# monatis/clip.cpp

Hardware: AMD Instinct MI355X
Metric: image+text embeddings/sec (higher is better)
Workload: dtype f16

## Files before the change

clip_cpp_amd/__init__.py:

```python
import ctypes as C
import os
import weakref

import numpy as np

_HERE = os.path.dirname(os.path.abspath(__file__))
LIB_PATH = os.environ.get("CLIP_AMD_LIB") or os.path.join(_HERE, "libclip.so")


class ClipTextHparams(C.Structure):
    _fields_ = [("n_vocab", C.c_int32), ("num_positions", C.c_int32), ("hidden_size", C.c_int32),
                ("n_intermediate", C.c_int32), ("projection_dim", C.c_int32), ("n_head", C.c_int32),
                ("n_layer", C.c_int32), ("eps", C.c_float)]


class ClipVisionHparams(C.Structure):
    _fields_ = [("image_size", C.c_int32), ("patch_size", C.c_int32), ("hidden_size", C.c_int32),
                ("n_intermediate", C.c_int32), ("projection_dim", C.c_int32), ("n_head", C.c_int32),
                ("n_layer", C.c_int32), ("eps", C.c_float)]


class ClipTokens(C.Structure):
    _fields_ = [("data", C.POINTER(C.c_int32)), ("size", C.c_size_t)]


class ClipImageU8(C.Structure):
    _fields_ = [("nx", C.c_int), ("ny", C.c_int), ("data", C.POINTER(C.c_uint8)), ("size", C.c_size_t)]


class ClipImageF32(C.Structure):
    _fields_ = [("nx", C.c_int), ("ny", C.c_int), ("data", C.POINTER(C.c_float)), ("size", C.c_size_t)]


class ClipImageU8Batch(C.Structure):
    _fields_ = [("data", C.POINTER(ClipImageU8)), ("size", C.c_size_t)]


class ClipImageF32Batch(C.Structure):
    _fields_ = [("data", C.POINTER(ClipImageF32)), ("size", C.c_size_t)]


API_SYMBOLS = [
    "clip_model_load", "clip_free", "clip_get_text_hparams", "clip_get_vision_hparams", "clip_tokenize",
    "clip_image_u8_make", "clip_image_f32_make", "clip_image_u8_clean", "clip_image_f32_clean", "clip_image_u8_free",
    "clip_image_f32_free", "clip_image_load_from_file", "clip_image_preprocess", "clip_image_batch_preprocess",
    "clip_text_encode", "clip_image_encode", "clip_image_batch_encode", "clip_compare_text_and_image",
    "clip_similarity_score", "softmax_with_sorting", "clip_zero_shot_label_image", "clip_model_quantize",
    "ggml_time_init", "ggml_time_us", "ggml_time_ms",
]
AMD_SYMBOLS = [
    "clip_amd_device_count", "clip_amd_model_load", "clip_amd_model_load_multi", "clip_amd_ctx_device_count", "clip_amd_weights_from_cache", "clip_amd_shard_bounds",
    "clip_amd_gathered_embeddings", "clip_amd_ctx_device", "clip_amd_set_stream", "clip_amd_set_device_shared", "clip_amd_image_batch_encode_device_multi",
    "clip_amd_text_batch_encode_device_multi", "clip_amd_encode_pair_device_multi",
    "clip_amd_image_batch_encode_device", "clip_text_batch_encode", "clip_amd_text_batch_encode_device",
    "clip_amd_image_batch_preprocess_device", "clip_amd_image_batch_encode_u8",
    "clip_amd_zero_shot_score_device", "clip_amd_zero_shot_label_images",
    "clip_amd_synchronize", "clip_amd_profile_enable", "clip_amd_profile_read", "clip_amd_profile_report",
    "clip_amd_test_gemm", "clip_amd_test_gemm_ex", "clip_amd_test_gemm_tile", "clip_amd_test_gemm_tile_ex", "clip_amd_test_skinny", "clip_amd_test_layernorm", "clip_amd_test_attention", "clip_amd_bench_gemm",
    "clip_amd_test_attention_ex", "clip_amd_bench_attention",
    "clip_amd_index_create", "clip_amd_index_add", "clip_amd_index_add_device", "clip_amd_index_size", "clip_amd_index_dim",
    "clip_amd_index_search", "clip_amd_index_search_device", "clip_amd_index_save", "clip_amd_index_load", "clip_amd_index_free",
    "clip_amd_bench_search", "clip_amd_index_range_search", "clip_amd_index_pairs", "clip_amd_bench_range",
]

_lib = None


def build_lib(force=False):
    import importlib
    return importlib.import_module(__name__ + ".build").build(force=force)


def lib():
    global _lib
    if _lib is not None:
        return _lib
    if not os.path.exists(LIB_PATH):
        build_lib()
    L = C.CDLL(LIB_PATH)
    vp, i32, f32p = C.c_void_p, C.c_int, C.POINTER(C.c_float)
    L.clip_model_load.restype = vp
    L.clip_model_load.argtypes = [C.c_char_p, i32]
    L.clip_amd_model_load.restype = vp
    L.clip_amd_model_load.argtypes = [C.c_char_p, i32, i32]
    L.clip_amd_model_load_multi.restype = vp
    L.clip_amd_model_load_multi.argtypes = [C.c_char_p, i32, i32]
    L.clip_amd_ctx_device_count.restype = i32
    L.clip_amd_ctx_device_count.argtypes = [vp]
    L.clip_amd_weights_from_cache.restype = i32
    L.clip_amd_weights_from_cache.argtypes = [vp]
    L.clip_amd_shard_bounds.argtypes = [i32, i32, i32, C.POINTER(i32), C.POINTER(i32), C.POINTER(i32)]
    L.clip_amd_gathered_embeddings.restype = vp
    L.clip_amd_gathered_embeddings.argtypes = [vp, i32]
    L.clip_free.argtypes = [vp]
    L.clip_get_text_hparams.restype = C.POINTER(ClipTextHparams)
    L.clip_get_text_hparams.argtypes = [vp]
    L.clip_get_vision_hparams.restype = C.POINTER(ClipVisionHparams)
    L.clip_get_vision_hparams.argtypes = [vp]
    L.clip_tokenize.restype = C.c_bool
    L.clip_tokenize.argtypes = [vp, C.c_char_p, C.POINTER(ClipTokens)]
    L.clip_image_u8_make.restype = C.POINTER(ClipImageU8)
    L.clip_image_f32_make.restype = C.POINTER(ClipImageF32)
    L.clip_image_u8_clean.argtypes = [C.POINTER(ClipImageU8)]
    L.clip_image_f32_clean.argtypes = [C.POINTER(ClipImageF32)]
    L.clip_image_u8_free.argtypes = [C.POINTER(ClipImageU8)]
    L.clip_image_f32_free.argtypes = [C.POINTER(ClipImageF32)]
    L.clip_image_load_from_file.restype = C.c_bool
    L.clip_image_load_from_file.argtypes = [C.c_char_p, C.POINTER(ClipImageU8)]
    L.clip_image_preprocess.restype = C.c_bool
    L.clip_image_preprocess.argtypes = [vp, C.POINTER(ClipImageU8), C.POINTER(ClipImageF32)]
    L.clip_image_batch_preprocess.argtypes = [vp, i32, C.POINTER(ClipImageU8Batch), C.POINTER(ClipImageF32Batch)]
    L.clip_text_encode.restype = C.c_bool
    L.clip_text_encode.argtypes = [vp, i32, C.POINTER(ClipTokens), f32p, C.c_bool]
    L.clip_text_batch_encode.restype = C.c_bool
    L.clip_text_batch_encode.argtypes = [vp, i32, C.POINTER(ClipTokens), C.c_size_t, f32p, C.c_bool]
    L.clip_image_encode.restype = C.c_bool
    L.clip_image_encode.argtypes = [vp, i32, C.POINTER(ClipImageF32), f32p, C.c_bool]
    L.clip_image_batch_encode.restype = C.c_bool
    L.clip_image_batch_encode.argtypes = [vp, i32, C.POINTER(ClipImageF32Batch), f32p, C.c_bool]
    L.clip_compare_text_and_image.restype = C.c_bool
    L.clip_compare_text_and_image.argtypes = [vp, i32, C.c_char_p, C.POINTER(ClipImageU8), f32p]
    L.clip_similarity_score.restype = C.c_float
    L.clip_similarity_score.argtypes = [f32p, f32p, i32]
    L.softmax_with_sorting.restype = C.c_bool
    L.softmax_with_sorting.argtypes = [f32p, i32, f32p, C.POINTER(C.c_int)]
    L.clip_zero_shot_label_image.restype = C.c_bool
    L.clip_zero_shot_label_image.argtypes = [vp, i32, C.POINTER(ClipImageU8), C.POINTER(C.c_char_p), C.c_size_t, f32p,
                                             C.POINTER(C.c_int)]
    L.clip_model_quantize.restype = C.c_bool
    L.clip_model_quantize.argtypes = [C.c_char_p, C.c_char_p, i32]
    L.clip_amd_device_count.restype = i32
    L.clip_amd_ctx_device.restype = i32
    L.clip_amd_ctx_device.argtypes = [vp]
    L.clip_amd_set_stream.argtypes = [vp, vp]
    L.clip_amd_set_device_shared.restype = None
    L.clip_amd_set_device_shared.argtypes = [vp, i32]
    L.clip_amd_synchronize.argtypes = [vp]
    L.clip_amd_image_batch_encode_device.restype = C.c_bool
    L.clip_amd_image_batch_encode_device.argtypes = [vp, vp, i32, vp, C.c_bool]
    L.clip_amd_image_batch_preprocess_device.restype = C.c_bool
    L.clip_amd_image_batch_preprocess_device.argtypes = [vp, C.POINTER(ClipImageU8), i32, vp]
    L.clip_amd_zero_shot_score_device.restype = C.c_bool
    L.clip_amd_zero_shot_score_device.argtypes = [vp, vp, i32, vp, i32, i32, vp, vp]
    L.clip_amd_zero_shot_label_images.restype = C.c_bool
    L.clip_amd_zero_shot_label_images.argtypes = [vp, C.POINTER(ClipImageU8), i32, C.POINTER(C.c_char_p), C.c_size_t, f32p, C.POINTER(C.c_int)]
    L.clip_amd_image_batch_encode_u8.restype = C.c_bool
    L.clip_amd_image_batch_encode_u8.argtypes = [vp, C.POINTER(ClipImageU8), i32, f32p, C.c_bool]
    L.clip_amd_text_batch_encode_device.restype = C.c_bool
    L.clip_amd_text_batch_encode_device.argtypes = [vp, vp, C.POINTER(C.c_int32), i32, vp, C.c_bool]
    L.clip_amd_image_batch_encode_device_multi.restype = C.c_bool
    L.clip_amd_image_batch_encode_device_multi.argtypes = [vp, C.POINTER(vp), i32, C.c_bool, f32p]
    L.clip_amd_text_batch_encode_device_multi.restype = C.c_bool
    L.clip_amd_text_batch_encode_device_multi.argtypes = [vp, C.POINTER(vp), C.POINTER(C.c_int32), i32, C.c_bool, f32p]
    L.clip_amd_encode_pair_device_multi.restype = C.c_bool
    L.clip_amd_encode_pair_device_multi.argtypes = [vp, C.POINTER(vp), i32, C.POINTER(vp), C.POINTER(C.c_int32), i32, C.c_bool, f32p, f32p]
    L.clip_amd_profile_enable.argtypes = [vp, C.c_bool]
    L.clip_amd_profile_report.restype = i32
    L.clip_amd_profile_report.argtypes = [vp, C.c_char_p, i32, C.c_bool]
    L.clip_amd_test_gemm.restype = i32
    L.clip_amd_test_gemm.argtypes = [i32, vp, C.c_int64, C.c_int64, f32p, C.c_int64, f32p, f32p, f32p, i32, i32]
    L.clip_amd_test_gemm_ex.restype = i32
    L.clip_amd_test_gemm_ex.argtypes = [i32, vp, C.c_int64, C.c_int64, f32p, C.c_int64, f32p, f32p, f32p, i32, i32, i32, C.c_float, i32, i32, f32p]
    L.clip_amd_test_lnfold.restype = i32
    L.clip_amd_test_lnfold.argtypes = [i32, vp, C.c_int64, C.c_int64, vp, C.c_int64, f32p, C.c_int64, f32p, f32p, f32p, f32p, C.c_float, f32p,
                                       i32, i32, i32, i32, i32, C.c_float, f32p, f32p]
    L.clip_amd_test_gemm_tile.restype = i32
    L.clip_amd_test_gemm_tile.argtypes = [C.c_int64, C.c_int64, C.c_int64, i32]
    L.clip_amd_test_gemm_tile_ex.restype = i32
    L.clip_amd_test_gemm_tile_ex.argtypes = [C.c_int64, C.c_int64, C.c_int64, i32, i32]
    L.clip_amd_test_skinny.restype = i32
    L.clip_amd_test_skinny.argtypes = [i32, vp, C.c_int64, C.c_int64, f32p, C.c_int64, f32p, f32p, f32p, f32p, C.c_float, f32p, i32, i32, C.c_float, f32p]
    L.clip_amd_bench_gemm.restype = C.c_float
    L.clip_amd_bench_gemm.argtypes = [i32, C.c_int64, C.c_int64, C.c_int64, i32, i32, i32]
    L.clip_amd_test_layernorm.restype = i32
    L.clip_amd_test_layernorm.argtypes = [f32p, f32p, f32p, C.c_float, C.c_int64, C.c_int64, f32p, i32]
    L.clip_amd_test_attention.restype = i32
    L.clip_amd_test_attention.argtypes = [f32p, i32, i32, i32, i32, i32, f32p]
    L.clip_amd_test_attention_ex.restype = i32
    L.clip_amd_test_attention_ex.argtypes = [f32p, i32, i32, i32, i32, i32, f32p, i32]
    L.clip_amd_bench_attention.restype = C.c_float
    L.clip_amd_bench_attention.argtypes = [i32, i32, i32, i32, i32, i32, i32]
    i64, i64p = C.c_int64, C.POINTER(C.c_int64)
    L.clip_amd_index_create.restype = vp
    L.clip_amd_index_create.argtypes = [vp, i32, i32]
    L.clip_amd_index_add.restype = C.c_bool
    L.clip_amd_index_add.argtypes = [vp, f32p, i64]
    L.clip_amd_index_add_device.restype = C.c_bool
    L.clip_amd_index_add_device.argtypes = [vp, vp, i64]
    L.clip_amd_index_size.restype = i64
    L.clip_amd_index_size.argtypes = [vp]
    L.clip_amd_index_dim.restype = i32
    L.clip_amd_index_dim.argtypes = [vp]
    L.clip_amd_index_search.restype = C.c_bool
    L.clip_amd_index_search.argtypes = [vp, f32p, i32, i32, f32p, i64p]
    L.clip_amd_index_search_device.restype = C.c_bool
    L.clip_amd_index_search_device.argtypes = [vp, vp, i32, i32, vp, vp]
    L.clip_amd_index_save.restype = C.c_bool
    L.clip_amd_index_save.argtypes = [vp, C.c_char_p]
    L.clip_amd_index_load.restype = vp
    L.clip_amd_index_load.argtypes = [vp, C.c_char_p]
    L.clip_amd_index_free.restype = None
    L.clip_amd_index_free.argtypes = [vp]
    L.clip_amd_bench_search.restype = C.c_float
    L.clip_amd_bench_search.argtypes = [i32, i64, i32, i32, i32, i32]
    L.clip_amd_index_range_search.restype = i64
    L.clip_amd_index_range_search.argtypes = [vp, f32p, i32, C.c_float, i64p, f32p, i64p, i64]
    L.clip_amd_index_pairs.restype = i64
    L.clip_amd_index_pairs.argtypes = [vp, C.c_float, i64p, f32p, i64p, i64]
    L.clip_amd_bench_range.restype = C.c_float
    L.clip_amd_bench_range.argtypes = [i32, i64, i32, i32, C.c_float, i32]
    _lib = L
    return L


def device_count():
    return lib().clip_amd_device_count()


def _fp(a):
    return a.ctypes.data_as(C.POINTER(C.c_float))


def _struct_to_dict(s):
    return {f: getattr(s, f) for f, _ in s._fields_}


class Clip:

    def __init__(self, model_path_or_repo_id, verbosity=0, device=None, n_devices=None):
        L = lib()
        path = os.fsencode(model_path_or_repo_id)
        if n_devices is not None:
            self.ctx = L.clip_amd_model_load_multi(path, verbosity, int(n_devices))
        elif device is None:
            self.ctx = L.clip_model_load(path, verbosity)
        else:
            self.ctx = L.clip_amd_model_load(path, verbosity, int(device))
        if not self.ctx:
            raise RuntimeError("clip_model_load failed for %r (no file, malformed GGUF, or no HIP device)" % (model_path_or_repo_id,))
        self.vec_dim = self.vision_config["projection_dim"] or self.text_config["projection_dim"]

    @property
    def vision_config(self):
        return _struct_to_dict(lib().clip_get_vision_hparams(self.ctx).contents)

    @property
    def text_config(self):
        return _struct_to_dict(lib().clip_get_text_hparams(self.ctx).contents)

    @property
    def device(self):
        return lib().clip_amd_ctx_device(self.ctx)

    def tokenize(self, text):
        t = ClipTokens()
        if not lib().clip_tokenize(self.ctx, text.encode("utf-8"), C.byref(t)):
            raise RuntimeError("Could not tokenize text")
        return [t.data[i] for i in range(t.size)]

    def encode_text(self, tokens, n_threads=os.cpu_count(), normalize=True):
        arr = (C.c_int32 * len(tokens))(*tokens)
        t = ClipTokens(C.cast(arr, C.POINTER(C.c_int32)), len(tokens))
        out = np.empty(self.text_config["projection_dim"], dtype=np.float32)
        if not lib().clip_text_encode(self.ctx, n_threads or 1, C.byref(t), _fp(out), normalize):
            raise RuntimeError("Could not encode text")
        return out.tolist()

    def load_preprocess_encode_image(self, image_path, n_threads=os.cpu_count(), normalize=True):
        L = lib()
        img = L.clip_image_u8_make()
        res = L.clip_image_f32_make()
        try:
            if not L.clip_image_load_from_file(os.fsencode(image_path), img):
                raise RuntimeError("Could not load image '%s'" % image_path)
            if not L.clip_image_preprocess(self.ctx, img, res):
                raise RuntimeError("Could not preprocess image")
            out = np.empty(self.vec_dim, dtype=np.float32)
            if not L.clip_image_encode(self.ctx, n_threads or 1, res, _fp(out), normalize):
                raise RuntimeError("Could not encode image")
            return out.tolist()
        finally:
            L.clip_image_u8_free(img)
            L.clip_image_f32_free(res)

    def calculate_similarity(self, text_embedding, image_embedding):
        a = np.asarray(text_embedding, dtype=np.float32)
        b = np.asarray(image_embedding, dtype=np.float32)
        return float(lib().clip_similarity_score(_fp(a), _fp(b), a.size))

    def compare_text_and_image(self, text, image_path, n_threads=os.cpu_count()):
        L = lib()
        img = L.clip_image_u8_make()
        try:
            if not L.clip_image_load_from_file(os.fsencode(image_path), img):
                raise RuntimeError("Could not load image '%s'" % image_path)
            score = C.c_float()
            if not L.clip_compare_text_and_image(self.ctx, n_threads or 1, text.encode("utf-8"), img, C.byref(score)):
                raise RuntimeError("Could not compare text and image")
            return score.value
        finally:
            L.clip_image_u8_free(img)

    def zero_shot_label_image(self, image_path, labels, n_threads=os.cpu_count()):
        L = lib()
        img = L.clip_image_u8_make()
        try:
            if not L.clip_image_load_from_file(os.fsencode(image_path), img):
                raise RuntimeError("Could not load image '%s'" % image_path)
            return self.zero_shot_label_pixels(img, labels, n_threads)
        finally:
            L.clip_image_u8_free(img)

    def zero_shot_label_pixels(self, img_u8_ptr, labels, n_threads=1):
        n = len(labels)
        arr = (C.c_char_p * n)(*[s.encode("utf-8") for s in labels])
        scores = np.empty(n, dtype=np.float32)
        idx = np.empty(n, dtype=np.int32)
        if not lib().clip_zero_shot_label_image(self.ctx, n_threads or 1, img_u8_ptr, arr, n, _fp(scores),
                                                idx.ctypes.data_as(C.POINTER(C.c_int))):
            raise RuntimeError("Could not zero-shot label image")
        return scores.tolist(), idx.tolist()

    def preprocess(self, rgb):
        rgb = np.ascontiguousarray(rgb, dtype=np.uint8)
        ny, nx, _ = rgb.shape
        src = ClipImageU8(nx, ny, rgb.ctypes.data_as(C.POINTER(C.c_uint8)), rgb.size)
        res = ClipImageF32()
        if not lib().clip_image_preprocess(self.ctx, C.byref(src), C.byref(res)):
            raise RuntimeError("Could not preprocess image")
        S = self.vision_config["image_size"]
        out = np.ctypeslib.as_array(res.data, shape=(S, S, 3)).copy()
        lib().clip_image_f32_clean(C.byref(res))
        return out

    @staticmethod
    def _u8_array(images):
        if isinstance(images, np.ndarray) and images.ndim == 4 and images.shape[0] > 0:
            blk = np.ascontiguousarray(images, dtype=np.uint8)
            B = blk.shape[0]
            rec = np.empty(B, dtype=np.dtype([("nx", np.int32), ("ny", np.int32), ("data", np.uint64), ("size", np.uint64)], align=True))
            assert rec.dtype.itemsize == C.sizeof(ClipImageU8)
            rec["nx"], rec["ny"], rec["size"] = blk.shape[2], blk.shape[1], blk[0].size
            rec["data"] = blk.ctypes.data + np.arange(B, dtype=np.uint64) * np.uint64(blk.strides[0])
            return (blk, rec), C.cast(rec.ctypes.data, C.POINTER(ClipImageU8)), B
        keep = [np.ascontiguousarray(im, dtype=np.uint8) for im in images]
        arr = (ClipImageU8 * len(keep))()
        for i, im in enumerate(keep):
            arr[i] = ClipImageU8(im.shape[1], im.shape[0], im.ctypes.data_as(C.POINTER(C.c_uint8)), im.size)
        return keep, arr, len(keep)

    def encode_images_u8(self, images, normalize=True):
        keep, arr, n = self._u8_array(images)
        out = np.empty((n, self.vision_config["projection_dim"]), dtype=np.float32)
        if not lib().clip_amd_image_batch_encode_u8(self.ctx, arr, n, _fp(out), normalize):
            raise RuntimeError("clip_amd_image_batch_encode_u8 failed (see stderr)")
        return out

    def zero_shot_label_images(self, images, labels):
        keep, arr, B = self._u8_array(images)
        n = len(labels)
        lab = (C.c_char_p * n)(*[l.encode("utf-8") for l in labels])
        scores = np.empty((B, n), dtype=np.float32)
        idx = np.empty((B, n), dtype=np.int32)
        if not lib().clip_amd_zero_shot_label_images(self.ctx, arr, B, lab, n, _fp(scores), idx.ctypes.data_as(C.POINTER(C.c_int))):
            raise RuntimeError("clip_amd_zero_shot_label_images failed (see stderr)")
        return scores, idx

    def preprocess_device(self, images, d_out_ptr):
        keep, arr, B = self._u8_array(images)
        if not lib().clip_amd_image_batch_preprocess_device(self.ctx, arr, B, C.c_void_p(d_out_ptr)):
            raise RuntimeError("clip_amd_image_batch_preprocess_device failed (see stderr)")
        self.synchronize()

    @property
    def weights_from_cache(self):
        return bool(lib().clip_amd_weights_from_cache(self.ctx))

    @property
    def n_devices(self):
        return lib().clip_amd_ctx_device_count(self.ctx)

    def encode_images(self, imgs, normalize=True, n_threads=None):
        imgs = np.ascontiguousarray(imgs, dtype=np.float32)
        B, S = imgs.shape[0], imgs.shape[1]
        rec = np.empty(B, dtype=np.dtype([("nx", np.int32), ("ny", np.int32), ("data", np.uint64), ("size", np.uint64)], align=True))
        assert rec.dtype.itemsize == C.sizeof(ClipImageF32)
        rec["nx"], rec["ny"], rec["size"] = S, imgs.shape[2], imgs[0].size if B else 0
        rec["data"] = imgs.ctypes.data + np.arange(B, dtype=np.uint64) * np.uint64(imgs.strides[0] if B else 0)
        batch = ClipImageF32Batch(C.cast(rec.ctypes.data, C.POINTER(ClipImageF32)), B)
        out = np.empty((B, self.vision_config["projection_dim"]), dtype=np.float32)
        if not lib().clip_image_batch_encode(self.ctx, n_threads or min(16, os.cpu_count() or 1), C.byref(batch), _fp(out), normalize):
            raise RuntimeError("clip_image_batch_encode failed (see stderr)")
        return out

    def encode_texts(self, token_lists, normalize=True):
        n = len(token_lists)
        keep = [np.ascontiguousarray(t, dtype=np.int32) for t in token_lists]
        arr = (ClipTokens * n)()
        for i, t in enumerate(keep):
            arr[i] = ClipTokens(t.ctypes.data_as(C.POINTER(C.c_int32)), t.size)
        out = np.empty((n, self.text_config["projection_dim"]), dtype=np.float32)
        if not lib().clip_text_batch_encode(self.ctx, 1, C.cast(arr, C.POINTER(ClipTokens)), n, _fp(out), normalize):
            raise RuntimeError("clip_text_batch_encode failed (see stderr)")
        return out

    def set_stream(self, stream_handle):
        lib().clip_amd_set_stream(self.ctx, C.c_void_p(stream_handle))

    def set_device_shared(self, shared=True):
        lib().clip_amd_set_device_shared(self.ctx, 1 if shared else 0)

    def synchronize(self):
        lib().clip_amd_synchronize(self.ctx)

    def encode_images_device(self, d_imgs_ptr, batch, d_out_ptr, normalize=True):
        if not lib().clip_amd_image_batch_encode_device(self.ctx, C.c_void_p(d_imgs_ptr), batch, C.c_void_p(d_out_ptr), normalize):
            raise RuntimeError("clip_amd_image_batch_encode_device failed (see stderr)")

    def encode_texts_device(self, d_ids_ptr, offsets, d_out_ptr, normalize=True):
        off = np.ascontiguousarray(offsets, dtype=np.int32)
        if not lib().clip_amd_text_batch_encode_device(self.ctx, C.c_void_p(d_ids_ptr), off.ctypes.data_as(C.POINTER(C.c_int32)),
                                                       off.size - 1, C.c_void_p(d_out_ptr), normalize):
            raise RuntimeError("clip_amd_text_batch_encode_device failed (see stderr)")

    def encode_images_device_multi(self, d_img_ptrs, total, normalize=True, out=None):
        arr = (C.c_void_p * len(d_img_ptrs))(*[C.c_void_p(p) for p in d_img_ptrs])
        if not lib().clip_amd_image_batch_encode_device_multi(self.ctx, arr, total, normalize, _fp(out) if out is not None else None):
            raise RuntimeError("clip_amd_image_batch_encode_device_multi failed (see stderr)")
        return out

    def encode_texts_device_multi(self, d_ids_ptrs, offsets, normalize=True, out=None):
        off = np.ascontiguousarray(offsets, dtype=np.int32)
        arr = (C.c_void_p * len(d_ids_ptrs))(*[C.c_void_p(p) for p in d_ids_ptrs])
        if not lib().clip_amd_text_batch_encode_device_multi(self.ctx, arr, off.ctypes.data_as(C.POINTER(C.c_int32)), off.size - 1, normalize,
                                                             _fp(out) if out is not None else None):
            raise RuntimeError("clip_amd_text_batch_encode_device_multi failed (see stderr)")
        return out

    def encode_pair_device_multi(self, d_img_ptrs, n_images, d_ids_ptrs, offsets, normalize=True, out_img=None, out_txt=None):
        off = np.ascontiguousarray(offsets, dtype=np.int32)
        ia = (C.c_void_p * len(d_img_ptrs))(*[C.c_void_p(p) for p in d_img_ptrs])
        ta = (C.c_void_p * len(d_ids_ptrs))(*[C.c_void_p(p) for p in d_ids_ptrs])
        if not lib().clip_amd_encode_pair_device_multi(self.ctx, ia, n_images, ta, off.ctypes.data_as(C.POINTER(C.c_int32)), off.size - 1, normalize,
                                                       _fp(out_img) if out_img is not None else None, _fp(out_txt) if out_txt is not None else None):
            raise RuntimeError("clip_amd_encode_pair_device_multi failed (see stderr)")
        return out_img, out_txt

    def gathered_embeddings_ptr(self, device_index=0):
        return lib().clip_amd_gathered_embeddings(self.ctx, device_index)

    def profile(self, on=True):
        lib().clip_amd_profile_enable(self.ctx, on)

    def profile_report(self, reset=True):
        n = lib().clip_amd_profile_report(self.ctx, None, 0, False)
        buf = C.create_string_buffer(n + 16)
        lib().clip_amd_profile_report(self.ctx, buf, n + 16, reset)
        out = {}
        for line in buf.value.decode().splitlines():
            tag, launches, ms, fl, by = line.split()
            out[tag] = dict(launches=int(launches), ms=float(ms), flops=float(fl), bytes=float(by))
        return out

    def close(self):
        if getattr(self, "ctx", None):
            for ix in list(getattr(self, "_indexes", ())):
                ix.close()
            lib().clip_free(self.ctx)
            self.ctx = None

    def __del__(self):
        try:
            self.close()
        except Exception:
            pass


class Index:

    DTYPES = {"f32": 0, "f16": 1, "i8": 3}
# ... 120 lines not shown
```

clip_cpp_amd/build.py:

```python
import os
import shutil
import subprocess
import sys
from concurrent.futures import ThreadPoolExecutor

HERE = os.path.dirname(os.path.abspath(__file__))
CSRC = os.path.join(HERE, "csrc")
BUILD = os.path.join(HERE, "build")
LIB = os.path.join(HERE, "libclip.so")
GGML_STUB = os.path.join(HERE, "libggml.so")
ARCH = "gfx950"

HOST_SOURCES = ["gguf.cpp", "quant.cpp", "load.cpp", "forward.cpp", "tokenizer.cpp", "preprocess.cpp", "image_io.cpp", "image_formats.cpp",
                "jpeg_decode.cpp", "host_pipeline.cpp", "api.cpp", "search.cpp"]
HIP_SOURCES = ["k_attn.hip", "k_attn_long.hip", "k_attn_f32.hip", "k_misc.hip", "k_preproc.hip", "k_gemm.hip", "k_gemm8.hip", "k_gemm4.hip", "k_gemm32.hip", "k_gemm_f32.hip", "k_skinny.hip", "k_gemm_ring.hip", "k_fold.hip", "k_search.hip", "k_join.hip"]
GEMM_WTYPES = [0, 1, 2, 3, 4, 5]
EXTRA_FLAGS = {"k_attn_f32.hip": ["-fno-slp-vectorize"], "k_attn_long.hip": ["-fno-slp-vectorize"], "k_gemm_f32.hip": ["-fno-slp-vectorize"]}

COMMON = ["-O3", "-std=c++17", "-fPIC", "-ffp-contract=off", "-Wall", "-Wno-unused-function", "-Wno-unused-result", "-Wno-inline-asm", "-Wno-bitwise-instead-of-logical",
          "-I" + os.path.join(os.path.dirname(HERE), "include")]


def hipcc():
    for c in (os.environ.get("HIPCC"), shutil.which("hipcc"), "/opt/rocm/bin/hipcc"):
        if c and os.path.exists(c):
            return c
    raise RuntimeError("hipcc not found")


def _newer(target, deps):
    if not os.path.exists(target):
        return True
    t = os.path.getmtime(target)
    return any(os.path.getmtime(d) > t for d in deps)


def _run(cmd):
    r = subprocess.run(cmd, stdout=subprocess.PIPE, stderr=subprocess.STDOUT, text=True)
    if r.returncode != 0:
        raise RuntimeError("command failed: %s\n%s" % (" ".join(cmd), r.stdout))
    return r.stdout


def build(force=False, verbose=False):
    os.makedirs(BUILD, exist_ok=True)
    cc = hipcc()
    headers = [os.path.join(CSRC, f) for f in os.listdir(CSRC) if f.endswith(".h")]
    headers += [os.path.join(os.path.dirname(HERE), "include", f) for f in ("clip.h", "clip_amd.h")]
    jobs = []
    objs = []
    for src in HOST_SOURCES:
        o = os.path.join(BUILD, src + ".o")
        objs.append(o)
        s = os.path.join(CSRC, src)
        if force or _newer(o, [s] + headers):
            jobs.append([cc, "-x", "hip", "--offload-arch=" + ARCH, "-fwrapv"] + COMMON + ["-c", s, "-o", o])
    for src in HIP_SOURCES:
        s = os.path.join(CSRC, src)
        o = os.path.join(BUILD, src + ".o")
        objs.append(o)
        if force or _newer(o, [s] + headers):
            jobs.append([cc, "--offload-arch=" + ARCH] + COMMON + EXTRA_FLAGS.get(src, []) + ["-c", s, "-o", o])
    s = os.path.join(CSRC, "k_gemm.hip")
    for wt in GEMM_WTYPES:
        o = os.path.join(BUILD, "k_gemm_wt%d.o" % wt)
        objs.append(o)
        if force or _newer(o, [s] + headers):
            jobs.append([cc, "--offload-arch=" + ARCH] + COMMON + ["-DCLIPAMD_GEMM_WT=%d" % wt, "-c", s, "-o", o])
    s = os.path.join(CSRC, "k_skinny.hip")
    for wt in GEMM_WTYPES:
        o = os.path.join(BUILD, "k_skinny_wt%d.o" % wt)
        objs.append(o)
        if force or _newer(o, [s] + headers):
            jobs.append([cc, "--offload-arch=" + ARCH] + COMMON + ["-DCLIPAMD_SKINNY_WT=%d" % wt, "-c", s, "-o", o])
    s = os.path.join(CSRC, "k_gemm_ring.hip")
    for wt in GEMM_WTYPES:
        o = os.path.join(BUILD, "k_gemm_ring_wt%d.o" % wt)
        objs.append(o)
        if force or _newer(o, [s] + headers):
            jobs.append([cc, "--offload-arch=" + ARCH] + COMMON + ["-DCLIPAMD_RING_WT=%d" % wt, "-c", s, "-o", o])
    if jobs:
        with ThreadPoolExecutor(max_workers=min(8, os.cpu_count() or 4)) as ex:
            for out in ex.map(_run, jobs):
                if verbose and out.strip():
                    print(out)
    if force or jobs or _newer(LIB, objs):
        _run([cc, "--offload-arch=" + ARCH, "-shared", "-fPIC", "-o", LIB] + objs + ["-lz", "-lpthread", "-ldl"])
    stub_src = os.path.join(CSRC, "ggml_stub.c")
    if force or _newer(GGML_STUB, [stub_src]):
        _run(["gcc", "-O2", "-fPIC", "-shared", "-o", GGML_STUB, stub_src])
    return LIB


if __name__ == "__main__":
    p = build(force="--force" in sys.argv, verbose=True)
    print("built", p)
```

clip_cpp_amd/csrc/api.cpp:

```cpp
#include <algorithm>
#include <chrono>
#include <cmath>
#include <cstdio>
#include <cstdlib>
#include <cstring>
#include <exception>
#include <thread>
#include <vector>

#include "../../include/clip_amd.h"
#include "model.h"

using namespace clipamd;

namespace {

int default_device() {
    const char * e = getenv("CLIP_AMD_DEVICE");
    if (!e || !*e) e = getenv("LOCAL_RANK");
    if (e && *e) {
        int n = 0;
        if (hipGetDeviceCount(&n) == hipSuccess && n > 0) return atoi(e) % n;
        (void)hipGetLastError();
    }
// ... 683 lines not shown
    DBuf dmu((size_t)M * 4), dmu2((size_t)M * 4);
    if (fold == 2) {
        std::vector<float> mu((size_t)M);
        for (int64_t m = 0; m < M; m++) {
            double sacc = 0;
            for (int64_t k = 0; k < h; k++) sacc += resid[m * h + k];
            mu[(size_t)m] = (float)(sacc / (double)h);
        }
        (void)hipMemcpy(dmu.p, mu.data(), (size_t)M * 4, hipMemcpyHostToDevice);
    }
    launch_f32_to_f16((const float *)da32.p, (int)K1, (half_t *)da16.p, W1.Kpad, (int)M, (int)K1, W1.Kpad, s);
    DBuf skw((size_t)64 << 20), skc(4096 * 4);
    (void)hipMemset(skc.p, 0, 4096 * 4);
    DBuf panel1((size_t)W1.Npad * W1.Kpad * 2), panel2((size_t)W2.Npad * W2.Kpad * 2);
    auto common = [&](GemmParams & p, const DBuf & panel, const DevWeight & W) {
        p.sk_ws = (float *)skw.p; p.sk_ws_floats = (size_t)16 << 20; p.sk_cnt = (unsigned *)skc.p; p.sk_cnt_n = 4096;
        p.w16_scratch = (half_t *)panel.p; p.w16_scratch_halfs = panel.p ? (size_t)W.Npad * W.Kpad : 0;
    };
    GemmParams p1;
    p1.A = (const half_t *)da16.p; p1.lda = W1.Kpad; p1.M = (int)M; p1.W = W1; p1.bias = (const float *)db1.p; p1.out = dx.p; p1.ldc = (int)h;
    p1.resid = (const float *)dx.p;
    common(p1, panel1, W1);
    GemmParams p2;
    p2.A = (const half_t *)dxn.p; p2.lda = W2.Kpad; p2.M = (int)M; p2.W = W2; p2.out = dy16.p; p2.ldc = (int)N2; p2.qcols = qcols; p2.qscale = qscale;
    common(p2, panel2, W2);
    const int epi = epi2 == 1 ? EPI_F16 : epi2 == 2 ? EPI_GELU_F16 : EPI_QGELU_F16;
    if (tile1 < 0) {
        if (M > 128 || h > 2048) { (void)hipFree(w1base); (void)hipFree(w2base); return -5; }
        DBuf dskst((size_t)2 * SKINNY_MAX_ROWS * 128 * sizeof(float2));
        SkinnyParams a1;
        a1.A16 = (const half_t *)da16.p; a1.lda = W1.Kpad; a1.M = (int)M; a1.W = W1; a1.bias = (const float *)db1.p; a1.out = dx.p; a1.ldc = (int)h; a1.resid = (const float *)dx.p;
        SkinnyParams a2;
        a2.M = (int)M; a2.W = W2; a2.out = dy16.p; a2.ldc = (int)N2; a2.qcols = qcols; a2.qscale = qscale; a2.eps = eps;
        if (fold) {
            launch_fold_vectors(W2, (const float *)dg.p, (const float *)dbeta.p, (const float *)db2.p, (float *)dc.p, (float *)dbf.p, s);
            a1.xg_out = (half_t *)dxn.p; a1.ldxg = W2.Kpad; a1.xg_gamma = (const float *)dg.p; a1.fstats_out = (float2 *)dstats.p; a1.fstride_out = st_stride;
            a2.A16 = (const half_t *)dxn.p; a2.lda = W2.Kpad; a2.bias = (const float *)dbf.p; a2.ln_c = (const float *)dc.p;
            a2.fstats = (const float2 *)dstats.p; a2.fslots = (int)h / 16; a2.fslotw = 16; a2.fstride = st_stride;
            if (fold == 2) { a1.xg_mu = (const float *)dmu.p; a2.ln_mu = (const float *)dmu.p; a2.mu_out = (float *)dmu2.p; }
        } else {
            a1.stats_out = (float2 *)dskst.p;
            a2.x32 = (const float *)dx.p; a2.ldx = (int)h; a2.ln_w = (const float *)dg.p; a2.ln_b = (const float *)dbeta.p; a2.stats_in = (const float2 *)dskst.p;
            a2.stats_slots = (int)h / 16; a2.bias = (const float *)db2.p;
        }
        int rc2 = 0;
        if (!skinny_supported(a1, EPI_RESID_F32) || !skinny_supported(a2, epi)) rc2 = -5;
        else {
            launch_skinny(a1, EPI_RESID_F32, s);
            launch_skinny(a2, epi, s);
            launch_f16_to_f32((const half_t *)dy16.p, (int)N2, (float *)dy32.p, (int)N2, (int)M, (int)N2, s);
            if (hipDeviceSynchronize() != hipSuccess || hipGetLastError() != hipSuccess) rc2 = -4;
            else {
                (void)hipMemcpy(x1_out, dx.p, (size_t)M * h * 4, hipMemcpyDeviceToHost);
                (void)hipMemcpy(y_out, dy32.p, (size_t)M * N2 * 4, hipMemcpyDeviceToHost);
            }
        }
        (void)hipFree(w1base);
        (void)hipFree(w2base);
        return rc2;
    }
    if (fold) {
        launch_fold_vectors(W2, (const float *)dg.p, (const float *)dbeta.p, (const float *)db2.p, (float *)dc.p, (float *)dbf.p, s);
        p1.xg_out = (half_t *)dxn.p; p1.ldxg = W2.Kpad; p1.xg_gamma = (const float *)dg.p; p1.stats_out = (float2 *)dstats.p; p1.stats_stride = st_stride;
        int t1 = tile1 ? tile1 : gemm_tile_for((int)M, (int)h, W1.Kpad, W1.wtype != W_F16);
        const int slotw = gemm_fold_slotw(t1);
        if (fold == 2) p1.xg_mu = (const float *)dmu.p;
        launch_gemm(p1, EPI_RESID_F32, tile1, s);
        p2.bias = (const float *)dbf.p; p2.ln_c = (const float *)dc.p; p2.ln_stats = (const float2 *)dstats.p; p2.ln_slotw = slotw; p2.ln_slots = (int)h / slotw;
        p2.ln_stride = st_stride; p2.ln_eps = eps;
        if (fold == 2) { p1.xg_mu = (const float *)dmu.p; p2.ln_mu = (const float *)dmu.p; p2.mu_out = (float *)dmu2.p; }
        launch_gemm(p2, epi, tile2, s);
    } else {
        launch_gemm(p1, EPI_RESID_F32, tile1, s);
        launch_layernorm((const float *)dx.p, (int)h, nullptr, 1, (const float *)dg.p, (const float *)dbeta.p, eps, (int)M, (int)h, (half_t *)dxn.p, W2.Kpad, nullptr, 0, s);
        p2.bias = (const float *)db2.p;
        launch_gemm(p2, epi, tile2, s);
    }
    launch_f16_to_f32((const half_t *)dy16.p, (int)N2, (float *)dy32.p, (int)N2, (int)M, (int)N2, s);
    int rc = 0;
    if (hipDeviceSynchronize() != hipSuccess || hipGetLastError() != hipSuccess) rc = -4;
    else {
        (void)hipMemcpy(x1_out, dx.p, (size_t)M * h * 4, hipMemcpyDeviceToHost);
        (void)hipMemcpy(y_out, dy32.p, (size_t)M * N2 * 4, hipMemcpyDeviceToHost);
    }
    (void)hipFree(w1base);
    (void)hipFree(w2base);
    return rc;
}

int clip_amd_test_gemm(int type, const void * w_raw, int64_t N, int64_t K, const float * x, int64_t M, const float * bias, const float * resid,
                       float * y, int epilogue, int tile) {
    return clip_amd_test_gemm_ex(type, w_raw, N, K, x, M, bias, resid, y, epilogue, tile, 0, 1.0f, 0, 0, nullptr);
}


float clip_amd_bench_gemm(int type, int64_t N, int64_t K, int64_t M, int epilogue, int tile, int iters) {
    int ndev = 0;
    if (hipGetDeviceCount(&ndev) != hipSuccess || ndev <= 0) { (void)hipGetLastError(); return -1.f; }
    std::vector<float> w((size_t)N * K);
    uint32_t st = 12345u;
    for (auto & v : w) { st = st * 1664525u + 1013904223u; v = ((int)(st >> 9) % 2001 - 1000) * 4e-5f; }
    std::vector<uint8_t> raw(ggml_row_bytes(type, K) * (size_t)N);
    if (raw.empty() || quantize_rows(type, w.data(), raw.data(), N, K) == 0) return -2.f;
    DevWeight W;
    void * wbase = nullptr;
    if (!repack_for_test(type, raw.data(), N, K, W, &wbase)) return -2.f;
    const int Kpad = W.Kpad;
    DBuf dx((size_t)(M + 1) * Kpad * 2), dbias((size_t)N * 4), dout((size_t)M * N * 4);
    std::vector<uint16_t> hx((size_t)M * Kpad);
    for (auto & v : hx) { st = st * 1664525u + 1013904223u; v = f32_to_f16_bits(((int)(st >> 9) % 2001 - 1000) * 1e-3f); }
    (void)hipMemcpy(dx.p, hx.data(), hx.size() * 2, hipMemcpyHostToDevice);
    (void)hipMemset(dbias.p, 0, (size_t)N * 4);
    (void)hipMemset(dout.p, 0, (size_t)M * N * 4);
    GemmParams p;
    p.A = (const half_t *)dx.p; p.lda = Kpad; p.M = (int)M; p.W = W; p.bias = (const float *)dbias.p; p.ldc = (int)N; p.out = dout.p;
    p.resid = (const float *)dout.p; p.qcols = 0;
    DBuf skw((size_t)64 << 20), skc(4096 * 4);
    (void)hipMemset(skc.p, 0, 4096 * 4);
    p.sk_ws = (float *)skw.p; p.sk_ws_floats = (size_t)16 << 20; p.sk_cnt = (unsigned *)skc.p; p.sk_cnt_n = 4096;
    DBuf panel((size_t)W.Npad * W.Kpad * 2);
    const bool pre = (epilogue >> 16) & 1;
    if (pre && W.wtype != W_F16 && W.wtype != W_F32 && panel.p) {
        const DevWeight * w = &W;
        half_t * o = (half_t *)panel.p;
        launch_dequant(&w, &o, 1, nullptr);
        p.w16_pre = (const half_t *)panel.p;
    } else {
        p.w16_scratch = (half_t *)panel.p; p.w16_scratch_halfs = panel.p ? (size_t)W.Npad * W.Kpad : 0;
    }
    p.debug = (epilogue >> 8) & 0xFF;
    const bool fold = (epilogue >> 17) & 1;
    epilogue &= 0xFF;
    const int st_stride = (int)((M + 63) & ~(int64_t)63);
    DBuf dstats(fold ? (size_t)(N > K ? N : K) / 32 * st_stride * 8 + 64 : 16), dvec(fold ? (size_t)(N > K ? N : K) * 4 + 64 : 16), dxg(fold ? (size_t)M * N * 2 + 64 : 16);
    if (fold) {
        std::vector<float> hs((size_t)(N > K ? N : K) / 32 * st_stride * 2), hv((size_t)(N > K ? N : K), 1.0f);
        for (size_t i = 0; i < hs.size(); i += 2) { hs[i] = 0.5f * 64; hs[i + 1] = 60.f; }
        (void)hipMemcpy(dstats.p, hs.data(), hs.size() * 4, hipMemcpyHostToDevice);
        (void)hipMemcpy(dvec.p, hv.data(), hv.size() * 4, hipMemcpyHostToDevice);
        if (epilogue == EPI_RESID_F32) {
            p.xg_out = (half_t *)dxg.p; p.ldxg = (int)N; p.xg_gamma = (const float *)dvec.p; p.stats_out = (float2 *)dstats.p; p.stats_stride = st_stride;
        } else if (epilogue == EPI_F16 || epilogue == EPI_GELU_F16 || epilogue == EPI_QGELU_F16) {
            p.ln_c = (const float *)dvec.p; p.ln_stats = (const float2 *)dstats.p; p.ln_slotw = 64; p.ln_slots = (int)K / 64; p.ln_stride = st_stride; p.ln_eps = 1e-5f;
        }
    }
    hipEvent_t a, b;
    (void)hipEventCreate(&a);
    (void)hipEventCreate(&b);
    int rot = 1;
    { const char * e = getenv("GEMM_ROTATE"); if (e) rot = atoi(e); if (rot < 1) rot = 1; if (rot > 64) rot = 64; }
    std::vector<DevWeight> Ws(1, p.W);
    std::vector<const half_t *> pans(1, p.w16_pre);
    std::vector<void *> owned;
    for (int r = 1; r < rot; r++) {
        DevWeight Wr;
        void * base = nullptr;
        if (!repack_for_test(type, raw.data(), N, K, Wr, &base)) break;
        owned.push_back(base);
        const half_t * pr = nullptr;
        if (pre && Wr.wtype != W_F16 && Wr.wtype != W_F32) {
            void * pp = nullptr;
            if (hipMalloc(&pp, (size_t)Wr.Npad * Wr.Kpad * 2) != hipSuccess) break;
            owned.push_back(pp);
            const DevWeight * w = &Wr;
            half_t * o = (half_t *)pp;
            launch_dequant(&w, &o, 1, nullptr);
            pr = (const half_t *)pp;
        }
        Ws.push_back(Wr);
        pans.push_back(pr);
    }
    rot = (int)Ws.size();
    auto go = [&](int i) { p.W = Ws[i % rot]; if (pre) p.w16_pre = pans[i % rot]; launch_gemm(p, epilogue, tile, nullptr); };
    for (int i = 0; i < 3; i++) go(i);
    (void)hipEventRecord(a, nullptr);
    for (int i = 0; i < iters; i++) go(i);
    (void)hipEventRecord(b, nullptr);
    float ms = -1.f;
    if (hipEventSynchronize(b) == hipSuccess && hipGetLastError() == hipSuccess) (void)hipEventElapsedTime(&ms, a, b);
    (void)hipEventDestroy(a);
    (void)hipEventDestroy(b);
    for (void * o : owned) (void)hipFree(o);
    if (getenv("CLIPAMD_G8_STAMPS")) {
        const int nwg = 4096;
        std::vector<unsigned long long> st((size_t)nwg * 8);
        (void)hipMemcpy(st.data(), skw.p, st.size() * 8, hipMemcpyDeviceToHost);
        FILE * f = fopen(getenv("CLIPAMD_G8_STAMPS"), "a");
        if (f) {
            fprintf(f, "# N=%lld K=%lld M=%lld epi=%d tile=%d\n", (long long)N, (long long)K, (long long)M, epilogue, tile);
            for (int i = 0; i < nwg; i++) {
                const unsigned long long * s8 = &st[(size_t)i * 8];
                if (!s8[0] || !s8[3]) continue;
                fprintf(f, "%d %llu %llu %llu %llu %llu %llu %llu\n", i, s8[0], s8[1], s8[2], s8[3], s8[5], s8[4], s8[6]);
            }
            fclose(f);
        }
    }
    (void)hipFree(wbase);
    return ms < 0 ? -4.f : ms * 1000.f / iters;
}

int clip_amd_test_skinny(int type, const void * w_raw, int64_t N, int64_t K, const float * x, int64_t M, const float * bias, const float * resid,
                         const float * ln_w, const float * ln_b, float eps, float * y, int epilogue, int qcols, float qscale, float * stats_out) {
    int ndev = 0;
    if (hipGetDeviceCount(&ndev) != hipSuccess || ndev <= 0) { (void)hipGetLastError(); return -1; }
    DevWeight W;
    void * wbase = nullptr;
    if (!repack_for_test(type, w_raw, N, K, W, &wbase)) return -2;
    const int Kpad = W.Kpad;
    DBuf dx32((size_t)M * K * 4), dx16((size_t)(M + 1) * Kpad * 2), dbias((size_t)N * 4), dout((size_t)M * N * 4), dout32((size_t)M * N * 4), dlw((size_t)K * 4), dlb((size_t)K * 4),
        dst((size_t)2 * SKINNY_MAX_ROWS * 128 * 8);
    hipStream_t s = nullptr;
    (void)hipMemcpy(dx32.p, x, (size_t)M * K * 4, hipMemcpyHostToDevice);
    if (bias) (void)hipMemcpy(dbias.p, bias, (size_t)N * 4, hipMemcpyHostToDevice);
    (void)hipMemset(dst.p, 0, (size_t)2 * SKINNY_MAX_ROWS * 128 * 8);
    SkinnyParams p;
    p.M = (int)M; p.W = W; p.bias = bias ? (const float *)dbias.p : nullptr; p.ldc = (int)N; p.qcols = qcols; p.qscale = qscale;
    if (ln_w) {
        (void)hipMemcpy(dlw.p, ln_w, (size_t)K * 4, hipMemcpyHostToDevice);
        (void)hipMemcpy(dlb.p, ln_b, (size_t)K * 4, hipMemcpyHostToDevice);
        launch_row_stats((const float *)dx32.p, (int)K, (int)M, (int)K, (float2 *)dst.p, s);
        p.x32 = (const float *)dx32.p; p.ldx = (int)K; p.ln_w = (const float *)dlw.p; p.ln_b = (const float *)dlb.p; p.eps = eps;
        p.stats_in = (const float2 *)dst.p; p.stats_slots = 1;
    } else {
        launch_f32_to_f16((const float *)dx32.p, (int)K, (half_t *)dx16.p, Kpad, (int)M, (int)K, Kpad, s);
        p.A16 = (const half_t *)dx16.p; p.lda = Kpad;
    }
    int epi = EPI_F32;
    switch (epilogue) {
    case 0: epi = EPI_F32; p.out = dout32.p; break;
    case 1: epi = EPI_F16; p.out = dout.p; break;
    case 2: epi = EPI_GELU_F16; p.out = dout.p; break;
    case 3: epi = EPI_QGELU_F16; p.out = dout.p; break;
    case 4:
        epi = EPI_RESID_F32;
        (void)hipMemcpy(dout32.p, resid, (size_t)M * N * 4, hipMemcpyHostToDevice);
        p.out = dout32.p; p.resid = (const float *)dout32.p;
        p.stats_out = (float2 *)dst.p + (size_t)SKINNY_MAX_ROWS * 128;
        break;
    default: (void)hipFree(wbase); return -3;
    }
    int rc = 0;
    if (!skinny_supported(p, epi)) rc = -5;
    else {
        launch_skinny(p, epi, s);
        if (epi == EPI_F16 || epi == EPI_GELU_F16 || epi == EPI_QGELU_F16)
            launch_f16_to_f32((const half_t *)dout.p, (int)N, (float *)dout32.p, (int)N, (int)M, (int)N, s);
        if (hipDeviceSynchronize() != hipSuccess || hipGetLastError() != hipSuccess) rc = -4;
        else {
            (void)hipMemcpy(y, dout32.p, (size_t)M * N * 4, hipMemcpyDeviceToHost);
            if (stats_out && epi == EPI_RESID_F32) (void)hipMemcpy(stats_out, (float2 *)dst.p + (size_t)SKINNY_MAX_ROWS * 128, (size_t)128 * 128 * 8, hipMemcpyDeviceToHost);
        }
    }
    (void)hipFree(wbase);
    return rc;
}

int clip_amd_test_layernorm(const float * x, const float * w, const float * b, float eps, int64_t rows, int64_t h, float * y, int out_f16) {
    int ndev = 0;
    if (hipGetDeviceCount(&ndev) != hipSuccess || ndev <= 0) { (void)hipGetLastError(); return -1; }
    DBuf dx((size_t)rows * h * 4), dw((size_t)h * 4), db((size_t)h * 4), dy((size_t)rows * h * 4), dh_((size_t)rows * h * 2);
    (void)hipMemcpy(dx.p, x, (size_t)rows * h * 4, hipMemcpyHostToDevice);
    (void)hipMemcpy(dw.p, w, (size_t)h * 4, hipMemcpyHostToDevice);
    (void)hipMemcpy(db.p, b, (size_t)h * 4, hipMemcpyHostToDevice);
    if (out_f16) {
        launch_layernorm((const float *)dx.p, (int)h, nullptr, 1, (const float *)dw.p, (const float *)db.p, eps, (int)rows, (int)h, (half_t *)dh_.p, (int)h, nullptr, 0, nullptr);
        launch_f16_to_f32((const half_t *)dh_.p, (int)h, (float *)dy.p, (int)h, (int)rows, (int)h, nullptr);
    } else {
        launch_layernorm((const float *)dx.p, (int)h, nullptr, 1, (const float *)dw.p, (const float *)db.p, eps, (int)rows, (int)h, nullptr, 0, (float *)dy.p, (int)h, nullptr);
    }
    if (hipDeviceSynchronize() != hipSuccess || hipGetLastError() != hipSuccess) return -4;
    (void)hipMemcpy(y, dy.p, (size_t)rows * h * 4, hipMemcpyDeviceToHost);
    return 0;
}

static bool launch_attention_kernel(int kernel, const half_t * qkv, half_t * out, int nseq, int T, int h, int n_head, bool causal) {
    switch (kernel) {
    case 0: return launch_attention(qkv, out, nseq, T, nullptr, T, h, n_head, causal, nullptr);
    case 1: return launch_attention_whole_row(qkv, out, nseq, T, nullptr, T, h, n_head, causal, nullptr);
    case 2: return launch_attention_long(qkv, out, nseq, T, nullptr, T, h, n_head, causal, nullptr);
    }
    return false;
}

int clip_amd_test_attention_ex(const float * qkv, int nseq, int T, int h, int n_head, int causal, float * out, int kernel) {
    int ndev = 0;
    if (hipGetDeviceCount(&ndev) != hipSuccess || ndev <= 0) { (void)hipGetLastError(); return -1; }
    if (nseq <= 0 || T <= 0 || h <= 0 || n_head <= 0 || h % n_head) return -3;
    const size_t rows = (size_t)nseq * T;
    DBuf d32(rows * 3 * h * 4), d16(rows * 3 * h * 2), o16(rows * h * 2), o32(rows * h * 4);
    (void)hipMemcpy(d32.p, qkv, rows * 3 * h * 4, hipMemcpyHostToDevice);
    launch_f32_to_f16((const float *)d32.p, 3 * h, (half_t *)d16.p, 3 * h, (int)rows, 3 * h, 3 * h, nullptr);
    if (!launch_attention_kernel(kernel, (const half_t *)d16.p, (half_t *)o16.p, nseq, T, h, n_head, causal != 0)) return -2;
    launch_f16_to_f32((const half_t *)o16.p, h, (float *)o32.p, h, (int)rows, h, nullptr);
    if (hipDeviceSynchronize() != hipSuccess || hipGetLastError() != hipSuccess) return -4;
    (void)hipMemcpy(out, o32.p, rows * h * 4, hipMemcpyDeviceToHost);
    return 0;
}

int clip_amd_test_attention(const float * qkv, int nseq, int T, int h, int n_head, int causal, float * out) {
    return clip_amd_test_attention_ex(qkv, nseq, T, h, n_head, causal, out, 0);
}

float clip_amd_bench_attention(int nseq, int T, int h, int n_head, int causal, int kernel, int iters) {
    int ndev = 0;
    if (hipGetDeviceCount(&ndev) != hipSuccess || ndev <= 0) { (void)hipGetLastError(); return -1.f; }
    if (nseq <= 0 || T <= 0 || h <= 0 || n_head <= 0 || h % n_head || iters <= 0) return -3.f;
    const size_t rows = (size_t)nseq * T;
    std::vector<uint16_t> hx(rows * 3 * h);
    uint32_t st = 12345u;
    const float qs = 1.0f / sqrtf((float)(h / n_head));
    for (size_t i = 0; i < hx.size(); i++) {
        st = st * 1664525u + 1013904223u;
        const float v = ((int)(st >> 9) % 2001 - 1000) * 1e-3f;
        hx[i] = f32_to_f16_bits((int)(i % (3 * h)) < h ? v * qs : v);
    }
    DBuf d16(hx.size() * 2), o16(rows * h * 2);
    (void)hipMemcpy(d16.p, hx.data(), hx.size() * 2, hipMemcpyHostToDevice);
    if (!launch_attention_kernel(kernel, (const half_t *)d16.p, (half_t *)o16.p, nseq, T, h, n_head, causal != 0)) return -2.f;
    if (hipDeviceSynchronize() != hipSuccess) { (void)hipGetLastError(); return -4.f; }
    hipEvent_t e0, e1;
    (void)hipEventCreate(&e0);
    (void)hipEventCreate(&e1);
    (void)hipEventRecord(e0, nullptr);
    for (int i = 0; i < iters; i++) launch_attention_kernel(kernel, (const half_t *)d16.p, (half_t *)o16.p, nseq, T, h, n_head, causal != 0);
    (void)hipEventRecord(e1, nullptr);
    float ms = -1.f;
    if (hipEventSynchronize(e1) != hipSuccess || hipEventElapsedTime(&ms, e0, e1) != hipSuccess) { (void)hipGetLastError(); ms = -1.f; }
    (void)hipEventDestroy(e0);
    (void)hipEventDestroy(e1);
    return ms < 0 ? -4.f : ms * 1000.f / iters;
}

#endif

}
```

clip_cpp_amd/csrc/forward.cpp:

```cpp
#include <cmath>
#include <cstdio>
#include <cstdlib>
#include <cstring>
#include <thread>
#include <utility>

#include "model.h"

namespace clipamd {

namespace {

constexpr size_t kGuardBytes = 4096;
constexpr int kGuardByte = 0xA5;
bool guard_mode() {
    static const bool on = [] { const char * e = getenv("CLIP_AMD_GUARD"); return e && e[0] == '1'; }();
    return on;
}

struct Carver {
    uint8_t * base;
    size_t off = 0;
    std::vector<size_t> * gaps = nullptr;
    explicit Carver(void * b, std::vector<size_t> * g = nullptr) : base((uint8_t *)b), gaps(g) { if (gaps) gaps->clear(); }
    template <typename T> T * take(size_t n) {
        off = (off + 255) & ~(size_t)255;
        T * p = base ? (T *)(base + off) : nullptr;
        off += n * sizeof(T);
        if (guard_mode()) {
            if (gaps) gaps->push_back(off);
            off += kGuardBytes;
        }
        return p;
    }
};

bool guard_arm(clip_ctx * ctx) {
    if (!guard_mode()) return true;
    if (hipMemsetAsync(ctx->ws.base, 0xFF, ctx->ws.bytes, ctx->stream) != hipSuccess) return false;
    for (size_t o : ctx->guard_gaps)
        if (hipMemsetAsync((uint8_t *)ctx->ws.base + o, kGuardByte, kGuardBytes, ctx->stream) != hipSuccess) return false;
    static const bool selftest = [] { const char * e = getenv("CLIP_AMD_GUARD_SELFTEST"); return e && e[0] == '1'; }();
    if (selftest && !ctx->guard_gaps.empty())
        return hipMemsetAsync((uint8_t *)ctx->ws.base + ctx->guard_gaps.back() + 100, 0, 1, ctx->stream) == hipSuccess;
    return true;
}

bool guard_check(clip_ctx * ctx, const char * who) {
    if (!guard_mode()) return true;
    if (hipStreamSynchronize(ctx->stream) != hipSuccess) return false;
    std::vector<uint8_t> h(kGuardBytes);
    bool ok = true;
    for (size_t i = 0; i < ctx->guard_gaps.size(); i++) {
        if (hipMemcpy(h.data(), (uint8_t *)ctx->ws.base + ctx->guard_gaps[i], kGuardBytes, hipMemcpyDeviceToHost) != hipSuccess) return false;
        for (size_t k = 0; k < kGuardBytes; k++)
            if (h[k] != (uint8_t)kGuardByte) {
                fprintf(stderr, "%s: CLIP_AMD_GUARD: workspace buffer %zu was written %zu bytes past its end\n", who, i, k);
                ok = false;
                break;
            }
    }
    return ok;
}

struct ProfScope {
    clip_ctx * ctx;
    hipEvent_t a = nullptr, b = nullptr;
    bool on;
    std::string tag;
    double flops, bytes;
    ProfScope(clip_ctx * c, const char * family, long m, long n, long k, double fl, double by) : ctx(c), on(c->profiling), flops(fl), bytes(by) {
        if (!on) return;
        char buf[96];
        snprintf(buf, sizeof buf, "%s:%ldx%ldx%ld", family, m, n, k);
        tag = buf;
        (void)hipEventCreate(&a);
        (void)hipEventCreate(&b);
        (void)hipEventRecord(a, ctx->stream);
    }
    ~ProfScope() {
        if (!on) return;
        (void)hipEventRecord(b, ctx->stream);
        ctx->pending.push_back({a, b, tag, flops, bytes});
    }
};

double weight_bytes(const DevWeight & W) {
    const double nblk = (double)(W.K / 32) * W.N;
    switch (W.wtype) {
    case W_F16: return (double)W.N * W.K * 2;
    case W_Q4_0: return nblk * 18;
    case W_Q4_1: return nblk * 20;
    case W_Q5_0: return nblk * 22;
    case W_Q5_1: return nblk * 24;
    case W_Q8_0: return nblk * 34;
    case W_F32: return (double)W.N * W.K * 4;
    }
    return 0;
}

bool acts_f32(const clip_ctx * ctx, const DevTower & tw) {
    return ctx->f32_acts && !tw.layers.empty() && tw.layers[0].qkv.wtype == W_F32 && tw.layers[0].o.wtype == W_F32 && tw.layers[0].ff1.wtype == W_F32 && tw.layers[0].ff2.wtype == W_F32 &&
           tw.proj.wtype == W_F32;
}
void layernorm_act(bool f32, const float * x, int ldx, const int * in_rows, int in_row_mul, const float * w, const float * b, float eps, int rows, int h, half_t * dst,
                   hipStream_t s) {
    if (f32) launch_layernorm(x, ldx, in_rows, in_row_mul, w, b, eps, rows, h, nullptr, 0, (float *)dst, h, s);
    else launch_layernorm(x, ldx, in_rows, in_row_mul, w, b, eps, rows, h, dst, h, nullptr, 0, s);
}

bool device_shared(const clip_ctx * ctx) { return ctx->device_shared || ctx->sibling_busy || ctx->owner != nullptr; }

void gemm(clip_ctx * ctx, const char * what, const GemmParams & p0, int epi) {
    GemmParams p = p0;
    p.shared_device = device_shared(ctx);
    p.sk_ws = ctx->sk_ws; p.sk_ws_floats = ctx->sk_ws_floats; p.sk_cnt = ctx->sk_cnt; p.sk_cnt_n = ctx->sk_cnt_n;
    if (!ctx->profiling) {
        launch_gemm(p, epi, 0, ctx->stream);
        return;
    }
    const int wt = p.w16_pre ? (int)W_F16 : p.W.wtype;
    const int tile = gemm_tile_for(p.M, p.W.N, p.W.Kpad, wt != W_F16, p.shared_device);
    const bool panel = gemm_tile_uses_panel(tile) && wt == W_F16;
    const double fl = 2.0 * p.M * (double)p.W.N * p.W.K;
    const double wb = wt == W_F16 ? (double)p.W.N * p.W.K * 2 : weight_bytes(p.W);
    const double by = wb + (double)p.M * p.W.K * 2 + (double)p.M * p.W.N * (epi == EPI_F16 || epi == EPI_GELU_F16 || epi == EPI_QGELU_F16 ? 2 : epi == EPI_RESID_F32 ? 8 : 4)
                      + (p.xg_out ? (double)p.M * p.W.N * 2 : 0.0);
    char fam[96];
    if (wt == W_F32) snprintf(fam, sizeof fam, "gemm_f32_kernel<%d>/%s", epi, what);
    else if (panel && tile % 1000 == 261 && (epi == EPI_F16 || epi == EPI_GELU_F16 || epi == EPI_QGELU_F16)) snprintf(fam, sizeof fam, "gemm32_kernel<%d,4,%d>/%s", tile / 1000 == 320 ? 5 : 4, epi, what);
    else if (panel && tile % 1000 >= 259) snprintf(fam, sizeof fam, "gemm4_kernel<%d>/%s", epi, what);
    else if (panel) snprintf(fam, sizeof fam, "gemm8_kernel<%d,%d>/%s", tile / 32000, epi, what);
    else if (gemm_tile_is_ring(tile)) snprintf(fam, sizeof fam, "gemm_ring_kernel<%d,%d,4,%d,%d>/%s", wt, tile % 1000, tile % 1000 >= 128 ? 4 : 2, epi, what);
    else snprintf(fam, sizeof fam, "gemm_dma_kernel<%d,%d,%d,%d>/%s", wt, gemm_tile_uses_panel(tile) ? 160 : tile / 1000, gemm_tile_uses_panel(tile) ? 128 : tile % 1000, epi, what);
    ProfScope ps(ctx, fam, p.M, p.W.N, p.W.K, fl, by);
    launch_gemm(p, epi, 0, ctx->stream);
}

struct LayerPanels { const half_t * qkv = nullptr, * o = nullptr, * ff1 = nullptr, * ff2 = nullptr; };

bool ensure_panel(clip_ctx * ctx, size_t halfs) {
    if (ctx->w16_panel_halfs >= halfs) return true;
    (void)hipStreamSynchronize(ctx->stream);
    if (ctx->w16_panel) (void)hipFree(ctx->w16_panel);
    ctx->w16_panel = nullptr;
    ctx->w16_panel_halfs = 0;
    if (hipMalloc((void **)&ctx->w16_panel, halfs * sizeof(half_t)) != hipSuccess) { (void)hipGetLastError(); return false; }
    ctx->w16_panel_halfs = halfs;
    return true;
}

LayerPanels dequant_layer(clip_ctx * ctx, const DevLayer & l, int rows, const half_t * const * res = nullptr) {
    LayerPanels lp;
    const DevWeight * ws[4] = {&l.qkv, &l.o, &l.ff1, &l.ff2};
    const half_t ** slot[4] = {&lp.qkv, &lp.o, &lp.ff1, &lp.ff2};
    const DevWeight * jw[4];
    half_t * jo[4];
    int nj = 0;
    size_t need = 0;
    bool todo[4];
    for (int i = 0; i < 4; i++) {
        const bool for32 = i == 0 || i == 2;
        if (res && res[i] && (!for32 || gemm_tile_for(rows, ws[i]->N, ws[i]->Kpad, false, device_shared(ctx)) % 1000 == 261)) { *slot[i] = res[i]; todo[i] = false; continue; }
        todo[i] = ws[i]->wtype != W_F16 && ws[i]->wtype != W_F32 && gemm_tile_uses_panel(gemm_tile_for(rows, ws[i]->N, ws[i]->Kpad, true));
        if (todo[i]) need += (size_t)ws[i]->Npad * ws[i]->Kpad;
    }
    if (!need || !ensure_panel(ctx, need)) return lp;
    size_t off = 0;
    for (int i = 0; i < 4; i++)
        if (todo[i]) {
            jw[nj] = ws[i];
            jo[nj] = ctx->w16_panel + off;
            *slot[i] = jo[nj];
            off += (size_t)ws[i]->Npad * ws[i]->Kpad;
            nj++;
        }
    ProfScope ps(ctx, "dequant_layer", rows, nj, 0, 0, (double)need * 2.5625);
    launch_dequant(jw, jo, nj, ctx->stream);
    return lp;
}

bool skinny_enabled() {
    static int on = -1;
    if (on < 0) { const char * e = getenv("CLIP_AMD_SKINNY"); on = !(e && e[0] == '0'); }
    return on != 0;
}

#ifdef CLIPAMD_SK_TIMING
unsigned long long * g_sk_stamps = nullptr;
int g_sk_stamp_launch = 0;
constexpr int SK_STAMP_LAUNCHES = 512;
#endif

void skinny(clip_ctx * ctx, const char * what, const SkinnyParams & p0, int epi) {
#ifdef CLIPAMD_SK_TIMING
    SkinnyParams p = p0;
    if (!g_sk_stamps && hipMalloc((void **)&g_sk_stamps, SK_STAMP_LAUNCHES * 16 * 8) == hipSuccess) (void)hipMemset(g_sk_stamps, 0, SK_STAMP_LAUNCHES * 16 * 8);
    if (g_sk_stamps) p.stamps = g_sk_stamps + (size_t)(g_sk_stamp_launch++ % SK_STAMP_LAUNCHES) * 16;
#else
    const SkinnyParams & p = p0;
#endif
    if (!ctx->profiling) { launch_skinny(p, epi, ctx->stream); return; }
    char fam[96];
    const int nw = (!p.x32 && p.W.Kpad >= 2048 && (epi == EPI_RESID_F32 || epi == EPI_PATCH_F32)) ? 8 : 4;
    snprintf(fam, sizeof fam, "skinny_kernel<%d,1,%d,%d,%s>/%s", p.W.wtype, nw, epi, p.x32 ? "true" : "false", what);
    const double fl = 2.0 * p.M * (double)p.W.N * p.W.K;
    const double by = weight_bytes(p.W) + (double)p.M * p.W.K * (p.x32 ? 4 : 2) + (double)p.M * p.W.N * (epi == EPI_RESID_F32 ? 8 : epi == EPI_F32 || epi == EPI_PATCH_F32 ? 4 : 2);
    ProfScope ps(ctx, fam, p.M, p.W.N, p.W.K, fl, by);
    launch_skinny(p, epi, ctx->stream);
}

int skinny_row_limit() {
    static int lim = -1;
    if (lim < 0) {
        const char * e = getenv("CLIP_AMD_SKINNY_ROWS");
        lim = e ? atoi(e) : 64;
        if (lim > SKINNY_MAX_ROWS) lim = SKINNY_MAX_ROWS;
    }
    return lim;
}

bool layers_fit_skinny(const DevTower & tw, int rows, int h, int ff) {
    if (!skinny_enabled() || rows <= 0 || rows > skinny_row_limit() || h > 2048 || h % 16 || h / 16 > 128 || tw.layers.empty()) return false;
    const DevLayer & l = tw.layers[0];
    if (l.qkv.wtype == W_F32 || l.o.wtype == W_F32 || l.ff1.wtype == W_F32 || l.ff2.wtype == W_F32) return false;
    return l.qkv.K == l.qkv.Kpad && l.ff1.K == l.ff1.Kpad && l.o.N == h && l.ff2.N == h && l.ff1.N == ff;
}

bool run_layers_skinny(clip_ctx * ctx, const DevTower & tw, int rows, int h, int nh, int ff, float eps, int nseq, int T_uniform,
                       const int * d_seq_start, int max_len, bool causal, float * x, half_t * qkv, half_t * att, half_t * mid) {
    hipStream_t s = ctx->stream;
    const int dh = h / nh;
    const float qscale = 1.0f / sqrtf((float)dh);
    const int act = ctx->use_gelu ? EPI_GELU_F16 : EPI_QGELU_F16;
    float2 * stA = ctx->sk_stats, * stB = ctx->sk_stats + (size_t)SKINNY_MAX_ROWS * 128;
    int slotsA = 1;
    for (const DevLayer & l : tw.layers) {
        SkinnyParams q;
        q.x32 = x; q.ldx = h; q.ln_w = l.ln1_w; q.ln_b = l.ln1_b; q.eps = eps; q.stats_in = stA; q.stats_slots = slotsA;
        q.M = rows; q.W = l.qkv; q.bias = l.qkv_b; q.out = qkv; q.ldc = 3 * h; q.qscale = qscale; q.qcols = h;
        skinny(ctx, "ln1_qkv", q, EPI_F16);
        {
            const double afl = 4.0 * (double)nseq * nh * (double)max_len * max_len * dh;
            ProfScope ps(ctx, "attention", nseq * nh, max_len, dh, afl, (double)rows * h * 8);
            if (!launch_attention(qkv, att, nseq, T_uniform, d_seq_start, max_len, h, nh, causal, s)) {
                fprintf(stderr, "clip (hip): attention kernel does not support T=%d d_head=%d\n", max_len, dh);
                return false;
            }
        }
        SkinnyParams o;
        o.A16 = att; o.lda = h; o.M = rows; o.W = l.o; o.bias = l.o_b; o.out = x; o.ldc = h; o.resid = x; o.stats_out = stB;
        skinny(ctx, "out_resid", o, EPI_RESID_F32);
        SkinnyParams u;
        u.x32 = x; u.ldx = h; u.ln_w = l.ln2_w; u.ln_b = l.ln2_b; u.eps = eps; u.stats_in = stB; u.stats_slots = h / 16;
        u.M = rows; u.W = l.ff1; u.bias = l.ff1_b; u.out = mid; u.ldc = ff;
        skinny(ctx, "ln2_ffn_up", u, act);
        SkinnyParams d;
        d.A16 = mid; d.lda = ff; d.M = rows; d.W = l.ff2; d.bias = l.ff2_b; d.out = x; d.ldc = h; d.resid = x; d.stats_out = stA;
        skinny(ctx, "ffn_down_resid", d, EPI_RESID_F32);
        slotsA = h / 16;
    }
    return true;
}

bool run_layers_skinny_fold(clip_ctx * ctx, const DevTower & tw, int rows, int h, int nh, int ff, float eps, int nseq, int T_uniform,
                            const int * d_seq_start, int max_len, bool causal, float * x, half_t * xn, half_t * qkv, half_t * att, half_t * mid,
                            float2 * stats, int stats_stride, float * mu) {
    hipStream_t s = ctx->stream;
    const int dh = h / nh;
    const float qscale = 1.0f / sqrtf((float)dh);
    const int act = ctx->use_gelu ? EPI_GELU_F16 : EPI_QGELU_F16;
    int slots = 1, slotw = h;
    float * mu_cur = mu, * mu_alt = mu ? mu + stats_stride : nullptr;
    auto consume = [&](SkinnyParams & p, const float * c, const float * bf) {
        p.A16 = xn; p.lda = h; p.bias = bf; p.ln_c = c; p.fstats = stats; p.fslots = slots; p.fslotw = slotw; p.fstride = stats_stride; p.eps = eps;
        if (mu) { p.ln_mu = mu_cur; p.mu_out = mu_alt; std::swap(mu_cur, mu_alt); }
    };
    auto produce = [&](SkinnyParams & p, const float * gamma_next) {
        if (!gamma_next) return;
        p.xg_mu = mu_cur;
        p.xg_out = xn; p.ldxg = h; p.xg_gamma = gamma_next; p.fstats_out = stats; p.fstride_out = stats_stride;
        slots = h / 16; slotw = 16;
    };
    for (size_t li = 0; li < tw.layers.size(); li++) {
        const DevLayer & l = tw.layers[li];
        SkinnyParams q;
        q.M = rows; q.W = l.qkv; q.out = qkv; q.ldc = 3 * h; q.qscale = qscale; q.qcols = h;
        consume(q, l.qkv_c, l.qkv_bf);
        skinny(ctx, "ln1_qkv", q, EPI_F16);
        {
            const double afl = 4.0 * (double)nseq * nh * (double)max_len * max_len * dh;
            ProfScope ps(ctx, "attention", nseq * nh, max_len, dh, afl, (double)rows * h * 8);
            if (!launch_attention(qkv, att, nseq, T_uniform, d_seq_start, max_len, h, nh, causal, s)) {
                fprintf(stderr, "clip (hip): attention kernel does not support T=%d d_head=%d\n", max_len, dh);
                return false;
            }
        }
        SkinnyParams o;
        o.A16 = att; o.lda = h; o.M = rows; o.W = l.o; o.bias = l.o_b; o.out = x; o.ldc = h; o.resid = x;
        produce(o, l.ln2_w);
        skinny(ctx, "out_resid", o, EPI_RESID_F32);
        SkinnyParams u;
        u.M = rows; u.W = l.ff1; u.out = mid; u.ldc = ff;
        consume(u, l.ff1_c, l.ff1_bf);
        skinny(ctx, "ln2_ffn_up", u, act);
        SkinnyParams d;
        d.A16 = mid; d.lda = ff; d.M = rows; d.W = l.ff2; d.bias = l.ff2_b; d.out = x; d.ldc = h; d.resid = x;
        produce(d, li + 1 < tw.layers.size() ? tw.layers[li + 1].ln1_w : nullptr);
        skinny(ctx, "ffn_down_resid", d, EPI_RESID_F32);
    }
    return true;
}

bool run_layers(clip_ctx * ctx, const DevTower & tw, int rows, int h, int nh, int ff, float eps, int nseq, int T_uniform,
                const int * d_seq_start, int max_len, bool causal, float * x, half_t * xn, half_t * qkv, half_t * att, half_t * mid, bool prune_last,
                const half_t * const * resp = nullptr) {
    hipStream_t s = ctx->stream;
    const int dh = h / nh;
    const float qscale = 1.0f / sqrtf((float)dh);
    const int act = ctx->use_gelu ? EPI_GELU_F16 : EPI_QGELU_F16;
    const bool f32 = acts_f32(ctx, tw);
    for (size_t li = 0; li < tw.layers.size(); li++) {
        const DevLayer & l = tw.layers[li];
        const LayerPanels lp = dequant_layer(ctx, l, rows, resp ? resp + 4 * li : nullptr);
        {
            ProfScope ps(ctx, "layernorm", rows, h, 0, 0, (double)rows * h * 6);
            layernorm_act(f32, x, h, nullptr, 1, l.ln1_w, l.ln1_b, eps, rows, h, xn, s);
        }
        GemmParams p;
        p.A = xn; p.lda = h; p.M = rows; p.W = l.qkv; p.bias = l.qkv_b; p.out = qkv; p.ldc = 3 * h; p.w16_pre = lp.qkv;
        p.qscale = qscale; p.qcols = h;
        p.act_f32 = f32;
        gemm(ctx, "gemm_qkv", p, EPI_F16);
        {
            const double afl = 4.0 * (double)nseq * nh * (double)max_len * max_len * dh;
            ProfScope ps(ctx, "attention", nseq * nh, max_len, dh, afl, (double)rows * h * 8);
            if (!(f32 ? launch_attention_f32((const float *)qkv, (float *)att, nseq, T_uniform, d_seq_start, max_len, h, nh, causal, s)
                      : launch_attention(qkv, att, nseq, T_uniform, d_seq_start, max_len, h, nh, causal, s))) {
                fprintf(stderr, "clip (hip): attention kernel does not support T=%d d_head=%d\n", max_len, dh);
                return false;
            }
        }
        if (prune_last && li + 1 == tw.layers.size()) break;
        GemmParams po;
        po.A = att; po.lda = h; po.M = rows; po.W = l.o; po.bias = l.o_b; po.out = x; po.ldc = h; po.resid = x; po.w16_pre = lp.o; po.act_f32 = f32;
        gemm(ctx, "gemm_out", po, EPI_RESID_F32);
        {
            ProfScope ps(ctx, "layernorm", rows, h, 0, 0, (double)rows * h * 6);
            layernorm_act(f32, x, h, nullptr, 1, l.ln2_w, l.ln2_b, eps, rows, h, xn, s);
        }
        GemmParams p1;
        p1.A = xn; p1.lda = h; p1.M = rows; p1.W = l.ff1; p1.bias = l.ff1_b; p1.out = mid; p1.ldc = ff; p1.w16_pre = lp.ff1; p1.act_f32 = f32;
        gemm(ctx, "gemm_ffn_up", p1, act);
        GemmParams p2;
        p2.A = mid; p2.lda = ff; p2.M = rows; p2.W = l.ff2; p2.bias = l.ff2_b; p2.out = x; p2.ldc = h; p2.resid = x; p2.w16_pre = lp.ff2; p2.act_f32 = f32;
        gemm(ctx, "gemm_ffn_down", p2, EPI_RESID_F32);
    }
    return true;
}

bool run_layers_fold(clip_ctx * ctx, const DevTower & tw, int rows, int h, int nh, int ff, float eps, int nseq, int T_uniform,
                     const int * d_seq_start, int max_len, bool causal, float * x, half_t * xn, half_t * qkv, half_t * att, half_t * mid,
                     float2 * stats, int stats_stride, float * mu, bool prune_last, const half_t * const * ff2p = nullptr) {
    hipStream_t s = ctx->stream;
    const int dh = h / nh;
    const float qscale = 1.0f / sqrtf((float)dh);
    const int act = ctx->use_gelu ? EPI_GELU_F16 : EPI_QGELU_F16;
    int slots = 1, slotw = h;
    float * mu_cur = mu, * mu_alt = mu ? mu + stats_stride : nullptr;
    auto consume = [&](GemmParams & p, const float * c, const float * bf) {
        p.A = xn; p.lda = h; p.bias = bf; p.ln_c = c; p.ln_stats = stats; p.ln_slots = slots; p.ln_slotw = slotw; p.ln_stride = stats_stride; p.ln_eps = eps;
        if (mu) { p.ln_mu = mu_cur; p.mu_out = mu_alt; std::swap(mu_cur, mu_alt); }
    };
    auto produce = [&](GemmParams & p, const float * gamma_next) {
        if (!gamma_next) return;
        p.xg_mu = mu_cur;
        p.xg_out = xn; p.ldxg = h; p.xg_gamma = gamma_next; p.stats_out = stats; p.stats_stride = stats_stride;
        const bool quant = !p.w16_pre && p.W.wtype != W_F16;
        slotw = gemm_fold_slotw_for(p.M, p.W.N, p.W.Kpad, quant, device_shared(ctx));
        slots = h / slotw;
    };
    for (size_t li = 0; li < tw.layers.size(); li++) {
        const DevLayer & l = tw.layers[li];
        const LayerPanels lp = dequant_layer(ctx, l, rows, ff2p ? ff2p + 4 * li : nullptr);
        GemmParams p;
        p.M = rows; p.W = l.qkv; p.out = qkv; p.ldc = 3 * h; p.w16_pre = lp.qkv;
        p.qscale = qscale; p.qcols = h;
        consume(p, l.qkv_c, l.qkv_bf);
        gemm(ctx, "gemm_qkv", p, EPI_F16);
        {
            const double afl = 4.0 * (double)nseq * nh * (double)max_len * max_len * dh;
            ProfScope ps(ctx, "attention", nseq * nh, max_len, dh, afl, (double)rows * h * 8);
            if (!launch_attention(qkv, att, nseq, T_uniform, d_seq_start, max_len, h, nh, causal, s)) {
                fprintf(stderr, "clip (hip): attention kernel does not support T=%d d_head=%d\n", max_len, dh);
                return false;
            }
        }
        if (prune_last && li + 1 == tw.layers.size()) break;
        GemmParams po;
        po.A = att; po.lda = h; po.M = rows; po.W = l.o; po.bias = l.o_b; po.out = x; po.ldc = h; po.resid = x; po.w16_pre = lp.o;
        produce(po, l.ln2_w);
        gemm(ctx, "gemm_out", po, EPI_RESID_F32);
        GemmParams p1;
        p1.M = rows; p1.W = l.ff1; p1.out = mid; p1.ldc = ff; p1.w16_pre = lp.ff1;
        consume(p1, l.ff1_c, l.ff1_bf);
        gemm(ctx, "gemm_ffn_up", p1, act);
        GemmParams p2;
        p2.A = mid; p2.lda = ff; p2.M = rows; p2.W = l.ff2; p2.bias = l.ff2_b; p2.out = x; p2.ldc = h; p2.resid = x; p2.w16_pre = lp.ff2;
        produce(p2, li + 1 < tw.layers.size() ? tw.layers[li + 1].ln1_w : nullptr);
        gemm(ctx, "gemm_ffn_down", p2, EPI_RESID_F32);
    }
    return true;
}

bool pooled_tail(clip_ctx * ctx, const DevLayer & l, int n, int h, int ff, float eps, const float * x, const half_t * att, const int * in_rows,
                 int in_row_mul, float * xp, half_t * ap, half_t * xnp, half_t * midp) {
    hipStream_t s = ctx->stream;
    const int act = ctx->use_gelu ? EPI_GELU_F16 : EPI_QGELU_F16;
    const bool f32 = ctx->f32_acts && l.o.wtype == W_F32 && l.ff1.wtype == W_F32 && l.ff2.wtype == W_F32;
    {
        ProfScope ps(ctx, "gather_pooled", n, h, 0, 0, (double)n * h * 12);
        if (f32) {
            launch_gather_rows(x, nullptr, in_rows, in_row_mul, n, h, xp, nullptr, s);
            launch_gather_rows((const float *)att, nullptr, in_rows, in_row_mul, n, h, (float *)ap, nullptr, s);
        } else launch_gather_rows(x, att, in_rows, in_row_mul, n, h, xp, ap, s);
    }
    GemmParams po;
    po.A = ap; po.lda = h; po.M = n; po.W = l.o; po.bias = l.o_b; po.out = xp; po.ldc = h; po.resid = xp; po.act_f32 = f32;
    gemm(ctx, "gemm_out_pooled", po, EPI_RESID_F32);
    {
        ProfScope ps(ctx, "layernorm", n, h, 0, 0, (double)n * h * 6);
        layernorm_act(f32, xp, h, nullptr, 1, l.ln2_w, l.ln2_b, eps, n, h, xnp, s);
    }
    GemmParams p1;
    p1.A = xnp; p1.lda = h; p1.M = n; p1.W = l.ff1; p1.bias = l.ff1_b; p1.out = midp; p1.ldc = ff; p1.act_f32 = f32;
    gemm(ctx, "gemm_ffn_up_pooled", p1, act);
    GemmParams p2;
    p2.A = midp; p2.lda = ff; p2.M = n; p2.W = l.ff2; p2.bias = l.ff2_b; p2.out = xp; p2.ldc = h; p2.resid = xp; p2.act_f32 = f32;
    gemm(ctx, "gemm_ffn_down_pooled", p2, EPI_RESID_F32);
    return true;
}

const half_t * const * resident_panels(clip_ctx * ctx, const DevTower & tw, int which, int rows) {
    if (!ctx->resident_panels_on || tw.layers.empty()) return nullptr;
    if (ctx->owner) {
        clip_ctx * o = ctx->owner;
        return (o->res_panel_mask[which] && o->res_panels[which].size() == 4 * tw.layers.size()) ? o->res_panels[which].data() : nullptr;
    }
    const DevLayer & l0 = tw.layers[0];
    unsigned want = 0;
    if (l0.ff2.wtype != W_F16 && l0.ff2.wtype != W_F32 && rows >= 4096 && gemm_tile_uses_panel(gemm_tile_for(rows, l0.ff2.N, l0.ff2.Kpad, false))) want |= 8u;
    if (l0.o.wtype != W_F16 && l0.o.wtype != W_F32 && rows >= 4096 && rows < 32768 && gemm_tile_uses_panel(gemm_tile_for(rows, l0.o.N, l0.o.Kpad, false))) want |= 2u;
    if (rows >= 32768 && l0.qkv.wtype != W_F16 && l0.qkv.wtype != W_F32 && gemm_tile_for(rows, l0.qkv.N, l0.qkv.Kpad, false, device_shared(ctx)) % 1000 == 261) want |= 1u;
    if (rows >= 32768 && l0.ff1.wtype != W_F16 && l0.ff1.wtype != W_F32 && gemm_tile_for(rows, l0.ff1.N, l0.ff1.Kpad, false, device_shared(ctx)) % 1000 == 261) want |= 4u;
    if (!want) return nullptr;
    auto & tab = ctx->res_panels[which];
    if ((ctx->res_panel_mask[which] & want) == want && tab.size() == 4 * tw.layers.size()) return tab.data();
    hipStreamCaptureStatus cs = hipStreamCaptureStatusNone;
    (void)hipStreamIsCapturing(ctx->stream, &cs);
    if (cs != hipStreamCaptureStatusNone) return (ctx->res_panel_mask[which] && tab.size() == 4 * tw.layers.size()) ? tab.data() : nullptr;
    want |= ctx->res_panel_mask[which];
    (void)hipStreamSynchronize(ctx->stream);
    if (ctx->res_panel_buf[which]) (void)hipFree(ctx->res_panel_buf[which]);
    ctx->res_panel_buf[which] = nullptr;
    ctx->res_panel_mask[which] = 0;
    tab.clear();
    size_t halfs = 0;
    for (const DevLayer & l : tw.layers) {
        const DevWeight * ws[4] = {&l.qkv, &l.o, &l.ff1, &l.ff2};
        for (int i = 0; i < 4; i++) if (want >> i & 1) halfs += (size_t)ws[i]->Npad * ws[i]->Kpad;
    }
    if (hipMalloc((void **)&ctx->res_panel_buf[which], halfs * sizeof(half_t)) != hipSuccess) { (void)hipGetLastError(); return nullptr; }
    size_t off = 0;
    for (const DevLayer & l : tw.layers) {
        const DevWeight * ws[4] = {&l.qkv, &l.o, &l.ff1, &l.ff2};
        for (int i = 0; i < 4; i++) {
            if (!(want >> i & 1)) { tab.push_back(nullptr); continue; }
            half_t * o = ctx->res_panel_buf[which] + off;
            launch_dequant(&ws[i], &o, 1, ctx->stream);
            tab.push_back(o);
            off += (size_t)ws[i]->Npad * ws[i]->Kpad;
        }
    }
    (void)hipStreamSynchronize(ctx->stream);
    ctx->res_panel_mask[which] = want;
    return tab.data();
}

bool fold_pays(const DevTower & tw, int rows, bool shared) {
    if (tw.layers.empty()) return false;
    const DevLayer & l = tw.layers[0];
    for (const DevWeight * w : {&l.qkv, &l.o, &l.ff1, &l.ff2})
        if (gemm_tile_uses_panel(gemm_tile_for(rows, w->N, w->Kpad, w->wtype != W_F16, shared)) &&
            gemm_tile_for(rows, w->N, w->Kpad, w->wtype != W_F16, shared) % 1000 != 261) return false;
    return true;
}

bool check_device(clip_ctx * ctx, const char * who) {
    if (!ctx || ctx->device < 0) {
        fprintf(stderr, "%s: no HIP device bound to this context — the encoders have no CPU fallback\n", who);
        return false;
    }
    if (hipSetDevice(ctx->device) != hipSuccess) {
        fprintf(stderr, "%s: hipSetDevice(%d) failed\n", who, ctx->device);
        return false;
    }
    return true;
}

bool launch_ok(const char * who) {
    const hipError_t e = hipGetLastError();
    if (e != hipSuccess) {
        fprintf(stderr, "%s: HIP launch error: %s\n", who, hipGetErrorString(e));
        return false;
    }
    return true;
}

}

void drop_graphs(clip_ctx * ctx) {
    for (auto & g : ctx->vgraphs) {
        if (g.exec) (void)hipGraphExecDestroy(g.exec);
        if (g.graph) (void)hipGraphDestroy(g.graph);
    }
    ctx->vgraphs.clear();
    for (auto & g : ctx->tgraphs) {
        if (g.exec) (void)hipGraphExecDestroy(g.exec);
        if (g.graph) (void)hipGraphDestroy(g.graph);
    }
    ctx->tgraphs.clear();
}

bool ensure_workspace(clip_ctx * ctx, size_t bytes) {
    if (ctx->ws.bytes >= bytes) return true;
    (void)hipStreamSynchronize(ctx->stream);
    drop_graphs(ctx);
    if (ctx->owner) {
        (void)hipStreamSynchronize(ctx->owner->stream);
        drop_graphs(ctx->owner);
    }
    if (ctx->ws.base) (void)hipFree(ctx->ws.base);
    ctx->ws.base = nullptr;
    ctx->ws.bytes = 0;
    const size_t want = bytes + bytes / 8 + (1 << 20);
    if (hipMalloc(&ctx->ws.base, want) != hipSuccess) {
        (void)hipGetLastError();
        fprintf(stderr, "clip (hip): cannot allocate %zu MB of workspace\n", want >> 20);
        return false;
    }
    ctx->ws.bytes = want;
    return true;
}

bool ensure_pinned(clip_ctx * ctx, size_t bytes) {
    if (ctx->pinned_bytes >= bytes) return true;
    if (ctx->pinned) (void)hipHostFree(ctx->pinned);
    ctx->pinned = nullptr;
    ctx->pinned_bytes = 0;
    if (hipHostMalloc(&ctx->pinned, bytes, hipHostMallocDefault) != hipSuccess) {
        (void)hipGetLastError();
        return false;
    }
    ctx->pinned_bytes = bytes;
    return true;
}

bool ensure_io(clip_ctx * ctx, size_t in_bytes, size_t out_bytes) {
    auto grow = [&](void *& p, size_t & have, size_t want) {
        if (have >= want) return true;
        (void)hipStreamSynchronize(ctx->stream);
        if (p) (void)hipFree(p);
        p = nullptr;
        have = 0;
        if (hipMalloc(&p, want) != hipSuccess) { (void)hipGetLastError(); return false; }
        have = want;
        return true;
    };
    return grow(ctx->io_in, ctx->io_in_bytes, in_bytes) && grow(ctx->io_out, ctx->io_out_bytes, out_bytes);
}

void prof_collect(clip_ctx * ctx) {
    if (ctx->pending.empty()) return;
    (void)hipStreamSynchronize(ctx->stream);
    for (auto & p : ctx->pending) {
        float ms = 0;
        if (hipEventElapsedTime(&ms, p.a, p.b) == hipSuccess) {
            ProfEntry & e = ctx->prof[p.tag];
            e.ms += ms;
            e.launches += 1;
            e.flops += p.flops;
            e.bytes += p.bytes;
        }
        (void)hipEventDestroy(p.a);
        (void)hipEventDestroy(p.b);
    }
    ctx->pending.clear();
}

static bool vision_forward_one(clip_ctx * ctx, const float * d_imgs, int B, float * d_out, bool normalize);

static bool vision_forward_launch(clip_ctx * ctx, const float * d_imgs, int B, float * d_out, bool normalize) {
    bool split = !ctx->weights_borrowed && !ctx->sibling_busy && !ctx->profiling && ctx->has_vision_encoder && B >= 2;
    if (split) {
        if (ctx->split_max >= 0) split = B >= ctx->split_min && B <= ctx->split_max;
        else {
            const auto & hp = ctx->vision_hparams;
            const int G = hp.image_size / hp.patch_size;
            const long rows = (long)B * (G * G + 1);
            split = hp.hidden_size >= 1024 ? (rows >= 2000 && rows <= 8400) : (rows >= 2000 && rows <= 3300);
        }
    }
    int ways = split ? std::min(ctx->split_ways, B) : 1;
    clip_ctx * part_ctx[4] = {ctx, nullptr, nullptr, nullptr};
    if (split) {
        hipStreamCaptureStatus cs = hipStreamCaptureStatusNone;
        (void)hipStreamIsCapturing(ctx->stream, &cs);
        for (int w = 1; w < ways; w++) {
            clip_ctx * have = w == 1 ? ctx->sibling : ctx->more_siblings[w - 2];
            part_ctx[w] = have ? have : (cs == hipStreamCaptureStatusNone ? sibling_context(ctx, w - 1) : nullptr);
            if (!part_ctx[w]) { ways = 1; break; }
        }
    }
    ctx->last_launch_split = ways >= 2;
    if (ways < 2) return vision_forward_one(ctx, d_imgs, B, d_out, normalize);
    const size_t per = (size_t)ctx->vision_hparams.image_size * ctx->vision_hparams.image_size * 3;
    const int proj = ctx->vision_hparams.projection_dim;
    if (hipEventRecord(ctx->ev_fork, ctx->stream) != hipSuccess) return false;
    bool ok = true;
    int b0 = 0;
    for (int w = 0; w < ways; w++) {
        const int n = B / ways + (w < B % ways ? 1 : 0);
        clip_ctx * c = part_ctx[w];
        c->input_f16 = ctx->input_f16;
        const float * src = ctx->input_f16 ? (const float *)((const half_t *)d_imgs + (size_t)b0 * per) : d_imgs + (size_t)b0 * per;
        if (w > 0 && hipStreamWaitEvent(c->stream, ctx->ev_fork, 0) != hipSuccess) return false;
        ok = vision_forward_one(c, src, n, d_out + (size_t)b0 * proj, normalize) && ok;
        b0 += n;
    }
    for (int w = 1; w < ways; w++) {
        hipEvent_t ej = w == 1 ? ctx->ev_join : ctx->ev_join_more[w - 2];
        if (hipEventRecord(ej, part_ctx[w]->stream) != hipSuccess || hipStreamWaitEvent(ctx->stream, ej, 0) != hipSuccess) return false;
    }
    return ok;
}

bool renew_streams_after_failed_capture(clip_ctx * ctx) {
    bool ok = true, synced = false;
    auto one = [&](clip_ctx * c) {
        if (!c) return;
        hipStreamCaptureStatus st = hipStreamCaptureStatusNone;
        const hipError_t qe = hipStreamIsCapturing(c->stream, &st);
        (void)hipGetLastError();
        if (qe == hipSuccess && st == hipStreamCaptureStatusNone) return;
        if (c->stream != c->own_stream) { ok = false; return; }
        if (!synced) { (void)hipDeviceSynchronize(); (void)hipGetLastError(); synced = true; }
        hipStream_t fresh = nullptr;
        if (hipStreamCreateWithFlags(&fresh, hipStreamNonBlocking) != hipSuccess) { (void)hipGetLastError(); ok = false; return; }
        (void)hipStreamDestroy(c->own_stream);
        (void)hipGetLastError();
        c->own_stream = c->stream = fresh;
        if (c->verbosity >= 1 || (c->owner && c->owner->verbosity >= 1)) fprintf(stderr, "clip (hip): stream replaced after an invalidated capture\n");
    };
    one(ctx);
    one(ctx->sibling);
    for (clip_ctx * ms : ctx->more_siblings) one(ms);
    return ok;
}

namespace {
void break_capture_for_test() {
    static const bool on = [] { const char * e = getenv("CLIP_AMD_TEST_BREAK_CAPTURE"); return e && e[0] == '1'; }();
    if (!on) return;
    hipStreamCaptureMode m = hipStreamCaptureModeThreadLocal;
    (void)hipThreadExchangeStreamCaptureMode(&m);
    void * q = nullptr;
    if (hipMalloc(&q, 256) == hipSuccess && q) (void)hipFree(q);
    (void)hipThreadExchangeStreamCaptureMode(&m);
    (void)hipGetLastError();
}
}

bool vision_forward_device(clip_ctx * ctx, const float * d_imgs, int B, float * d_out, bool normalize) {
    if (!check_device(ctx, "clip_image_batch_encode")) return false;
    if (!ctx->graphs_enabled || ctx->profiling || B <= 0 || B > 32 || !ctx->has_vision_encoder || guard_mode())
        return vision_forward_launch(ctx, d_imgs, B, d_out, normalize);
    auto find = [&]() -> clip_ctx::GraphEntry * {
        for (auto & g : ctx->vgraphs)
            if (g.B == B && g.in == d_imgs && g.out == d_out && g.norm == normalize && g.in_f16 == ctx->input_f16 && g.busy_seen == ctx->sibling_busy) return &g;
        return nullptr;
    };
    clip_ctx::GraphEntry * e = find();
    if (e && e->exec) {
        if (e->split && ctx->sibling_busy) return vision_forward_launch(ctx, d_imgs, B, d_out, normalize);
        return hipGraphLaunch(e->exec, ctx->stream) == hipSuccess;
    }
    if (!e) {
        if (ctx->vgraphs.size() >= 16) drop_graphs(ctx);
        ctx->vgraphs.push_back({B, d_imgs, d_out, normalize, ctx->input_f16, 1, nullptr, nullptr, false, ctx->sibling_busy});
        return vision_forward_launch(ctx, d_imgs, B, d_out, normalize);
    }
    if (hipStreamBeginCapture(ctx->stream, hipStreamCaptureModeThreadLocal) != hipSuccess) {
        (void)hipGetLastError();
        return vision_forward_launch(ctx, d_imgs, B, d_out, normalize);
    }
    break_capture_for_test();
    const bool ok = vision_forward_launch(ctx, d_imgs, B, d_out, normalize);
    const bool captured_split = ctx->last_launch_split;
    hipGraph_t graph = nullptr;
    const hipError_t ce = hipStreamEndCapture(ctx->stream, &graph);
    e = find();
    if (!ok || ce != hipSuccess || !graph || !e) {
        (void)hipGetLastError();
        if (graph) (void)hipGraphDestroy(graph);
        ctx->graphs_enabled = false;
        if (!renew_streams_after_failed_capture(ctx)) { fprintf(stderr, "clip_image_batch_encode: the caller's stream is left in an invalidated capture\n"); return false; }
        return vision_forward_launch(ctx, d_imgs, B, d_out, normalize);
    }
    hipGraphExec_t exec = nullptr;
    if (hipGraphInstantiate(&exec, graph, nullptr, nullptr, 0) != hipSuccess) {
        (void)hipGetLastError();
        (void)hipGraphDestroy(graph);
        ctx->graphs_enabled = false;
        return vision_forward_launch(ctx, d_imgs, B, d_out, normalize);
    }
    e->graph = graph;
    e->exec = exec;
    e->split = captured_split;
    return hipGraphLaunch(exec, ctx->stream) == hipSuccess;
}

bool vision_stage_begin(clip_ctx * ctx, int Bc, VisionStage & st) {
    const auto & hp = ctx->vision_hparams;
    const DevTower & V = ctx->vision;
    const int S = hp.image_size, P = hp.patch_size, G = S / P, Np = G * G, T = Np + 1;
    const int h = hp.hidden_size, ff = hp.n_intermediate, proj = hp.projection_dim;
    const int rows = Bc * T;
    st.Bc = Bc;
    st.st_stride = (rows + 63) & ~63;
    auto carve = [&](Carver & c) {
        st.stats = c.take<float2>((size_t)(h / 16) * st.st_stride);
        st.mu = c.take<float>((size_t)2 * st.st_stride);
        st.x = c.take<float>((size_t)rows * h);
        const size_t aw = acts_f32(ctx, V) ? 2 : 1;
        st.xn = c.take<half_t>(aw * rows * h);
        st.qkv = c.take<half_t>(aw * rows * 3 * h);
        st.att = c.take<half_t>(aw * rows * h);
        st.mid = c.take<half_t>(aw * rows * ff);
        st.col = c.take<half_t>((size_t)Bc * Np * V.patch.Kpad);
        st.pooled = c.take<half_t>(aw * Bc * h);
        st.emb = c.take<float>((size_t)Bc * proj);
        st.xp = c.take<float>((size_t)Bc * h);
        st.ap = c.take<half_t>(aw * Bc * h);
        st.xnp = c.take<half_t>(aw * Bc * h);
        st.midp = c.take<half_t>(aw * Bc * ff);
    };
    Carver sizer(nullptr);
    carve(sizer);
    if (!ensure_workspace(ctx, sizer.off + 4096)) return false;
    Carver c(ctx->ws.base, &ctx->guard_gaps);
    carve(c);
    return guard_arm(ctx);
}

bool vision_stage_patch(clip_ctx * ctx, const VisionStage & st, const void * imgs, int i0, int n) {
    const bool piece = n < st.Bc;
    const auto & hp = ctx->vision_hparams;
    const DevTower & V = ctx->vision;
    const int S = hp.image_size, P = hp.patch_size, G = S / P, Np = G * G, T = Np + 1, h = hp.hidden_size;
    hipStream_t s = ctx->stream;
    half_t * col = st.col + (size_t)i0 * Np * V.patch.Kpad;
    float * x = st.x + (size_t)i0 * T * h;
    {
        ProfScope ps(ctx, "im2col", n * Np, V.patch.Kpad, 0, 0, (double)n * S * S * 3 * (ctx->input_f16 ? 2 : 4) + (double)n * Np * V.patch.Kpad * 2);
        launch_im2col(imgs, ctx->input_f16, col, n, S, P, V.patch.Kpad, s);
    }
    GemmParams pp;
    pp.A = col; pp.lda = V.patch.Kpad; pp.M = n * Np; pp.W = V.patch; pp.out = x; pp.ldc = h;
    pp.Np = Np; pp.T = T; pp.pos = V.pos; pp.no_splitk = piece;
    gemm(ctx, "gemm_patch", pp, EPI_PATCH_F32);
    return true;
}

bool vision_stage_finish(clip_ctx * ctx, const VisionStage & st, float * d_out, bool normalize) {
    const auto & hp = ctx->vision_hparams;
    const DevTower & V = ctx->vision;
    const int S = hp.image_size, P = hp.patch_size, G = S / P, Np = G * G, T = Np + 1;
    const int h = hp.hidden_size, ff = hp.n_intermediate, nh = hp.n_head, proj = hp.projection_dim;
    hipStream_t s = ctx->stream;
    const int Bc = st.Bc, rows = Bc * T;
    float * x = st.x;
    const bool skinny = layers_fit_skinny(V, rows, h, ff);
    const bool fold = ctx->ln_fold && !V.layers.empty() && (ctx->ln_fold_force || fold_pays(V, rows, device_shared(ctx)));
    {
        ProfScope ps(ctx, "layernorm", rows, h, 0, 0, (double)rows * h * (fold ? 10 : 8));
        if (fold)
            launch_layernorm_prep(x, h, V.pre_ln_w, V.pre_ln_b, hp.eps, rows, h, x, h, V.layers[0].ln1_w, st.xn, h, st.stats, s, ctx->ln_fold_centre ? st.mu : nullptr,
                                  V.class_embd, V.pos, T);
        else {
            launch_cls_rows(x, V.class_embd, V.pos, Bc, T, h, s);
            launch_layernorm(x, h, nullptr, 1, V.pre_ln_w, V.pre_ln_b, hp.eps, rows, h, nullptr, 0, x, h, s);
        }
    }
    const bool prune = ctx->prune_last && !skinny && !V.layers.empty() && T > 1;
    if (skinny && fold) {
        if (!run_layers_skinny_fold(ctx, V, rows, h, nh, ff, hp.eps, Bc, T, nullptr, T, false, x, st.xn, st.qkv, st.att, st.mid, st.stats, st.st_stride, ctx->ln_fold_centre ? st.mu : nullptr)) return false;
    } else if (skinny) {
        launch_row_stats(x, h, rows, h, ctx->sk_stats, s);
        if (!run_layers_skinny(ctx, V, rows, h, nh, ff, hp.eps, Bc, T, nullptr, T, false, x, st.qkv, st.att, st.mid)) return false;
    } else if (fold) {
        if (!run_layers_fold(ctx, V, rows, h, nh, ff, hp.eps, Bc, T, nullptr, T, false, x, st.xn, st.qkv, st.att, st.mid, st.stats, st.st_stride, ctx->ln_fold_centre ? st.mu : nullptr, prune, resident_panels(ctx, V, 0, rows))) return false;
    } else if (!run_layers(ctx, V, rows, h, nh, ff, hp.eps, Bc, T, nullptr, T, false, x, st.xn, st.qkv, st.att, st.mid, prune, resident_panels(ctx, V, 0, rows))) return false;
    const bool f32 = acts_f32(ctx, V);
    if (prune) {
        if (!pooled_tail(ctx, V.layers.back(), Bc, h, ff, hp.eps, x, st.att, nullptr, T, st.xp, st.ap, st.xnp, st.midp)) return false;
        layernorm_act(f32, st.xp, h, nullptr, 1, V.post_ln_w, V.post_ln_b, hp.eps, Bc, h, st.pooled, s);
    } else {
        layernorm_act(f32, x, h, nullptr, T, V.post_ln_w, V.post_ln_b, hp.eps, Bc, h, st.pooled, s);
    }
    GemmParams pj;
    pj.A = st.pooled; pj.lda = h; pj.M = Bc; pj.W = V.proj; pj.out = st.emb; pj.ldc = proj; pj.act_f32 = f32;
    gemm(ctx, "gemm_proj", pj, EPI_F32);
    launch_l2norm(st.emb, d_out, Bc, proj, normalize, s);
    return launch_ok("clip_image_batch_encode") && guard_check(ctx, "clip_image_batch_encode");
}

int vision_max_chunk(const clip_ctx * ctx) {
    const auto & hp = ctx->vision_hparams;
    const int S = hp.image_size, P = hp.patch_size, G = S / P, Np = G * G, T = Np + 1;
    const int h = hp.hidden_size, ff = hp.n_intermediate;
    const size_t aw = acts_f32(ctx, ctx->vision) ? 2 : 1;
    const size_t per_img = (size_t)T * ((size_t)h * 4 + aw * ((size_t)h * 2 * 2 + (size_t)3 * h * 2 + (size_t)ff * 2)) + (size_t)Np * ctx->vision.patch.Kpad * 2;
    return (int)std::min<size_t>(1024, std::max<size_t>(1, ((size_t)6 << 30) / per_img));
}

static bool vision_forward_one(clip_ctx * ctx, const float * d_imgs, int B, float * d_out, bool normalize) {
    if (!ctx->has_vision_encoder) {
        printf("This gguf file seems to have no vision encoder\n");
        return false;
    }
    if (B <= 0) return true;
    const int S = ctx->vision_hparams.image_size, proj = ctx->vision_hparams.projection_dim;
    const int chunk = std::min(B, vision_max_chunk(ctx));
    for (int b0 = 0; b0 < B; b0 += chunk) {
        const int Bc = std::min(chunk, B - b0);
        VisionStage st;
        if (!vision_stage_begin(ctx, Bc, st)) return false;
        const void * imgs = ctx->input_f16 ? (const void *)((const half_t *)d_imgs + (size_t)b0 * S * S * 3) : (const void *)(d_imgs + (size_t)b0 * S * S * 3);
        if (!vision_stage_patch(ctx, st, imgs, 0, Bc)) return false;
        if (!vision_stage_finish(ctx, st, d_out + (size_t)b0 * proj, normalize)) return false;
    }
    return true;
}

bool text_forward_device(clip_ctx * ctx, const int32_t * d_ids, const int32_t * h_offsets, int n_texts, float * d_out,
                         bool normalize) {
    if (!check_device(ctx, "clip_text_encode")) return false;
    if (!ctx->has_text_encoder) {
        printf("This GGUF file seems to have no text encoder\n");
        return false;
    }
    if (n_texts <= 0) return true;
    const auto & hp = ctx->text_hparams;
    const DevTower & Tw = ctx->text;
    const int h = hp.hidden_size, ff = hp.n_intermediate, nh = hp.n_head, proj = hp.projection_dim;
    hipStream_t s = ctx->stream;
    const int rows = h_offsets[n_texts] - h_offsets[0];
    int max_len = 0;
    for (int i = 0; i < n_texts; i++) {
        const int len = h_offsets[i + 1] - h_offsets[i];
        if (len <= 0 || len > hp.num_positions) {
            fprintf(stderr, "clip_text_encode: %d tokens is outside [1, %d]\n", len, hp.num_positions);
            return false;
        }
        max_len = std::max(max_len, len);
    }
    const int st_stride = (rows + 63) & ~63;
    float2 * stats = nullptr;
    float * mu = nullptr;
    float * xp = nullptr;
    half_t * ap = nullptr, * xnp = nullptr, * midp = nullptr;
    auto carve = [&](Carver & c, float *& x, half_t *& xn, half_t *& qkv, half_t *& att, half_t *& mid, half_t *& pooled,
                     float *& emb, int *& seq, int *& last) {
        stats = c.take<float2>((size_t)(h / 16) * st_stride);
        mu = c.take<float>((size_t)2 * st_stride);
        x = c.take<float>((size_t)rows * h);
        const size_t aw = acts_f32(ctx, Tw) ? 2 : 1;
        xn = c.take<half_t>(aw * rows * h);
        qkv = c.take<half_t>(aw * rows * 3 * h);
        att = c.take<half_t>(aw * rows * h);
        mid = c.take<half_t>(aw * rows * ff);
        pooled = c.take<half_t>(aw * n_texts * h);
        emb = c.take<float>((size_t)n_texts * proj);
        seq = c.take<int>((size_t)n_texts + 1);
        last = c.take<int>((size_t)n_texts);
        xp = c.take<float>((size_t)n_texts * h);
        ap = c.take<half_t>(aw * n_texts * h);
        xnp = c.take<half_t>(aw * n_texts * h);
        midp = c.take<half_t>(aw * n_texts * ff);
    };
    float *x, *emb;
    half_t *xn, *qkv, *att, *mid, *pooled;
    int *seq, *last;
    Carver sizer(nullptr);
    carve(sizer, x, xn, qkv, att, mid, pooled, emb, seq, last);
    if (!ensure_workspace(ctx, sizer.off + 4096)) return false;
    Carver c(ctx->ws.base, &ctx->guard_gaps);
    carve(c, x, xn, qkv, att, mid, pooled, emb, seq, last);
    if (!guard_arm(ctx)) return false;
    {
        MetaRing & mr = ctx->meta;
        const int sl = mr.next;
        mr.next = (mr.next + 1) % MetaRing::SLOTS;
        const size_t n_ints = 2 * (size_t)n_texts + 1;
        if (!mr.done) {
            unsigned * d = nullptr;
            if (hipHostMalloc((void **)&d, MetaRing::SLOTS * sizeof(unsigned), hipHostMallocMapped) == hipSuccess) {
                memset(d, 0, MetaRing::SLOTS * sizeof(unsigned));
                if (hipHostGetDevicePointer((void **)&mr.done_dev, d, 0) == hipSuccess) mr.done = d;
                else { (void)hipGetLastError(); (void)hipHostFree(d); }
            } else (void)hipGetLastError();
        }
        if (mr.done && mr.expect[sl]) {
            for (unsigned spins = 0; mr.done[sl] != mr.expect[sl]; spins++) {
                if (spins > 64) std::this_thread::yield();
                if (spins > 20000) {
                    const hipError_t qe = hipStreamSynchronize(s);
                    if (qe != hipSuccess || mr.done[sl] != mr.expect[sl]) {
                        fprintf(stderr, "clip_text_encode: the metadata upload of an earlier call never completed (%s)\n", hipGetErrorString(qe));
                        (void)hipGetLastError();
                        mr.expect[sl] = 0;
                        if (qe != hipSuccess) return false;
                    }
                    break;
                }
            }
        } else if (mr.busy[sl]) {
            (void)hipEventSynchronize(mr.ev[sl]);
        }
        if (mr.cap[sl] < n_ints) {
            if (mr.pin[sl]) (void)hipHostFree(mr.pin[sl]);
            mr.pin[sl] = nullptr;
            mr.dev[sl] = nullptr;
            mr.cap[sl] = 0;
            const size_t want = std::max<size_t>(n_ints, 1024);
            if (hipHostMalloc((void **)&mr.pin[sl], want * sizeof(int), hipHostMallocMapped) != hipSuccess) { (void)hipGetLastError(); return false; }
            if (hipHostGetDevicePointer((void **)&mr.dev[sl], mr.pin[sl], 0) != hipSuccess) { (void)hipGetLastError(); mr.dev[sl] = nullptr; }
            mr.cap[sl] = want;
        }
        int * hs = mr.pin[sl];
        for (int i = 0; i <= n_texts; i++) hs[i] = h_offsets[i] - h_offsets[0];
        for (int i = 0; i < n_texts; i++) hs[n_texts + 1 + i] = hs[i + 1] - 1;
        if (mr.done && mr.dev[sl]) {
            if (++mr.stamp == 0) mr.stamp = 1;
            mr.expect[sl] = mr.stamp;
            mr.busy[sl] = false;
            launch_meta_upload(mr.dev[sl], seq, last, n_texts, mr.done_dev + sl, mr.stamp, s);
            if (hipGetLastError() != hipSuccess) {
                mr.expect[sl] = 0;
                fprintf(stderr, "clip_text_encode: metadata upload launch failed\n");
                return false;
            }
        } else {
            if (!mr.ev[sl] && hipEventCreateWithFlags(&mr.ev[sl], hipEventDisableTiming) != hipSuccess) return false;
            (void)hipMemcpyAsync(seq, hs, ((size_t)n_texts + 1) * 4, hipMemcpyHostToDevice, s);
            (void)hipMemcpyAsync(last, hs + n_texts + 1, (size_t)n_texts * 4, hipMemcpyHostToDevice, s);
            (void)hipEventRecord(mr.ev[sl], s);
            mr.expect[sl] = 0;
            mr.busy[sl] = true;
        }
    }
    auto launch_all = [&]() -> bool {
        const bool skinny = layers_fit_skinny(Tw, rows, h, ff);
        const bool fold = ctx->ln_fold && !Tw.layers.empty() && (ctx->ln_fold_force || fold_pays(Tw, rows, device_shared(ctx)));
        const bool prune = ctx->prune_last && !skinny && !Tw.layers.empty() && rows > n_texts;
        if (fold)
            launch_text_embed(d_ids + h_offsets[0], seq, n_texts, rows, Tw.tok_raw, Tw.tok_type, Tw.pos, h, x, s, Tw.layers[0].ln1_w, xn, h, stats, ctx->ln_fold_centre ? mu : nullptr);
        else launch_text_embed(d_ids + h_offsets[0], seq, n_texts, rows, Tw.tok_raw, Tw.tok_type, Tw.pos, h, x, s);
        if (skinny && fold) {
            if (!run_layers_skinny_fold(ctx, Tw, rows, h, nh, ff, hp.eps, n_texts, 0, seq, max_len, true, x, xn, qkv, att, mid, stats, st_stride, ctx->ln_fold_centre ? mu : nullptr)) return false;
        } else if (skinny) {
            launch_row_stats(x, h, rows, h, ctx->sk_stats, s);
            if (!run_layers_skinny(ctx, Tw, rows, h, nh, ff, hp.eps, n_texts, 0, seq, max_len, true, x, qkv, att, mid)) return false;
        } else if (fold) {
            if (!run_layers_fold(ctx, Tw, rows, h, nh, ff, hp.eps, n_texts, 0, seq, max_len, true, x, xn, qkv, att, mid, stats, st_stride, ctx->ln_fold_centre ? mu : nullptr, prune, resident_panels(ctx, Tw, 1, rows))) return false;
        } else if (!run_layers(ctx, Tw, rows, h, nh, ff, hp.eps, n_texts, 0, seq, max_len, true, x, xn, qkv, att, mid, prune, resident_panels(ctx, Tw, 1, rows))) return false;
        if (prune) {
            if (!pooled_tail(ctx, Tw.layers.back(), n_texts, h, ff, hp.eps, x, att, last, 1, xp, ap, xnp, midp)) return false;
            layernorm_act(acts_f32(ctx, Tw), xp, h, nullptr, 1, Tw.post_ln_w, Tw.post_ln_b, hp.eps, n_texts, h, pooled, s);
        } else {
            layernorm_act(acts_f32(ctx, Tw), x, h, last, 1, Tw.post_ln_w, Tw.post_ln_b, hp.eps, n_texts, h, pooled, s);
        }
        GemmParams pj;
        pj.A = pooled; pj.lda = h; pj.M = n_texts; pj.W = Tw.proj; pj.out = emb; pj.ldc = proj; pj.act_f32 = acts_f32(ctx, Tw);
        gemm(ctx, "gemm_proj", pj, EPI_F32);
        launch_l2norm(emb, d_out, n_texts, proj, normalize, s);
        return true;
    };
    const int nt_bucket = (max_len + 15) / 16;
    if (ctx->graphs_enabled && !ctx->profiling && rows <= 1024 && !guard_mode()) {
        clip_ctx::TextGraphEntry * e = nullptr;
        const void * ids_key = d_ids + h_offsets[0];
        for (auto & g : ctx->tgraphs)
            if (g.n_texts == n_texts && g.rows == rows && g.nt == nt_bucket && g.ids == ids_key && g.out == d_out && g.norm == normalize) { e = &g; break; }
        if (e && e->exec) return hipGraphLaunch(e->exec, s) == hipSuccess;
        if (!e) {
            if (ctx->tgraphs.size() >= 96) drop_graphs(ctx);
            ctx->tgraphs.push_back({n_texts, rows, nt_bucket, ids_key, d_out, normalize, 1, nullptr, nullptr});
        } else if (hipStreamBeginCapture(s, hipStreamCaptureModeThreadLocal) == hipSuccess) {
            break_capture_for_test();
            const bool ok = launch_all();
            hipGraph_t graph = nullptr;
            const hipError_t ce = hipStreamEndCapture(s, &graph);
            hipGraphExec_t exec = nullptr;
            if (ok && ce == hipSuccess && graph && hipGraphInstantiate(&exec, graph, nullptr, nullptr, 0) == hipSuccess) {
                e->graph = graph;
                e->exec = exec;
                return hipGraphLaunch(exec, s) == hipSuccess;
            }
            (void)hipGetLastError();
            if (graph) (void)hipGraphDestroy(graph);
            ctx->graphs_enabled = false;
            if (!renew_streams_after_failed_capture(ctx)) { fprintf(stderr, "clip_text_encode: the caller's stream is left in an invalidated capture\n"); return false; }
            s = ctx->stream;
        } else {
            (void)hipGetLastError();
        }
    }
    if (!launch_all()) return false;
    return launch_ok("clip_text_encode") && guard_check(ctx, "clip_text_encode");
}

}

#ifdef CLIPAMD_SK_TIMING
extern "C" int clip_amd_debug_read_sk_stamps(unsigned long long * out, int cap_launches) {
    using namespace clipamd;
    (void)hipDeviceSynchronize();
    const int n = g_sk_stamp_launch < cap_launches ? g_sk_stamp_launch : cap_launches;
    if (g_sk_stamps && n > 0) (void)hipMemcpy(out, g_sk_stamps, (size_t)n * 16 * 8, hipMemcpyDeviceToHost);
    g_sk_stamp_launch = 0;
    return n;
}
#endif
```

clip_cpp_amd/csrc/k_misc.hip:

```cpp

#include "kernels.h"

namespace clipamd {

typedef _Float16 h2 __attribute__((ext_vector_type(2)));
typedef float f4 __attribute__((ext_vector_type(4)));

namespace {

__device__ __forceinline__ float wave_sum(float v) {
#pragma unroll
    for (int o = 32; o > 0; o >>= 1) v += __shfl_xor(v, o);
    return v;
}

template <int LN_MAXV, int RW>
__global__ void __launch_bounds__(256) layernorm_kernel(const float * __restrict__ x, int ldx, const int * __restrict__ in_rows, int in_row_mul,
                                                        const float * __restrict__ w, const float * __restrict__ b, float eps,
                                                        int rows, int h, half_t * __restrict__ out16, int ld16,
                                                        float * __restrict__ out32, int ld32) {
    const int lane = threadIdx.x & 63;
    const int r0 = (blockIdx.x * 4 + (threadIdx.x >> 6)) * RW;
    if (r0 >= rows) return;
    f4 v[RW][LN_MAXV];
// ... 223 lines not shown
        const uint32_t qh = blk[4] | (blk[5] << 8) | (blk[6] << 16) | ((uint32_t)blk[7] << 24);
        const uint8_t q = blk[8 + (j & 15)];
        const int lo = j < 16 ? (q & 0x0F) : (q >> 4);
        const int hi = (qh >> j) & 1;
        return (float)(lo | (hi << 4)) * ld_h(blk) + ld_h(blk + 2);
    }
    case 8: {
        const uint8_t * blk = row + ib * 34;
        return (float)(int8_t)blk[2 + j] * ld_h(blk);
    }
    }
    return 0.f;
}

__device__ __forceinline__ f4 dequant4(const uint8_t * row, int type, int k) {
    const int ib = k >> 5, j = k & 31;
    f4 o;
    switch (type) {
    case 0: return *(const f4 *)((const float *)row + k);
    case 1: {
#pragma unroll
        for (int e = 0; e < 4; e++) o[e] = ld_h(row + 2 * (k + e));
        return o;
    }
    case 2: {
        const uint8_t * blk = row + ib * 18;
        const float d = ld_h(blk);
#pragma unroll
        for (int e = 0; e < 4; e++) {
            const uint8_t q = blk[2 + ((j + e) & 15)];
            o[e] = (float)((j < 16 ? (q & 0x0F) : (q >> 4)) - 8) * d;
        }
        return o;
    }
    case 3: {
        const uint8_t * blk = row + ib * 20;
        const float d = ld_h(blk), m = ld_h(blk + 2);
#pragma unroll
        for (int e = 0; e < 4; e++) {
            const uint8_t q = blk[4 + ((j + e) & 15)];
            o[e] = (float)(j < 16 ? (q & 0x0F) : (q >> 4)) * d + m;
        }
        return o;
    }
    case 6: {
        const uint8_t * blk = row + ib * 22;
        const float d = ld_h(blk);
        const uint32_t qh = blk[2] | (blk[3] << 8) | (blk[4] << 16) | ((uint32_t)blk[5] << 24);
#pragma unroll
        for (int e = 0; e < 4; e++) {
            const uint8_t q = blk[6 + ((j + e) & 15)];
            const int lo = j < 16 ? (q & 0x0F) : (q >> 4);
            o[e] = (float)((lo | (int)(((qh >> (j + e)) & 1u) << 4)) - 16) * d;
        }
        return o;
    }
    case 7: {
        const uint8_t * blk = row + ib * 24;
        const float d = ld_h(blk), m = ld_h(blk + 2);
        const uint32_t qh = blk[4] | (blk[5] << 8) | (blk[6] << 16) | ((uint32_t)blk[7] << 24);
#pragma unroll
        for (int e = 0; e < 4; e++) {
            const uint8_t q = blk[8 + ((j + e) & 15)];
            const int lo = j < 16 ? (q & 0x0F) : (q >> 4);
            o[e] = (float)(lo | (int)(((qh >> (j + e)) & 1u) << 4)) * d + m;
        }
        return o;
    }
    case 8: {
        const uint8_t * blk = row + ib * 34;
        const float d = ld_h(blk);
#pragma unroll
        for (int e = 0; e < 4; e++) o[e] = (float)(int8_t)blk[2 + j + e] * d;
        return o;
    }
    }
    return (f4){0.f, 0.f, 0.f, 0.f};
}

template <int NV>
__global__ void __launch_bounds__(256) text_embed_kernel(const int32_t * __restrict__ ids, const int * __restrict__ seq_start, int nseq, int rows,
                                                         const uint8_t * __restrict__ tok, int tok_type, size_t tok_row_bytes,
                                                         const float * __restrict__ pos, int h, float * __restrict__ x,
                                                         const float * __restrict__ gnext, half_t * __restrict__ xg, int ldxg,
                                                         float2 * __restrict__ stats, float * __restrict__ mu_out) {
    const int lane = threadIdx.x & 63;
    const int row = blockIdx.x * 4 + (threadIdx.x >> 6);
    if (row >= rows) return;
    const int id = ids[row];
    int lo = 0, hi = nseq, start = seq_start[0];
    while (hi - lo > 1) {
        const int step = (hi - lo + 63) >> 6;
        const int idx = lo + (lane + 1) * step;
        const int val = idx < hi ? seq_start[idx] : 0x7fffffff;
        const int cnt = __popcll(__ballot(val <= row));
        if (cnt > 0) start = __shfl(val, cnt - 1, 64);
        const int nlo = lo + cnt * step;
        hi = min(hi, nlo + step);
        lo = nlo;
    }
    const int t = row - start;
    const uint8_t * trow = tok + (size_t)id * tok_row_bytes;
    f4 v[NV];
#pragma unroll
    for (int i = 0; i < NV; i++) {
        const int c = (i * 64 + lane) * 4;
        if (c < h) {
            const f4 pe = *(const f4 *)(pos + (size_t)t * h + c);
            v[i] = pe + dequant4(trow, tok_type, c);
            *(f4 *)(x + (size_t)row * h + c) = v[i];
        } else {
            v[i] = (f4){0.f, 0.f, 0.f, 0.f};
        }
    }
    if (gnext) row_fold_prep<NV>(v, h, lane, gnext, xg + (size_t)row * ldxg, stats + row, mu_out ? mu_out + row : nullptr);
}

__global__ void __launch_bounds__(256, 4) l2norm_kernel(const float * __restrict__ v, float * __restrict__ out, int rows, int n,
                                                     int normalize) {
    const int lane = threadIdx.x & 63;
    const int r = blockIdx.x * 4 + (threadIdx.x >> 6);
    if (r >= rows) return;
    const float * vr = v + (size_t)r * n;
    float sq = 0.f;
    for (int c = lane; c < n; c += 64) sq += vr[c] * vr[c];
    sq = wave_sum(sq);
    const float inv = normalize ? 1.0f / sqrtf(sq) : 1.0f;
    for (int c = lane; c < n; c += 64) out[(size_t)r * n + c] = vr[c] * inv;
}

__global__ void __launch_bounds__(256) f32_to_f16_kernel(const float * __restrict__ src, int lds, half_t * __restrict__ dst, int ldd,
                                                         int rows, int cols, int cols_pad) {
    const long i = (long)blockIdx.x * 256 + threadIdx.x;
    if (i >= (long)rows * cols_pad) return;
    const int r = (int)(i / cols_pad), c = (int)(i % cols_pad);
    dst[(size_t)r * ldd + c] = c < cols ? (_Float16)src[(size_t)r * lds + c] : (_Float16)0.f;
}
__global__ void __launch_bounds__(256) f16_to_f32_kernel(const half_t * __restrict__ src, int lds, float * __restrict__ dst, int ldd,
                                                         int rows, int cols) {
    const long i = (long)blockIdx.x * 256 + threadIdx.x;
    if (i >= (long)rows * cols) return;
    const int r = (int)(i / cols), c = (int)(i % cols);
    dst[(size_t)r * ldd + c] = (float)src[(size_t)r * lds + c];
}

}

void launch_layernorm(const float * x, int ldx, const int * in_rows, int in_row_mul, const float * w, const float * b, float eps,
                      int rows, int h, half_t * out16, int ld16, float * out32, int ld32, hipStream_t stream) {
    if (rows <= 0) return;
    const dim3 block(256);
    const bool two = rows >= 4096;
    const dim3 grid(two ? (rows + 7) / 8 : (rows + 3) / 4);
#define CLIPAMD_LN(NV)                                                                                                               \
    if (two) hipLaunchKernelGGL((layernorm_kernel<NV, 2>), grid, block, 0, stream, x, ldx, in_rows, in_row_mul, w, b, eps, rows, h, out16, ld16, out32, ld32); \
    else hipLaunchKernelGGL((layernorm_kernel<NV, 1>), grid, block, 0, stream, x, ldx, in_rows, in_row_mul, w, b, eps, rows, h, out16, ld16, out32, ld32)
    if (h <= 256) { CLIPAMD_LN(1); }
    else if (h <= 512) { CLIPAMD_LN(2); }
    else if (h <= 768) { CLIPAMD_LN(3); }
    else if (h <= 1024) { CLIPAMD_LN(4); }
    else if (h <= 1280) { CLIPAMD_LN(5); }
    else { CLIPAMD_LN(8); }
#undef CLIPAMD_LN
}

template <typename IT>
static void launch_im2col_t(const IT * imgs, half_t * col, int B, int S, int P, int Kpad, hipStream_t stream) {
    const int G = S / P;
    const long total2 = (long)B * G * G * (Kpad / 2);
    if (total2 <= 0) return;
    if (P % 2 == 0 && Kpad == 3 * P * P && S % 2 == 0) {
        const long total = (long)B * G * G * P * (P / 2);
        hipLaunchKernelGGL(im2col_rows_kernel<IT>, dim3((unsigned)((total + 255) / 256)), dim3(256), 0, stream, imgs, col, S, P, Kpad, total);
        return;
    }
    hipLaunchKernelGGL(im2col_kernel<IT>, dim3((unsigned)((total2 + 255) / 256)), dim3(256), 0, stream, imgs, col, B, S, P, Kpad, total2);
}

void launch_im2col(const void * imgs, bool imgs_f16, half_t * col, int B, int S, int P, int Kpad, hipStream_t stream) {
    if (imgs_f16) launch_im2col_t<half_t>((const half_t *)imgs, col, B, S, P, Kpad, stream);
    else launch_im2col_t<float>((const float *)imgs, col, B, S, P, Kpad, stream);
}

void launch_cls_rows(float * x, const float * class_embd, const float * pos, int B, int T, int h, hipStream_t stream) {
    if (B <= 0) return;
    hipLaunchKernelGGL(cls_rows_kernel, dim3((B * h + 255) / 256), dim3(256), 0, stream, x, class_embd, pos, B, T, h);
}


__global__ void __launch_bounds__(256) zero_shot_kernel(const float * img, const float * txt, int n, int dim, int npad, float * scores, int * indices) {
    extern __shared__ __attribute__((aligned(16))) unsigned char zs_smem[];
    float * key = (float *)zs_smem;
    int * idx = (int *)(key + npad);
    float * iv = (float *)(idx + npad);
    __shared__ double red[256];
    const int b = blockIdx.x, tid = threadIdx.x;
    for (int i = tid; i < dim; i += 256) iv[i] = img[(size_t)b * dim + i];
    __syncthreads();
    double part = 0.0;
    for (int j = tid; j < npad; j += 256) {
        float e = -1.0f;
        if (j < n) {
            const float * t = txt + (size_t)j * dim;
            float dot = 0.0f;
            for (int i = 0; i < dim; i++) dot += iv[i] * t[i];
            e = (float)(exp((double)dot) + 1e-9);
            part += (double)e;
        }
        key[j] = e;
        idx[j] = j;
    }
    red[tid] = part;
    __syncthreads();
    for (int s = 128; s > 0; s >>= 1) {
        if (tid < s) red[tid] += red[tid + s];
        __syncthreads();
    }
    const double sum = red[0];
    for (int j = tid; j < n; j += 256) key[j] = (float)((double)key[j] / sum);
    __syncthreads();
    for (int k = 2; k <= npad; k <<= 1) {
        for (int j = k >> 1; j > 0; j >>= 1) {
            for (int i = tid; i < npad; i += 256) {
                const int l = i ^ j;
                if (l > i) {
                    const float ka = key[i], kb = key[l];
                    const int ia = idx[i], ib = idx[l];
                    const bool a_first = ka > kb || (ka == kb && ia < ib);
                    const bool up = (i & k) == 0;
                    if (up ? !a_first : a_first) { key[i] = kb; key[l] = ka; idx[i] = ib; idx[l] = ia; }
                }
            }
            __syncthreads();
        }
    }
    for (int j = tid; j < n; j += 256) {
        scores[(size_t)b * n + j] = key[j];
        indices[(size_t)b * n + j] = idx[j];
    }
}

static size_t raw_row_bytes(int type, int k) {
    switch (type) {
    case 0: return (size_t)k * 4;
    case 1: return (size_t)k * 2;
    case 2: return (size_t)(k / 32) * 18;
    case 3: return (size_t)(k / 32) * 20;
    case 6: return (size_t)(k / 32) * 22;
    case 7: return (size_t)(k / 32) * 24;
    case 8: return (size_t)(k / 32) * 34;
    }
    return 0;
}

void launch_text_embed(const int32_t * ids, const int * seq_start, int nseq, int rows, const void * tok_raw, int tok_type,
                       const float * pos, int h, float * x, hipStream_t stream, const float * gamma_next, half_t * xg, int ldxg, float2 * stats, float * mu_out) {
    if (rows <= 0) return;
    const dim3 grid((rows + 3) / 4), block(256);
#define CLIPAMD_TE(NV)                                                                                                              \
    hipLaunchKernelGGL((text_embed_kernel<NV>), grid, block, 0, stream, ids, seq_start, nseq, rows, (const uint8_t *)tok_raw, tok_type, \
                       raw_row_bytes(tok_type, h), pos, h, x, gamma_next, xg, ldxg, stats, mu_out)
    if (h <= 256) { CLIPAMD_TE(1); }
    else if (h <= 512) { CLIPAMD_TE(2); }
    else if (h <= 768) { CLIPAMD_TE(3); }
    else if (h <= 1024) { CLIPAMD_TE(4); }
    else if (h <= 1280) { CLIPAMD_TE(5); }
    else { CLIPAMD_TE(8); }
#undef CLIPAMD_TE
}

void launch_layernorm_prep(const float * x, int ldx, const float * w, const float * b, float eps, int rows, int h, float * out32, int ld32,
                           const float * gamma_next, half_t * xg, int ldxg, float2 * stats, hipStream_t stream, float * mu_out,
                           const float * class_embd, const float * pos0, int T) {
    if (rows <= 0) return;
    const dim3 grid((rows + 3) / 4), block(256);
#define CLIPAMD_LNP(NV)                                                                                                             \
    hipLaunchKernelGGL((layernorm_prep_kernel<NV>), grid, block, 0, stream, x, ldx, w, b, eps, rows, h, out32, ld32, gamma_next, xg, ldxg, stats, mu_out, class_embd, pos0, T > 0 ? T : 1)
    if (h <= 256) { CLIPAMD_LNP(1); }
    else if (h <= 512) { CLIPAMD_LNP(2); }
    else if (h <= 768) { CLIPAMD_LNP(3); }
    else if (h <= 1024) { CLIPAMD_LNP(4); }
    else if (h <= 1280) { CLIPAMD_LNP(5); }
    else { CLIPAMD_LNP(8); }
#undef CLIPAMD_LNP
}

namespace {
__global__ void __launch_bounds__(256) gather_rows_kernel(const float * __restrict__ x, const half_t * __restrict__ a, const int * __restrict__ in_rows,
                                                          int in_row_mul, int rows, int h, float * __restrict__ xp, half_t * __restrict__ ap) {
    const int r = blockIdx.x;
    const long src = in_rows ? (long)in_rows[r] : (long)r * in_row_mul;
    for (int c = threadIdx.x * 4; c < h; c += 256 * 4) {
        *(f4 *)(xp + (size_t)r * h + c) = *(const f4 *)(x + (size_t)src * h + c);
        if (a) *(uint2 *)(ap + (size_t)r * h + c) = *(const uint2 *)(a + (size_t)src * h + c);
    }
}
}
void launch_gather_rows(const float * x, const half_t * a, const int * in_rows, int in_row_mul, int rows, int h, float * xp, half_t * ap, hipStream_t stream) {
    if (rows <= 0) return;
    hipLaunchKernelGGL(gather_rows_kernel, dim3(rows), dim3(256), 0, stream, x, a, in_rows, in_row_mul, rows, h, xp, ap);
}

namespace {
__global__ void __launch_bounds__(256) meta_upload_kernel(const int * __restrict__ src, int * __restrict__ seq, int * __restrict__ last, int n_texts,
                                                          unsigned * done, unsigned stamp) {
    for (int i = threadIdx.x; i < 2 * n_texts + 1; i += 256) {
        const int v = src[i];
        if (i <= n_texts) seq[i] = v; else last[i - n_texts - 1] = v;
    }
    __syncthreads();
    if (threadIdx.x == 0) __hip_atomic_store(done, stamp, __ATOMIC_RELEASE, __HIP_MEMORY_SCOPE_SYSTEM);
}
}
void launch_meta_upload(const int * src_mapped, int * seq, int * last, int n_texts, unsigned * done_mapped, unsigned stamp, hipStream_t stream) {
    hipLaunchKernelGGL(meta_upload_kernel, dim3(1), dim3(256), 0, stream, src_mapped, seq, last, n_texts, done_mapped, stamp);
}

void launch_l2norm(const float * v, float * out, int rows, int n, bool normalize, hipStream_t stream) {
    if (rows <= 0) return;
    hipLaunchKernelGGL(l2norm_kernel, dim3((rows + 3) / 4), dim3(256), 0, stream, v, out, rows, n, normalize ? 1 : 0);
}

bool launch_zero_shot(const float * img, int B, const float * txt, int n, int dim, float * scores, int * indices, hipStream_t stream) {
    if (B <= 0 || n <= 0) return true;
    int npad = 1;
    while (npad < n) npad <<= 1;
    if (npad > 8192) return false;
    const size_t smem = (size_t)npad * 8 + (size_t)dim * 4;
    static unsigned long long lds_ok = 0;
    opt_in_dynamic_lds(zero_shot_kernel, 8192 * 8 + 4096 * 4, lds_ok);
    if (dim > 4096) return false;
    hipLaunchKernelGGL(zero_shot_kernel, dim3(B), dim3(256), smem, stream, img, txt, n, dim, npad, scores, indices);
    return true;
}

void launch_f32_to_f16(const float * src, int lds, half_t * dst, int ldd, int rows, int cols, int cols_pad,
                       hipStream_t stream) {
    const long total = (long)rows * cols_pad;
    if (total <= 0) return;
    hipLaunchKernelGGL(f32_to_f16_kernel, dim3((unsigned)((total + 255) / 256)), dim3(256), 0, stream, src, lds, dst, ldd, rows,
                       cols, cols_pad);
}
void launch_f16_to_f32(const half_t * src, int lds, float * dst, int ldd, int rows, int cols, hipStream_t stream) {
    const long total = (long)rows * cols;
    if (total <= 0) return;
    hipLaunchKernelGGL(f16_to_f32_kernel, dim3((unsigned)((total + 255) / 256)), dim3(256), 0, stream, src, lds, dst, ldd, rows,
                       cols);
}

}
```

clip_cpp_amd/csrc/kernels.h:

```cpp
#pragma once

#include <hip/hip_runtime.h>
#include <cstdint>
#include <cstdio>

namespace clipamd {

typedef _Float16 half_t;

template <typename K>
inline void opt_in_dynamic_lds(K kernel, size_t bytes, unsigned long long & done) {
    int dev = 0;
    (void)hipGetDevice(&dev);
    const unsigned long long bit = 1ull << (dev & 63);
    if (done & bit) return;
    const hipError_t e = hipFuncSetAttribute((const void *)kernel, hipFuncAttributeMaxDynamicSharedMemorySize, (int)bytes);
    if (e != hipSuccess) {
        fprintf(stderr, "clip (hip): hipFuncSetAttribute(MaxDynamicSharedMemorySize = %zu) failed: %s\n", bytes, hipGetErrorString(e));
        (void)hipGetLastError();
        return;
    }
    done |= bit;
}

enum WType : int { W_F16 = 0, W_Q4_0 = 1, W_Q4_1 = 2, W_Q5_0 = 3, W_Q5_1 = 4, W_Q8_0 = 5, W_F32 = 6 };

struct DevWeight {
    int wtype = W_F16;
    int N = 0, K = 0;
    int Npad = 0;
    int Kpad = 0;
    const void * qs = nullptr;
    const void * qh = nullptr;
    const void * dm = nullptr;
    const void * w16 = nullptr;
};

enum Epilogue : int {
    EPI_F32 = 0,
    EPI_F16 = 1,
    EPI_GELU_F16 = 2,
    EPI_QGELU_F16 = 3,
    EPI_RESID_F32 = 4,
    EPI_PATCH_F32 = 5,
    EPI_COUNT = 6
};

struct GemmParams {
    const half_t * A = nullptr;
    int lda = 0;
    int M = 0;
    DevWeight W;
    const float * bias = nullptr;
    void * out = nullptr;
    int ldc = 0;
    const float * resid = nullptr;
    float qscale = 1.0f;
    int qcols = 0;
    int Np = 0, T = 0;
    const float * pos = nullptr;
    float * sk_ws = nullptr;
    size_t sk_ws_floats = 0;
    unsigned * sk_cnt = nullptr;
    int sk_cnt_n = 0;
    int ksplit = 1;
    bool no_splitk = false;
    const half_t * w16_pre = nullptr;
    half_t * w16_scratch = nullptr;
    size_t w16_scratch_halfs = 0;
    int debug = 0;
    const float * ln_c = nullptr;
    const float2 * ln_stats = nullptr;
    int ln_slots = 0, ln_slotw = 0;
    int ln_stride = 0;
    float ln_eps = 0.f;
    half_t * xg_out = nullptr;
    int ldxg = 0;
    const float * xg_gamma = nullptr;
    float2 * stats_out = nullptr;
    int stats_stride = 0;
    const float * xg_mu = nullptr;
    const float * ln_mu = nullptr;
    float * mu_out = nullptr;
    bool shared_device = false;
    bool act_f32 = false;
};

void launch_gemm(const GemmParams & p, int epilogue, int tile, hipStream_t stream);
int gemm_tile_for(int M, int N, int Kpad, bool quantised, bool shared_device = false);
inline bool gemm_tile_is_ring(int tile) { return (tile % 1000000) / 1000 == 65; }
inline bool gemm_tile_uses_panel(int tile) { const int bn = tile % 1000; return !gemm_tile_is_ring(tile) && (bn == 256 || (bn >= 258 && bn <= 261)); }

void launch_gemm_ring(const GemmParams & p, int epilogue, int bn, hipStream_t stream);

void launch_gemm8(const GemmParams & p, int epilogue, int tm, hipStream_t stream);
void launch_gemm_f32(const GemmParams & p, int epilogue, hipStream_t stream);
void launch_gemm4(const GemmParams & p, int epilogue, hipStream_t stream);
bool gemm32_supported(const GemmParams & p, int epilogue);
void launch_gemm32(const GemmParams & p, int epilogue, int form, hipStream_t stream);
struct DequantJobs { DevWeight W[4]; half_t * out[4]; int blk_end[4]; int n = 0; };
void launch_dequant(const DevWeight * const * ws, half_t * const * outs, int n, hipStream_t stream);

int gemm_fold_slotw(int tile);
int gemm_fold_slotw_for(int M, int N, int Kpad, bool quantised, bool shared_device = false);
void launch_fold_vectors(const DevWeight & W, const float * gamma, const float * beta, const float * bias, float * c_out, float * b_out,
                         hipStream_t stream);

struct SkinnyParams {
    const half_t * A16 = nullptr;
    int lda = 0;
    const float * x32 = nullptr;
    int ldx = 0;
    const float * ln_w = nullptr, * ln_b = nullptr;
    float eps = 0.f;
    const float2 * stats_in = nullptr;
    int stats_slots = 0;
    int M = 0;
    DevWeight W;
    const float * bias = nullptr;
    void * out = nullptr;
    int ldc = 0;
    const float * resid = nullptr;
    float qscale = 1.0f;
    int qcols = 0;
    int Np = 0, T = 0;
    const float * pos = nullptr;
    float2 * stats_out = nullptr;
    int stats_cap = 128;
    const float * ln_c = nullptr;
    const float2 * fstats = nullptr;
    int fslots = 0, fslotw = 0, fstride = 0;
    half_t * xg_out = nullptr;
    int ldxg = 0;
    const float * xg_gamma = nullptr;
    float2 * fstats_out = nullptr;
    int fstride_out = 0;
    const float * xg_mu = nullptr, * ln_mu = nullptr;
    float * mu_out = nullptr;
    unsigned long long * stamps = nullptr;
};
constexpr int SKINNY_MAX_ROWS = 512;
bool skinny_supported(const SkinnyParams & p, int epilogue);
void launch_skinny(const SkinnyParams & p, int epilogue, hipStream_t stream);
void launch_row_stats(const float * x, int ldx, int rows, int h, float2 * stats, hipStream_t stream);

void launch_layernorm(const float * x, int ldx, const int * in_rows, int in_row_mul, const float * w, const float * b, float eps,
                      int rows, int h, half_t * out16, int ld16, float * out32, int ld32, hipStream_t stream);
void launch_layernorm_prep(const float * x, int ldx, const float * w, const float * b, float eps, int rows, int h, float * out32, int ld32,
                           const float * gamma_next, half_t * xg, int ldxg, float2 * stats, hipStream_t stream, float * mu_out = nullptr,
                           const float * class_embd = nullptr, const float * pos0 = nullptr, int T = 0);

bool launch_attention(const half_t * qkv, half_t * out, int nseq, int T_uniform, const int * seq_start, int max_len,
                      int h, int n_head, bool causal, hipStream_t stream);
int attention_whole_row_max_len(int d_head);
bool launch_attention_whole_row(const half_t * qkv, half_t * out, int nseq, int T_uniform, const int * seq_start, int max_len,
                                int h, int n_head, bool causal, hipStream_t stream);
bool launch_attention_long(const half_t * qkv, half_t * out, int nseq, int T_uniform, const int * seq_start, int max_len,
                           int h, int n_head, bool causal, hipStream_t stream);

bool launch_attention_f32(const float * qkv, float * out, int nseq, int T_uniform, const int * seq_start, int max_len,
                          int h, int n_head, bool causal, hipStream_t stream);

void launch_im2col(const void * imgs, bool imgs_f16, half_t * col, int B, int S, int P, int Kpad, hipStream_t stream);

void launch_gather_rows(const float * x, const half_t * a, const int * in_rows, int in_row_mul, int rows, int h, float * xp, half_t * ap, hipStream_t stream);

void launch_cls_rows(float * x, const float * class_embd, const float * pos, int B, int T, int h, hipStream_t stream);

void launch_meta_upload(const int * src_mapped, int * seq, int * last, int n_texts, unsigned * done_mapped, unsigned stamp, hipStream_t stream);
void launch_text_embed(const int32_t * ids, const int * seq_start, int nseq, int rows, const void * tok_raw,
                       int tok_type, const float * pos, int h, float * x, hipStream_t stream,
                       const float * gamma_next = nullptr, half_t * xg = nullptr, int ldxg = 0, float2 * stats = nullptr, float * mu_out = nullptr);

void launch_l2norm(const float * v, float * out, int rows, int n, bool normalize, hipStream_t stream);

struct PreImg {
    long long src_off;
    int nx, ny;
    int x0, y0;
    int ylo, nrows;
    long long hbuf_off;
    int th, tv;
};
struct PreTaps { long long w_off; int first_off, count_off, ksize; };
void launch_preprocess(const uint8_t * raw, const PreImg * imgs, const PreTaps * taps, const double * wpool, const int * ipool, float * hbuf,
                       float * out, int n_imgs, int S, int max_rows, const float * mean, const float * stdv, hipStream_t stream);

bool launch_zero_shot(const float * img, int B, const float * txt, int n, int dim, float * scores, int * indices, hipStream_t stream);

void launch_f32_to_f16(const float * src, int lds, half_t * dst, int ldd, int rows, int cols, int cols_pad,
                       hipStream_t stream);
void launch_f16_to_f32(const half_t * src, int lds, float * dst, int ldd, int rows, int cols, hipStream_t stream);

enum { SEARCH_F32 = 0, SEARCH_F16 = 1, SEARCH_I8 = 3 };
int search_candidate_capacity(int k);
int search_sort_size(int k);
void launch_search_normalize(const float * src, int64_t n_src, int64_t n_rows, int dim, int Dpad, void * dst, int dtype, hipStream_t stream);
void launch_search_quantize(const float * src, int64_t n_src, int64_t n_rows, int dim, int Dpad, void * dst, float * inv, hipStream_t stream);
void launch_search_row_inv(const void * rows, int64_t n, int Dpad, float * inv, hipStream_t stream);
bool launch_search_scan(const void * rows, const float * rinv, int64_t n, int Dpad, int dtype, const void * q, const float * qinv, int nq, int qt,
                        int k, void * cand, int n_chunks, int64_t rows_per_chunk, hipStream_t stream);
void launch_search_merge(const void * in, int64_t in_stride, int n_in, void * out, int nq, int k, hipStream_t stream);
void launch_search_finish(const void * in, int64_t in_stride, int nq, int k, float * dist, int64_t * ids, hipStream_t stream);
void launch_search_fill_random(float * x, int64_t n, uint64_t seed, hipStream_t stream);

constexpr int JOIN_HIT_BYTES = 12;
bool launch_join(const void * rows, const float * rinv, int64_t n, const void * q, const float * qinv, int64_t nq, int Dpad, int dtype, bool pairs,
                 float radius, int * count, unsigned long long * total, void * hits, int64_t hit_cap, hipStream_t stream);
void launch_join_scatter(const void * hits, int64_t total, const int64_t * offs, int * cursor, void * out, hipStream_t stream);
void * launch_join_sort(void * buf, void * tmp, const int64_t * offs, int64_t nseg, int64_t total, int64_t longest, hipStream_t stream);
void launch_join_finish(const void * in, int64_t total, float * dist, int64_t * ids, hipStream_t stream);
void launch_join_plant(float * x, int64_t rows, int dim, uint64_t seed, hipStream_t stream);

}
```

clip_cpp_amd/csrc/model.h:

```cpp
#pragma once

#include <functional>
#include <map>
#include <string>
#include <unordered_map>
#include <vector>

#include "../../include/clip.h"
#include "gguf.h"
#include "kernels.h"

namespace clipamd {

struct DevLayer {
    DevWeight qkv, o, ff1, ff2;
    const float *qkv_b = nullptr, *o_b = nullptr, *ff1_b = nullptr, *ff2_b = nullptr;
    const float *ln1_w = nullptr, *ln1_b = nullptr, *ln2_w = nullptr, *ln2_b = nullptr;
    const float *qkv_c = nullptr, *qkv_bf = nullptr, *ff1_c = nullptr, *ff1_bf = nullptr;
};

struct DevTower {
    std::vector<DevLayer> layers;
    const float * pos = nullptr;
    const float *post_ln_w = nullptr, *post_ln_b = nullptr;
    DevWeight proj;
    DevWeight patch;
    const float * class_embd = nullptr;
    const float *pre_ln_w = nullptr, *pre_ln_b = nullptr;
    const void * tok_raw = nullptr;
    int tok_type = 0;
};

struct ProfEntry {
    double ms = 0;
    int64_t launches = 0;
    double flops = 0;
    double bytes = 0;
};

struct Workspace {
    void * base = nullptr;
    size_t bytes = 0;
};

struct HostPipe {
    hipStream_t copy_stream = nullptr;
    void * pin_in[2] = {nullptr, nullptr};
    size_t pin_in_bytes[2] = {0, 0};
    void * dev_in[2] = {nullptr, nullptr};
    size_t dev_in_bytes[2] = {0, 0};
    hipEvent_t ev_copied[2] = {nullptr, nullptr};
    hipEvent_t ev_consumed[2] = {nullptr, nullptr};
    hipEvent_t ev_sub = nullptr;
    bool used[2] = {false, false};
    struct PackPool * pool = nullptr;
};

struct MetaRing {
    static constexpr int SLOTS = 8;
    int * pin[SLOTS] = {nullptr};
    int * dev[SLOTS] = {nullptr};
    size_t cap[SLOTS] = {0};
    hipEvent_t ev[SLOTS] = {nullptr};
    bool busy[SLOTS] = {false};
    int next = 0;
    volatile unsigned * done = nullptr;
    unsigned * done_dev = nullptr;
    unsigned expect[SLOTS] = {0};
    unsigned stamp = 0;
};

}

struct clip_ctx {
    bool has_text_encoder = false;
    bool has_vision_encoder = false;
    bool use_gelu = false;
    int32_t ftype = 1;
    clip_text_hparams text_hparams{};
    clip_vision_hparams vision_hparams{};
    float image_mean[3] = {0, 0, 0};
    float image_std[3] = {1, 1, 1};

    std::vector<std::string> id_to_token;
    std::unordered_map<std::string, int32_t> token_to_id;
    size_t max_token_len = 0;

    int device = -1;
    hipStream_t own_stream = nullptr;
    hipStream_t stream = nullptr;
    void * weights_base = nullptr;
    size_t weights_bytes = 0;
    bool weights_from_cache = false;
    clipamd::DevTower vision, text;
    clipamd::Workspace ws;
    std::vector<size_t> guard_gaps;
    void * pinned = nullptr;
    size_t pinned_bytes = 0;
    void * io_in = nullptr;
    size_t io_in_bytes = 0;
    void * io_out = nullptr;
    size_t io_out_bytes = 0;
    bool input_f16 = false;
    clipamd::HostPipe pipe;
    clipamd::MetaRing meta;
    void * multi = nullptr;
    clip_ctx * sibling = nullptr;
    clip_ctx * more_siblings[2] = {nullptr, nullptr};
    hipEvent_t ev_join_more[2] = {nullptr, nullptr};
    int split_ways = 2;
    bool weights_borrowed = false;
    clip_ctx * owner = nullptr;
    bool last_launch_split = false;
    bool f32_acts = true;
    bool device_shared = false;
    bool sibling_busy = false;
    hipEvent_t ev_fork = nullptr, ev_join = nullptr;
    int split_min = -1, split_max = -1;
    hipEvent_t ev_stream_switch = nullptr;
    void * pre_buf = nullptr;
    size_t pre_bytes = 0;
    struct PreSlot { void * pin = nullptr; size_t pin_bytes = 0; void * dev = nullptr; size_t dev_bytes = 0; hipEvent_t ev_h2d = nullptr, ev_done = nullptr; bool used = false; };
    static constexpr int PRE_SLOTS = 4;
    PreSlot pre_slot[PRE_SLOTS];
    hipStream_t pre_copy_stream = nullptr;
    float * sk_ws = nullptr;
    size_t sk_ws_floats = 0;
    unsigned * sk_cnt = nullptr;
    int sk_cnt_n = 0;
    float2 * sk_stats = nullptr;
    bool ln_fold_force = false;
    bool prune_last = true;
    bool ln_fold_centre = true;
    bool ln_fold = true;
    clipamd::half_t * w16_panel = nullptr;
    size_t w16_panel_halfs = 0;
    clipamd::half_t * res_panel_buf[2] = {nullptr, nullptr};
    std::vector<const clipamd::half_t *> res_panels[2];
    unsigned res_panel_mask[2] = {0, 0};
    bool resident_panels_on = true;

    bool profiling = false;
    struct PendingEvent { hipEvent_t a, b; std::string tag; double flops, bytes; };
    std::vector<PendingEvent> pending;
    std::map<std::string, clipamd::ProfEntry> prof;

    struct GraphEntry { int B; const void * in; void * out; bool norm; bool in_f16; int seen; hipGraph_t graph; hipGraphExec_t exec; bool split; bool busy_seen; };
    std::vector<GraphEntry> vgraphs;
    struct TextGraphEntry { int n_texts, rows, nt; const void * ids; void * out; bool norm; int seen; hipGraph_t graph; hipGraphExec_t exec; };
    std::vector<TextGraphEntry> tgraphs;
    bool graphs_enabled = true;

    int verbosity = 0;
    std::string path;
};

namespace clipamd {

struct RelaxCapture {
    hipStreamCaptureMode prev = hipStreamCaptureModeRelaxed;
    bool armed = false;
    RelaxCapture() {
        static const bool off = [] { const char * e = getenv("CLIP_AMD_NO_RELAX_CAPTURE"); return e && e[0] == '1'; }();
        if (off) return;
        armed = hipThreadExchangeStreamCaptureMode(&prev) == hipSuccess;
        if (!armed) (void)hipGetLastError();
    }
    ~RelaxCapture() { if (armed) (void)hipThreadExchangeStreamCaptureMode(&prev); }
    RelaxCapture(const RelaxCapture &) = delete;
    RelaxCapture & operator=(const RelaxCapture &) = delete;
};

clip_ctx * load_model(const char * fname, int verbosity, int device);
clip_ctx * sibling_context(clip_ctx * owner, int index = 0);
void free_model(clip_ctx * ctx);
bool repack_for_test(int type, const void * w_raw, int64_t N, int64_t K, DevWeight & W, void ** dev_base);

bool vision_forward_device(clip_ctx * ctx, const float * d_imgs, int B, float * d_out, bool normalize);
bool text_forward_device(clip_ctx * ctx, const int32_t * d_ids, const int32_t * h_offsets, int n_texts, float * d_out,
                         bool normalize);
struct VisionStage {
    int Bc = 0, st_stride = 0;
    float * x = nullptr, * emb = nullptr;
    half_t * xn = nullptr, * qkv = nullptr, * att = nullptr, * mid = nullptr, * col = nullptr, * pooled = nullptr;
    float2 * stats = nullptr;
    float * mu = nullptr;
    float * xp = nullptr;
    half_t * ap = nullptr, * xnp = nullptr, * midp = nullptr;
};
bool vision_stage_begin(clip_ctx * ctx, int Bc, VisionStage & st);
bool vision_stage_patch(clip_ctx * ctx, const VisionStage & st, const void * imgs, int i0, int n);
bool vision_stage_finish(clip_ctx * ctx, const VisionStage & st, float * d_out, bool normalize);
int vision_max_chunk(const clip_ctx * ctx);
bool ensure_workspace(clip_ctx * ctx, size_t bytes);
bool ensure_pinned(clip_ctx * ctx, size_t bytes);
bool ensure_io(clip_ctx * ctx, size_t in_bytes, size_t out_bytes);
void prof_collect(clip_ctx * ctx);
void drop_graphs(clip_ctx * ctx);
bool renew_streams_after_failed_capture(clip_ctx * ctx);

bool encode_images_from_host(clip_ctx * ctx, const clip_image_f32 * imgs, int n, float * d_out, bool normalize, int n_threads);
void free_host_pipe(clip_ctx * ctx);
void multi_shard(int total, int n_dev, int g, int * lo, int * hi, int * per_dev);
clip_ctx * multi_load(const char * fname, int verbosity, int n_devices);
void multi_free(clip_ctx * primary);
int multi_device_count(const clip_ctx * primary);
bool multi_image_batch_encode(clip_ctx * primary, const clip_image_f32 * imgs, int B, float * vec, bool normalize, int n_threads);
bool multi_run(clip_ctx * primary, int total, int proj, float * vec, const char * who,
               const std::function<bool(int, clip_ctx *, int, int, float *)> & run);
bool multi_run_pair(clip_ctx * primary, int n_img, int n_txt, int proj, float * vec_img, float * vec_txt, const char * who,
                    const std::function<bool(int, clip_ctx *, int, int, float *)> & run_img,
                    const std::function<bool(int, clip_ctx *, int, int, float *)> & run_txt);
clip_ctx * multi_replica(const clip_ctx * primary, int g);
const float * multi_gathered(const clip_ctx * primary, int g);

bool tokenize_text(const clip_ctx * ctx, const char * text, std::vector<int32_t> & out);
bool preprocess_image(const clip_ctx * ctx, const clip_image_u8 * img, clip_image_f32 * res);
bool preprocess_batch_device(clip_ctx * ctx, const clip_image_u8 * imgs, int n, float * d_out, int slot = -1);
void free_preprocess_slots(clip_ctx * ctx);
bool load_image_file(const char * fname, clip_image_u8 * img);

void dequantize_row(int type, const void * src, float * dst, int64_t k);
size_t quantize_rows(int type, const float * src, void * dst, int64_t nrows, int64_t k);
uint16_t f32_to_f16_bits(float x);
float f16_bits_to_f32(uint16_t h);

}
```

include/clip_amd.h:

```cpp
#ifndef CLIP_AMD_H
#define CLIP_AMD_H

#include "clip.h"

#ifdef __cplusplus
extern "C" {
#endif

int clip_amd_device_count(void);

struct clip_ctx * clip_amd_model_load(const char * fname, int verbosity, int device);

struct clip_ctx * clip_amd_model_load_multi(const char * fname, int verbosity, int n_devices);
int clip_amd_ctx_device_count(const struct clip_ctx * ctx);

int clip_amd_weights_from_cache(const struct clip_ctx * ctx);
void clip_amd_shard_bounds(int total, int n_devices, int device_index, int * lo, int * hi, int * rows_per_device);
const float * clip_amd_gathered_embeddings(const struct clip_ctx * ctx, int device_index);

bool clip_amd_image_batch_encode_device_multi(struct clip_ctx * ctx, const float * const * d_imgs, int total, bool normalize, float * vec);
bool clip_amd_text_batch_encode_device_multi(struct clip_ctx * ctx, const int32_t * const * d_ids, const int32_t * h_offsets, int total, bool normalize,
                                             float * vec);
bool clip_amd_encode_pair_device_multi(struct clip_ctx * ctx, const float * const * d_imgs, int n_images, const int32_t * const * d_ids,
                                       const int32_t * h_offsets, int n_texts, bool normalize, float * vec_img, float * vec_txt);

int clip_amd_ctx_device(const struct clip_ctx * ctx);

void clip_amd_set_stream(struct clip_ctx * ctx, void * hip_stream);

void clip_amd_set_device_shared(struct clip_ctx * ctx, int shared);

bool clip_amd_image_batch_encode_device(struct clip_ctx * ctx, const float * d_imgs, int batch, float * d_out,
                                        bool normalize);

bool clip_amd_image_batch_preprocess_device(struct clip_ctx * ctx, const struct clip_image_u8 * imgs, int n, float * d_out);

bool clip_amd_image_batch_encode_u8(struct clip_ctx * ctx, const struct clip_image_u8 * imgs, int n, float * vec, bool normalize);

bool clip_text_batch_encode(const struct clip_ctx * ctx, const int n_threads, const struct clip_tokens * tokens,
                            size_t n_texts, float * vec, const bool normalize);

bool clip_amd_text_batch_encode_device(struct clip_ctx * ctx, const int32_t * d_ids, const int32_t * h_offsets,
                                       int n_texts, float * d_out, bool normalize);

bool clip_amd_zero_shot_score_device(struct clip_ctx * ctx, const float * d_img, int n_images, const float * d_txt, int n_labels, int dim,
                                     float * d_scores, int * d_indices);

bool clip_amd_zero_shot_label_images(struct clip_ctx * ctx, const struct clip_image_u8 * imgs, int n_images, const char ** labels,
                                     size_t n_labels, float * scores, int * indices);

void clip_amd_synchronize(struct clip_ctx * ctx);

void clip_amd_profile_enable(struct clip_ctx * ctx, bool on);
int clip_amd_profile_read(struct clip_ctx * ctx, float * ms, int64_t * launches, int cap, bool reset);
int clip_amd_profile_report(struct clip_ctx * ctx, char * buf, int cap, bool reset);

struct clip_amd_index;
struct clip_amd_index * clip_amd_index_create(struct clip_ctx * ctx, int dim, int dtype);
bool clip_amd_index_add(struct clip_amd_index * ix, const float * vecs, int64_t n);
bool clip_amd_index_add_device(struct clip_amd_index * ix, const float * d_vecs, int64_t n);
int64_t clip_amd_index_size(const struct clip_amd_index * ix);
int clip_amd_index_dim(const struct clip_amd_index * ix);
bool clip_amd_index_search(struct clip_amd_index * ix, const float * queries, int n_queries, int k, float * distances, int64_t * ids);
bool clip_amd_index_search_device(struct clip_amd_index * ix, const float * d_queries, int n_queries, int k, float * d_distances,
                                  int64_t * d_ids);
bool clip_amd_index_save(struct clip_amd_index * ix, const char * path);
struct clip_amd_index * clip_amd_index_load(struct clip_ctx * ctx, const char * path);
void clip_amd_index_free(struct clip_amd_index * ix);
float clip_amd_bench_search(int dtype, int64_t n, int dim, int n_queries, int k, int iters);
int64_t clip_amd_index_range_search(struct clip_amd_index * ix, const float * queries, int n_queries, float radius,
                                    int64_t * lims, float * distances, int64_t * ids, int64_t capacity);
int64_t clip_amd_index_pairs(struct clip_amd_index * ix, float radius, int64_t * lims, float * distances, int64_t * ids, int64_t capacity);
float clip_amd_bench_range(int dtype, int64_t n, int dim, int n_queries, float radius, int iters);

int clip_amd_test_gemm(int type, const void * w_raw, int64_t N, int64_t K, const float * x, int64_t M,
                       const float * bias, const float * resid, float * y, int epilogue, int tile);
int clip_amd_test_gemm_ex(int type, const void * w_raw, int64_t N, int64_t K, const float * x, int64_t M,
                          const float * bias, const float * resid, float * y, int epilogue, int tile,
                          int qcols, float qscale, int Np, int T, const float * pos);
int clip_amd_test_lnfold(int type, const void * w1_raw, int64_t h, int64_t K1, const void * w2_raw, int64_t N2, const float * a, int64_t M,
                         const float * b1, const float * resid, const float * gamma, const float * beta, float eps, const float * b2,
                         int epi2, int tile1, int tile2, int fold, int qcols, float qscale, float * x1_out, float * y_out);
int clip_amd_test_gemm_tile(int64_t M, int64_t N, int64_t K, int quantised);
int clip_amd_test_gemm_tile_ex(int64_t M, int64_t N, int64_t K, int quantised, int shared_device);
float clip_amd_bench_gemm(int type, int64_t N, int64_t K, int64_t M, int epilogue, int tile, int iters);
int clip_amd_test_skinny(int type, const void * w_raw, int64_t N, int64_t K, const float * x, int64_t M, const float * bias,
                         const float * resid, const float * ln_w, const float * ln_b, float eps, float * y, int epilogue,
                         int qcols, float qscale, float * stats_out);
int clip_amd_test_layernorm(const float * x, const float * w, const float * b, float eps, int64_t rows, int64_t h,
                            float * y, int out_f16);
int clip_amd_test_attention(const float * qkv, int nseq, int T, int h, int n_head, int causal, float * out);
int clip_amd_test_attention_ex(const float * qkv, int nseq, int T, int h, int n_head, int causal, float * out, int kernel);
float clip_amd_bench_attention(int nseq, int T, int h, int n_head, int causal, int kernel, int iters);

#ifdef __cplusplus
}
#endif

#endif
```

Baseline: 122,500.

## Compute only pooled-row queries and attention in the last encoder layer

In the last transformer layer, when pruning to the pooled token is enabled, the QKV GEMM now produces only the K and V columns for all rows. Q is computed only for the pooled rows through a fused gather+layernorm kernel and a small GEMM, and a new pooled-attention kernel handles a single query per sequence. This removes the full Q projection and the T×T attention of the last layer, which only feed the pooled output. The cost is extra kernels, new code paths with per-head-dim template limits, and some extra buffer carving.

Result: no change. 123,200, median of 6 (+0.5%).

```diff
diff --git a/clip_cpp_amd/__init__.py b/clip_cpp_amd/__init__.py
--- a/clip_cpp_amd/__init__.py
+++ b/clip_cpp_amd/__init__.py
@@ -57,7 +57,7 @@
     "clip_amd_zero_shot_score_device", "clip_amd_zero_shot_label_images",
     "clip_amd_synchronize", "clip_amd_profile_enable", "clip_amd_profile_read", "clip_amd_profile_report",
     "clip_amd_test_gemm", "clip_amd_test_gemm_ex", "clip_amd_test_gemm_tile", "clip_amd_test_gemm_tile_ex", "clip_amd_test_skinny", "clip_amd_test_layernorm", "clip_amd_test_attention", "clip_amd_bench_gemm",
-    "clip_amd_test_attention_ex", "clip_amd_bench_attention",
+    "clip_amd_test_attention_ex", "clip_amd_bench_attention", "clip_amd_test_attention_pooled", "clip_amd_test_gemm_rows",
     "clip_amd_index_create", "clip_amd_index_add", "clip_amd_index_add_device", "clip_amd_index_size", "clip_amd_index_dim",
     "clip_amd_index_search", "clip_amd_index_search_device", "clip_amd_index_save", "clip_amd_index_load", "clip_amd_index_free",
     "clip_amd_bench_search", "clip_amd_index_range_search", "clip_amd_index_pairs", "clip_amd_bench_range",
@@ -176,6 +176,10 @@
     L.clip_amd_test_layernorm.argtypes = [f32p, f32p, f32p, C.c_float, C.c_int64, C.c_int64, f32p, i32]
     L.clip_amd_test_attention.restype = i32
     L.clip_amd_test_attention.argtypes = [f32p, i32, i32, i32, i32, i32, f32p]
+    L.clip_amd_test_attention_pooled.restype = i32
+    L.clip_amd_test_attention_pooled.argtypes = [f32p, f32p, i32, i32, C.POINTER(i32), i32, i32, i32, C.POINTER(i32), f32p, f32p]
+    L.clip_amd_test_gemm_rows.restype = i32
+    L.clip_amd_test_gemm_rows.argtypes = [i32, vp, C.c_int64, C.c_int64, f32p, C.c_int64, f32p, f32p, i32, C.c_int64, C.c_int64, i32, C.c_float]
     L.clip_amd_test_attention_ex.restype = i32
     L.clip_amd_test_attention_ex.argtypes = [f32p, i32, i32, i32, i32, i32, f32p, i32]
     L.clip_amd_bench_attention.restype = C.c_float
diff --git a/clip_cpp_amd/build.py b/clip_cpp_amd/build.py
--- a/clip_cpp_amd/build.py
+++ b/clip_cpp_amd/build.py
@@ -13,9 +13,9 @@
 
 HOST_SOURCES = ["gguf.cpp", "quant.cpp", "load.cpp", "forward.cpp", "tokenizer.cpp", "preprocess.cpp", "image_io.cpp", "image_formats.cpp",
                 "jpeg_decode.cpp", "host_pipeline.cpp", "api.cpp", "search.cpp"]
-HIP_SOURCES = ["k_attn.hip", "k_attn_long.hip", "k_attn_f32.hip", "k_misc.hip", "k_preproc.hip", "k_gemm.hip", "k_gemm8.hip", "k_gemm4.hip", "k_gemm32.hip", "k_gemm_f32.hip", "k_skinny.hip", "k_gemm_ring.hip", "k_fold.hip", "k_search.hip", "k_join.hip"]
+HIP_SOURCES = ["k_attn.hip", "k_attn_long.hip", "k_attn_f32.hip", "k_attn_pooled.hip", "k_misc.hip", "k_preproc.hip", "k_gemm.hip", "k_gemm8.hip", "k_gemm4.hip", "k_gemm32.hip", "k_gemm_f32.hip", "k_skinny.hip", "k_gemm_ring.hip", "k_fold.hip", "k_search.hip", "k_join.hip"]
 GEMM_WTYPES = [0, 1, 2, 3, 4, 5]
-EXTRA_FLAGS = {"k_attn_f32.hip": ["-fno-slp-vectorize"], "k_attn_long.hip": ["-fno-slp-vectorize"], "k_gemm_f32.hip": ["-fno-slp-vectorize"]}
+EXTRA_FLAGS = {"k_attn_f32.hip": ["-fno-slp-vectorize"], "k_attn_long.hip": ["-fno-slp-vectorize"], "k_attn_pooled.hip": ["-fno-slp-vectorize"], "k_gemm_f32.hip": ["-fno-slp-vectorize"]}
 
 COMMON = ["-O3", "-std=c++17", "-fPIC", "-ffp-contract=off", "-Wall", "-Wno-unused-function", "-Wno-unused-result", "-Wno-inline-asm", "-Wno-bitwise-instead-of-logical",
           "-I" + os.path.join(os.path.dirname(HERE), "include")]
diff --git a/clip_cpp_amd/csrc/api.cpp b/clip_cpp_amd/csrc/api.cpp
--- a/clip_cpp_amd/csrc/api.cpp
+++ b/clip_cpp_amd/csrc/api.cpp
@@ -1009,6 +1009,85 @@
     return clip_amd_test_attention_ex(qkv, nseq, T, h, n_head, causal, out, 0);
 }
 
+int clip_amd_test_attention_pooled(const float * qkv, const float * qp, int nseq, int T, const int * seq_start, int h, int n_head, int causal,
+                                   const int * rows_in, float * out, float * full_rows) {
+    int ndev = 0;
+    if (hipGetDeviceCount(&ndev) != hipSuccess || ndev <= 0) { (void)hipGetLastError(); return -1; }
+    if (nseq <= 0 || h <= 0 || n_head <= 0 || h % n_head || (!seq_start && T <= 0)) return -3;
+    int max_len = T;
+    size_t rows = (size_t)nseq * (size_t)(T > 0 ? T : 0);
+    if (seq_start) {
+        max_len = 0;
+        for (int i = 0; i < nseq; i++) {
+            if (seq_start[i + 1] <= seq_start[i]) return -3;
+            max_len = std::max(max_len, seq_start[i + 1] - seq_start[i]);
+        }
+        if (seq_start[0] != 0) return -3;
+        rows = (size_t)seq_start[nseq];
+    }
+    DBuf d32(rows * 3 * h * 4), d16(rows * 3 * h * 2), q32((size_t)nseq * h * 4), q16((size_t)nseq * h * 2), o16((size_t)nseq * h * 2), o32((size_t)nseq * h * 4),
+        dseq(((size_t)nseq + 1) * 4), a16(full_rows ? rows * h * 2 : 16), a32(full_rows ? rows * h * 4 : 16);
+    (void)hipMemcpy(d32.p, qkv, rows * 3 * h * 4, hipMemcpyHostToDevice);
+    (void)hipMemcpy(q32.p, qp, (size_t)nseq * h * 4, hipMemcpyHostToDevice);
+    if (seq_start) (void)hipMemcpy(dseq.p, seq_start, ((size_t)nseq + 1) * 4, hipMemcpyHostToDevice);
+    const int * d_seq = seq_start ? (const int *)dseq.p : nullptr;
+    launch_f32_to_f16((const float *)d32.p, 3 * h, (half_t *)d16.p, 3 * h, (int)rows, 3 * h, 3 * h, nullptr);
+    launch_f32_to_f16((const float *)q32.p, h, (half_t *)q16.p, h, nseq, h, h, nullptr);
+    if (!launch_attention_pooled((const half_t *)d16.p, (const half_t *)q16.p, (half_t *)o16.p, nseq, seq_start ? 0 : T, d_seq, h, n_head, nullptr)) return -2;
+    launch_f16_to_f32((const half_t *)o16.p, h, (float *)o32.p, h, nseq, h, nullptr);
+    if (full_rows) {
+        if (!rows_in) return -3;
+        if (!launch_attention((const half_t *)d16.p, (half_t *)a16.p, nseq, seq_start ? 0 : T, d_seq, max_len, h, n_head, causal != 0, nullptr)) return -2;
+        launch_f16_to_f32((const half_t *)a16.p, h, (float *)a32.p, h, (int)rows, h, nullptr);
+    }
+    if (hipDeviceSynchronize() != hipSuccess || hipGetLastError() != hipSuccess) return -4;
+    (void)hipMemcpy(out, o32.p, (size_t)nseq * h * 4, hipMemcpyDeviceToHost);
+    if (full_rows)
+        for (int i = 0; i < nseq; i++) {
+            if (rows_in[i] < 0 || (size_t)rows_in[i] >= rows) return -3;
+            (void)hipMemcpy(full_rows + (size_t)i * h, (const float *)a32.p + (size_t)rows_in[i] * h, (size_t)h * 4, hipMemcpyDeviceToHost);
+        }
+    return 0;
+}
+
+int clip_amd_test_gemm_rows(int type, const void * w_raw, int64_t N, int64_t K, const float * x, int64_t M, const float * bias, float * y, int tile,
+                            int64_t n0, int64_t n, int qcols, float qscale) {
+    int ndev = 0;
+    if (hipGetDeviceCount(&ndev) != hipSuccess || ndev <= 0) { (void)hipGetLastError(); return -1; }
+    if (n0 < 0 || n <= 0 || n0 + n > N || n0 % 128 || (n0 > 0 && n % 128)) return -3;
+    DevWeight W;
+    void * wbase = nullptr;
+    if (!repack_for_test(type, w_raw, N, K, W, &wbase)) return -2;
+    const int Kpad = W.Kpad;
+    DBuf dx32((size_t)M * K * 4), dx16((size_t)(M + 1) * Kpad * 2), dbias((size_t)N * 4), dout((size_t)M * N * 2), dout32((size_t)M * N * 4);
+    hipStream_t s = nullptr;
+    (void)hipMemcpy(dx32.p, x, (size_t)M * K * 4, hipMemcpyHostToDevice);
+    if (bias) (void)hipMemcpy(dbias.p, bias, (size_t)N * 4, hipMemcpyHostToDevice);
+    (void)hipMemset(dout.p, 0, (size_t)M * N * 2);
+    launch_f32_to_f16((const float *)dx32.p, (int)K, (half_t *)dx16.p, Kpad, (int)M, (int)K, Kpad, s);
+    GemmParams p;
+    p.A = (const half_t *)dx16.p; p.lda = Kpad; p.M = (int)M; p.W = weight_rows(W, (int)n0, (int)n); p.bias = bias ? (const float *)dbias.p + n0 : nullptr;
+    p.out = (half_t *)dout.p + n0; p.ldc = (int)N; p.qscale = qscale; p.qcols = qcols;
+    DBuf skw((size_t)64 << 20), skc(4096 * 4);
+    (void)hipMemset(skc.p, 0, 4096 * 4);
+    p.sk_ws = (float *)skw.p; p.sk_ws_floats = (size_t)16 << 20; p.sk_cnt = (unsigned *)skc.p; p.sk_cnt_n = 4096;
+    DBuf panel((size_t)W.Npad * W.Kpad * 2);
+    const int t = tile ? tile : gemm_tile_for((int)M, (int)n, Kpad, W.wtype != W_F16);
+    if (W.wtype != W_F16 && W.wtype != W_F32 && gemm_tile_uses_panel(t % 1000000)) {
+        const DevWeight * w = &W;
+        half_t * o = (half_t *)panel.p;
+        launch_dequant(&w, &o, 1, s);
+        p.w16_pre = (const half_t *)panel.p + (size_t)n0 * Kpad;
+    }
+    launch_gemm(p, EPI_F16, tile, s);
+    launch_f16_to_f32((const half_t *)dout.p, (int)N, (float *)dout32.p, (int)N, (int)M, (int)N, s);
+    int rc = 0;
+    if (hipDeviceSynchronize() != hipSuccess || hipGetLastError() != hipSuccess) rc = -4;
+    else (void)hipMemcpy(y, dout32.p, (size_t)M * N * 4, hipMemcpyDeviceToHost);
+    (void)hipFree(wbase);
+    return rc;
+}
+
 float clip_amd_bench_attention(int nseq, int T, int h, int n_head, int causal, int kernel, int iters) {
     int ndev = 0;
     if (hipGetDeviceCount(&ndev) != hipSuccess || ndev <= 0) { (void)hipGetLastError(); return -1.f; }
diff --git a/clip_cpp_amd/csrc/forward.cpp b/clip_cpp_amd/csrc/forward.cpp
--- a/clip_cpp_amd/csrc/forward.cpp
+++ b/clip_cpp_amd/csrc/forward.cpp
@@ -312,8 +312,49 @@
     return true;
 }
 
+struct PooledRows {
+    int n = 0;
+    const int * in_rows = nullptr;
+    int in_row_mul = 1;
+    float * xp = nullptr;
+    half_t * ap = nullptr, * xnp = nullptr, * qp = nullptr;
+    bool pooled_q = false;
+};
+
+bool last_layer_pooled(clip_ctx * ctx, const DevLayer & l, GemmParams p, PooledRows & pr, int h, int nh, float eps, int nseq, int T_uniform,
+                       const int * d_seq_start, int max_len, const float * x, half_t * qkv) {
+    hipStream_t s = ctx->stream;
+    const int dh = h / nh;
+    if (h % 128 == 0) {
+        p.W = weight_rows(l.qkv, h, 2 * h);
+        if (p.w16_pre) p.w16_pre += (size_t)h * l.qkv.Kpad;
+        if (p.bias) p.bias += h;
+        if (p.ln_c) p.ln_c += h;
+        p.out = qkv + h;
+        p.qcols = 0;
+    }
+    gemm(ctx, "gemm_qkv", p, EPI_F16);
+    {
+        ProfScope ps(ctx, "gather_pooled", pr.n, h, 0, 0, (double)pr.n * h * 10);
+        launch_gather_ln_rows(x, pr.in_rows, pr.in_row_mul, l.ln1_w, l.ln1_b, eps, pr.n, h, pr.xp, pr.xnp, s);
+    }
+    GemmParams q;
+    q.A = pr.xnp; q.lda = h; q.M = pr.n; q.W = weight_rows(l.qkv, 0, h); q.bias = l.qkv_b; q.out = pr.qp; q.ldc = h;
+    q.qscale = 1.0f / sqrtf((float)dh); q.qcols = h;
+    gemm(ctx, "gemm_q_last", q, EPI_F16);
+    {
+        ProfScope ps(ctx, "attention_pooled", nseq * nh, max_len, dh, 4.0 * (double)nseq * nh * (double)max_len * dh, (double)nseq * max_len * h * 4);
+        if (!launch_attention_pooled(qkv, pr.qp, pr.ap, nseq, T_uniform, d_seq_start, h, nh, s)) {
+            fprintf(stderr, "clip (hip): pooled attention kernel does not support d_head=%d\n", dh);
+            return false;
+        }
+    }
+    pr.pooled_q = true;
+    return true;
+}
+
 bool run_layers(clip_ctx * ctx, const DevTower & tw, int rows, int h, int nh, int ff, float eps, int nseq, int T_uniform,
-                const int * d_seq_start, int max_len, bool causal, float * x, half_t * xn, half_t * qkv, half_t * att, half_t * mid, bool prune_last,
+                const int * d_seq_start, int max_len, bool causal, float * x, half_t * xn, half_t * qkv, half_t * att, half_t * mid, PooledRows * pool,
                 const half_t * const * resp = nullptr) {
     hipStream_t s = ctx->stream;
     const int dh = h / nh;
@@ -331,6 +372,8 @@
         p.A = xn; p.lda = h; p.M = rows; p.W = l.qkv; p.bias = l.qkv_b; p.out = qkv; p.ldc = 3 * h; p.w16_pre = lp.qkv;
         p.qscale = qscale; p.qcols = h;
         p.act_f32 = f32;
+        const bool last = pool && li + 1 == tw.layers.size();
+        if (last && !f32) return last_layer_pooled(ctx, l, p, *pool, h, nh, eps, nseq, T_uniform, d_seq_start, max_len, x, qkv);
         gemm(ctx, "gemm_qkv", p, EPI_F16);
         {
             const double afl = 4.0 * (double)nseq * nh * (double)max_len * max_len * dh;
@@ -341,7 +384,7 @@
                 return false;
             }
         }
-        if (prune_last && li + 1 == tw.layers.size()) break;
+        if (last) break;
         GemmParams po;
         po.A = att; po.lda = h; po.M = rows; po.W = l.o; po.bias = l.o_b; po.out = x; po.ldc = h; po.resid = x; po.w16_pre = lp.o; po.act_f32 = f32;
         gemm(ctx, "gemm_out", po, EPI_RESID_F32);
@@ -361,7 +404,7 @@
 
 bool run_layers_fold(clip_ctx * ctx, const DevTower & tw, int rows, int h, int nh, int ff, float eps, int nseq, int T_uniform,
                      const int * d_seq_start, int max_len, bool causal, float * x, half_t * xn, half_t * qkv, half_t * att, half_t * mid,
-                     float2 * stats, int stats_stride, float * mu, bool prune_last, const half_t * const * ff2p = nullptr) {
+                     float2 * stats, int stats_stride, float * mu, PooledRows * pool, const half_t * const * ff2p = nullptr) {
     hipStream_t s = ctx->stream;
     const int dh = h / nh;
     const float qscale = 1.0f / sqrtf((float)dh);
@@ -387,6 +430,7 @@
         p.M = rows; p.W = l.qkv; p.out = qkv; p.ldc = 3 * h; p.w16_pre = lp.qkv;
         p.qscale = qscale; p.qcols = h;
         consume(p, l.qkv_c, l.qkv_bf);
+        if (pool && li + 1 == tw.layers.size()) return last_layer_pooled(ctx, l, p, *pool, h, nh, eps, nseq, T_uniform, d_seq_start, max_len, x, qkv);
         gemm(ctx, "gemm_qkv", p, EPI_F16);
         {
             const double afl = 4.0 * (double)nseq * nh * (double)max_len * max_len * dh;
@@ -396,7 +440,6 @@
                 return false;
             }
         }
-        if (prune_last && li + 1 == tw.layers.size()) break;
         GemmParams po;
         po.A = att; po.lda = h; po.M = rows; po.W = l.o; po.bias = l.o_b; po.out = x; po.ldc = h; po.resid = x; po.w16_pre = lp.o;
         produce(po, l.ln2_w);
@@ -413,12 +456,15 @@
     return true;
 }
 
-bool pooled_tail(clip_ctx * ctx, const DevLayer & l, int n, int h, int ff, float eps, const float * x, const half_t * att, const int * in_rows,
-                 int in_row_mul, float * xp, half_t * ap, half_t * xnp, half_t * midp) {
+bool pooled_tail(clip_ctx * ctx, const DevLayer & l, const PooledRows & pr, int h, int ff, float eps, const float * x, const half_t * att, half_t * midp) {
     hipStream_t s = ctx->stream;
     const int act = ctx->use_gelu ? EPI_GELU_F16 : EPI_QGELU_F16;
     const bool f32 = ctx->f32_acts && l.o.wtype == W_F32 && l.ff1.wtype == W_F32 && l.ff2.wtype == W_F32;
-    {
+    const int n = pr.n, in_row_mul = pr.in_row_mul;
+    const int * in_rows = pr.in_rows;
+    float * xp = pr.xp;
+    half_t * ap = pr.ap, * xnp = pr.xnp;
+    if (!pr.pooled_q) {
         ProfScope ps(ctx, "gather_pooled", n, h, 0, 0, (double)n * h * 12);
         if (f32) {
             launch_gather_rows(x, nullptr, in_rows, in_row_mul, n, h, xp, nullptr, s);
@@ -754,6 +800,7 @@
         st.ap = c.take<half_t>(aw * Bc * h);
         st.xnp = c.take<half_t>(aw * Bc * h);
         st.midp = c.take<half_t>(aw * Bc * ff);
+        st.qp = c.take<half_t>((size_t)Bc * h);
     };
     Carver sizer(nullptr);
     carve(sizer);
@@ -803,17 +850,19 @@
         }
     }
     const bool prune = ctx->prune_last && !skinny && !V.layers.empty() && T > 1;
+    PooledRows pool;
+    pool.n = Bc; pool.in_row_mul = T; pool.xp = st.xp; pool.ap = st.ap; pool.xnp = st.xnp; pool.qp = st.qp;
     if (skinny && fold) {
         if (!run_layers_skinny_fold(ctx, V, rows, h, nh, ff, hp.eps, Bc, T, nullptr, T, false, x, st.xn, st.qkv, st.att, st.mid, st.stats, st.st_stride, ctx->ln_fold_centre ? st.mu : nullptr)) return false;
     } else if (skinny) {
         launch_row_stats(x, h, rows, h, ctx->sk_stats, s);
         if (!run_layers_skinny(ctx, V, rows, h, nh, ff, hp.eps, Bc, T, nullptr, T, false, x, st.qkv, st.att, st.mid)) return false;
     } else if (fold) {
-        if (!run_layers_fold(ctx, V, rows, h, nh, ff, hp.eps, Bc, T, nullptr, T, false, x, st.xn, st.qkv, st.att, st.mid, st.stats, st.st_stride, ctx->ln_fold_centre ? st.mu : nullptr, prune, resident_panels(ctx, V, 0, rows))) return false;
-    } else if (!run_layers(ctx, V, rows, h, nh, ff, hp.eps, Bc, T, nullptr, T, false, x, st.xn, st.qkv, st.att, st.mid, prune, resident_panels(ctx, V, 0, rows))) return false;
+        if (!run_layers_fold(ctx, V, rows, h, nh, ff, hp.eps, Bc, T, nullptr, T, false, x, st.xn, st.qkv, st.att, st.mid, st.stats, st.st_stride, ctx->ln_fold_centre ? st.mu : nullptr, prune ? &pool : nullptr, resident_panels(ctx, V, 0, rows))) return false;
+    } else if (!run_layers(ctx, V, rows, h, nh, ff, hp.eps, Bc, T, nullptr, T, false, x, st.xn, st.qkv, st.att, st.mid, prune ? &pool : nullptr, resident_panels(ctx, V, 0, rows))) return false;
     const bool f32 = acts_f32(ctx, V);
     if (prune) {
-        if (!pooled_tail(ctx, V.layers.back(), Bc, h, ff, hp.eps, x, st.att, nullptr, T, st.xp, st.ap, st.xnp, st.midp)) return false;
+        if (!pooled_tail(ctx, V.layers.back(), pool, h, ff, hp.eps, x, st.att, st.midp)) return false;
         layernorm_act(f32, st.xp, h, nullptr, 1, V.post_ln_w, V.post_ln_b, hp.eps, Bc, h, st.pooled, s);
     } else {
         layernorm_act(f32, x, h, nullptr, T, V.post_ln_w, V.post_ln_b, hp.eps, Bc, h, st.pooled, s);
@@ -879,7 +928,7 @@
     float2 * stats = nullptr;
     float * mu = nullptr;
     float * xp = nullptr;
-    half_t * ap = nullptr, * xnp = nullptr, * midp = nullptr;
+    half_t * ap = nullptr, * xnp = nullptr, * midp = nullptr, * qp = nullptr;
     auto carve = [&](Carver & c, float *& x, half_t *& xn, half_t *& qkv, half_t *& att, half_t *& mid, half_t *& pooled,
                      float *& emb, int *& seq, int *& last) {
         stats = c.take<float2>((size_t)(h / 16) * st_stride);
@@ -898,6 +947,7 @@
         ap = c.take<half_t>(aw * n_texts * h);
         xnp = c.take<half_t>(aw * n_texts * h);
         midp = c.take<half_t>(aw * n_texts * ff);
+        qp = c.take<half_t>((size_t)n_texts * h);
     };
     float *x, *emb;
     half_t *xn, *qkv, *att, *mid, *pooled;
@@ -974,6 +1024,8 @@
         const bool skinny = layers_fit_skinny(Tw, rows, h, ff);
         const bool fold = ctx->ln_fold && !Tw.layers.empty() && (ctx->ln_fold_force || fold_pays(Tw, rows, device_shared(ctx)));
         const bool prune = ctx->prune_last && !skinny && !Tw.layers.empty() && rows > n_texts;
+        PooledRows pool;
+        pool.n = n_texts; pool.in_rows = last; pool.xp = xp; pool.ap = ap; pool.xnp = xnp; pool.qp = qp;
         if (fold)
             launch_text_embed(d_ids + h_offsets[0], seq, n_texts, rows, Tw.tok_raw, Tw.tok_type, Tw.pos, h, x, s, Tw.layers[0].ln1_w, xn, h, stats, ctx->ln_fold_centre ? mu : nullptr);
         else launch_text_embed(d_ids + h_offsets[0], seq, n_texts, rows, Tw.tok_raw, Tw.tok_type, Tw.pos, h, x, s);
@@ -983,10 +1035,10 @@
             launch_row_stats(x, h, rows, h, ctx->sk_stats, s);
             if (!run_layers_skinny(ctx, Tw, rows, h, nh, ff, hp.eps, n_texts, 0, seq, max_len, true, x, qkv, att, mid)) return false;
         } else if (fold) {
-            if (!run_layers_fold(ctx, Tw, rows, h, nh, ff, hp.eps, n_texts, 0, seq, max_len, true, x, xn, qkv, att, mid, stats, st_stride, ctx->ln_fold_centre ? mu : nullptr, prune, resident_panels(ctx, Tw, 1, rows))) return false;
-        } else if (!run_layers(ctx, Tw, rows, h, nh, ff, hp.eps, n_texts, 0, seq, max_len, true, x, xn, qkv, att, mid, prune, resident_panels(ctx, Tw, 1, rows))) return false;
+            if (!run_layers_fold(ctx, Tw, rows, h, nh, ff, hp.eps, n_texts, 0, seq, max_len, true, x, xn, qkv, att, mid, stats, st_stride, ctx->ln_fold_centre ? mu : nullptr, prune ? &pool : nullptr, resident_panels(ctx, Tw, 1, rows))) return false;
+        } else if (!run_layers(ctx, Tw, rows, h, nh, ff, hp.eps, n_texts, 0, seq, max_len, true, x, xn, qkv, att, mid, prune ? &pool : nullptr, resident_panels(ctx, Tw, 1, rows))) return false;
         if (prune) {
-            if (!pooled_tail(ctx, Tw.layers.back(), n_texts, h, ff, hp.eps, x, att, last, 1, xp, ap, xnp, midp)) return false;
+            if (!pooled_tail(ctx, Tw.layers.back(), pool, h, ff, hp.eps, x, att, midp)) return false;
             layernorm_act(acts_f32(ctx, Tw), xp, h, nullptr, 1, Tw.post_ln_w, Tw.post_ln_b, hp.eps, n_texts, h, pooled, s);
         } else {
             layernorm_act(acts_f32(ctx, Tw), x, h, last, 1, Tw.post_ln_w, Tw.post_ln_b, hp.eps, n_texts, h, pooled, s);
diff --git a/clip_cpp_amd/csrc/k_attn_pooled.hip b/clip_cpp_amd/csrc/k_attn_pooled.hip
--- /dev/null
+++ b/clip_cpp_amd/csrc/k_attn_pooled.hip
@@ -0,0 +1,113 @@
+
+#include "kernels.h"
+
+namespace clipamd {
+
+typedef _Float16 h8 __attribute__((ext_vector_type(8)));
+typedef unsigned int u32x4 __attribute__((ext_vector_type(4)));
+
+namespace {
+
+template <int DH>
+__global__ void __launch_bounds__(256) attn_pooled_kernel(const half_t * __restrict__ qkv, const half_t * __restrict__ qp, half_t * __restrict__ out,
+                                                          const int * __restrict__ seq_start, int T_uniform, int h, int n_head) {
+    static_assert(DH % 8 == 0 && DH <= 128, "head size: whole 16-byte chunks, at most 16 per row");
+    constexpr int DCH = DH / 8;
+    constexpr int LPK = DCH <= 4 ? 4 : DCH <= 8 ? 8 : 16;
+    constexpr int KPI = 64 / LPK;
+    const int lane = threadIdx.x & 63, wave = threadIdx.x >> 6;
+    const int c = lane % LPK, kg = lane / LPK;
+    const bool cl = c < DCH;
+    const int cc = cl ? c : DCH - 1;
+    const int hg = (n_head + 3) / 4;
+    const int seq = blockIdx.x / hg;
+    const int head = (blockIdx.x % hg) * 4 + wave;
+    if (head >= n_head) return;
+    int row0, len;
+    if (seq_start) {
+        row0 = seq_start[seq];
+        len = seq_start[seq + 1] - row0;
+    } else {
+        row0 = seq * T_uniform;
+        len = T_uniform;
+    }
+    if (len <= 0) return;
+    const int ld = 3 * h;
+    const half_t * Kg = qkv + (size_t)row0 * ld + h + head * DH + cc * 8;
+    const half_t * Vg = Kg + h;
+    const h8 q = __builtin_bit_cast(h8, *(const u32x4 *)(qp + (size_t)seq * h + head * DH + cc * 8));
+    auto score = [&](int k) -> float {
+        const h8 kh = __builtin_bit_cast(h8, *(const u32x4 *)(Kg + (size_t)(k < len ? k : len - 1) * ld));
+        float a = 0.f;
+#pragma unroll
+        for (int e = 0; e < 8; e++) a = __builtin_fmaf((float)q[e], (float)kh[e], a);
+        a = cl ? a : 0.f;
+#pragma unroll
+        for (int o = LPK / 2; o > 0; o >>= 1) a += __shfl_xor(a, o);
+        return a;
+    };
+    const int nit = (len + KPI - 1) / KPI;
+    float mx = -INFINITY;
+#pragma unroll 4
+    for (int it = 0; it < nit; it++) {
+        const int k = it * KPI + kg;
+        const float s = score(k);
+        mx = fmaxf(mx, k < len ? s : -INFINITY);
+    }
+#pragma unroll
+    for (int o = 32; o >= LPK; o >>= 1) mx = fmaxf(mx, __shfl_xor(mx, o));
+    const float L2E = 1.44269504088896340736f;
+    const float nmx = -mx * L2E;
+    float sum = 0.f, o[8];
+#pragma unroll
+    for (int e = 0; e < 8; e++) o[e] = 0.f;
+#pragma unroll 4
+    for (int it = 0; it < nit; it++) {
+        const int k = it * KPI + kg;
+        const h8 vh = __builtin_bit_cast(h8, *(const u32x4 *)(Vg + (size_t)(k < len ? k : len - 1) * ld));
+        const float s = score(k);
+        const float e = k < len ? __builtin_amdgcn_exp2f(__builtin_fmaf(s, L2E, nmx)) : 0.f;
+        sum += c == 0 ? e : 0.f;
+        const float p = (float)(_Float16)e;
+#pragma unroll
+        for (int i = 0; i < 8; i++) o[i] = __builtin_fmaf(p, (float)vh[i], o[i]);
+    }
+#pragma unroll
+    for (int x = 32; x > 0; x >>= 1) sum += __shfl_xor(sum, x);
+#pragma unroll
+    for (int x = LPK; x < 64; x <<= 1) {
+#pragma unroll
+        for (int i = 0; i < 8; i++) o[i] += __shfl_xor(o[i], x);
+    }
+    const float inv = 1.0f / sum;
+    if (kg == 0 && cl) {
+        h8 r;
+#pragma unroll
+        for (int i = 0; i < 8; i++) r[i] = (_Float16)(o[i] * inv);
+        *(u32x4 *)(out + (size_t)seq * h + head * DH + c * 8) = __builtin_bit_cast(u32x4, r);
+    }
+}
+
+template <int DH>
+void launch_dh(const half_t * qkv, const half_t * qp, half_t * out, int nseq, int T_uniform, const int * seq_start, int h, int n_head, hipStream_t stream) {
+    hipLaunchKernelGGL((attn_pooled_kernel<DH>), dim3(nseq * ((n_head + 3) / 4)), dim3(256), 0, stream, qkv, qp, out, seq_start, T_uniform, h, n_head);
+}
+
+}
+
+bool launch_attention_pooled(const half_t * qkv, const half_t * qp, half_t * out, int nseq, int T_uniform, const int * seq_start, int h, int n_head,
+                             hipStream_t stream) {
+    if (nseq <= 0) return true;
+    if (n_head <= 0 || h % n_head) return false;
+    switch (h / n_head) {
+    case 32: launch_dh<32>(qkv, qp, out, nseq, T_uniform, seq_start, h, n_head, stream); return true;
+    case 64: launch_dh<64>(qkv, qp, out, nseq, T_uniform, seq_start, h, n_head, stream); return true;
+    case 80: launch_dh<80>(qkv, qp, out, nseq, T_uniform, seq_start, h, n_head, stream); return true;
+    case 88: launch_dh<88>(qkv, qp, out, nseq, T_uniform, seq_start, h, n_head, stream); return true;
+    case 96: launch_dh<96>(qkv, qp, out, nseq, T_uniform, seq_start, h, n_head, stream); return true;
+    case 104: launch_dh<104>(qkv, qp, out, nseq, T_uniform, seq_start, h, n_head, stream); return true;
+    }
+    return false;
+}
+
+}
diff --git a/clip_cpp_amd/csrc/k_misc.hip b/clip_cpp_amd/csrc/k_misc.hip
--- a/clip_cpp_amd/csrc/k_misc.hip
+++ b/clip_cpp_amd/csrc/k_misc.hip
@@ -549,6 +549,65 @@
 }
 
 namespace {
+template <int NV>
+__global__ void __launch_bounds__(256) gather_ln_rows_kernel(const float * __restrict__ x, const int * __restrict__ in_rows, int in_row_mul,
+                                                             const float * __restrict__ w, const float * __restrict__ b, float eps, int rows, int h,
+                                                             float * __restrict__ xp, half_t * __restrict__ xn) {
+    const int lane = threadIdx.x & 63;
+    const int r = blockIdx.x * 4 + (threadIdx.x >> 6);
+    if (r >= rows) return;
+    const long src = in_rows ? (long)in_rows[r] : (long)r * in_row_mul;
+    const float * xr = x + (size_t)src * h;
+    f4 v[NV];
+    float sum = 0.f;
+#pragma unroll
+    for (int i = 0; i < NV; i++) {
+        const int c = (i * 64 + lane) * 4;
+        if (c < h) {
+            v[i] = *(const f4 *)(xr + c);
+            *(f4 *)(xp + (size_t)r * h + c) = v[i];
+            sum += v[i][0] + v[i][1] + v[i][2] + v[i][3];
+        }
+    }
+    const float mean = wave_sum(sum) / (float)h;
+    float sq = 0.f;
+#pragma unroll
+    for (int i = 0; i < NV; i++) {
+        const int c = (i * 64 + lane) * 4;
+        if (c < h) {
+            v[i] = v[i] - mean;
+            sq += v[i][0] * v[i][0] + v[i][1] * v[i][1] + v[i][2] * v[i][2] + v[i][3] * v[i][3];
+        }
+    }
+    const float var = wave_sum(sq) / (float)h;
+    const float scale = 1.0f / sqrtf(var + eps);
+#pragma unroll
+    for (int i = 0; i < NV; i++) {
+        const int c = (i * 64 + lane) * 4;
+        if (c < h) {
+            const f4 ww = *(const f4 *)(w + c), bb = *(const f4 *)(b + c);
+            const f4 y = (v[i] * scale) * ww + bb;
+            const h2 lo = (h2){(_Float16)y[0], (_Float16)y[1]}, hi = (h2){(_Float16)y[2], (_Float16)y[3]};
+            *(uint2 *)(xn + (size_t)r * h + c) = make_uint2(__builtin_bit_cast(uint32_t, lo), __builtin_bit_cast(uint32_t, hi));
+        }
+    }
+}
+}
+void launch_gather_ln_rows(const float * x, const int * in_rows, int in_row_mul, const float * w, const float * b, float eps, int rows, int h,
+                           float * xp, half_t * xn, hipStream_t stream) {
+    if (rows <= 0) return;
+    const dim3 grid((rows + 3) / 4), block(256);
+#define CLIPAMD_GLN(NV) hipLaunchKernelGGL((gather_ln_rows_kernel<NV>), grid, block, 0, stream, x, in_rows, in_row_mul, w, b, eps, rows, h, xp, xn)
+    if (h <= 256) { CLIPAMD_GLN(1); }
+    else if (h <= 512) { CLIPAMD_GLN(2); }
+    else if (h <= 768) { CLIPAMD_GLN(3); }
+    else if (h <= 1024) { CLIPAMD_GLN(4); }
+    else if (h <= 1280) { CLIPAMD_GLN(5); }
+    else { CLIPAMD_GLN(8); }
+#undef CLIPAMD_GLN
+}
+
+namespace {
 __global__ void __launch_bounds__(256) meta_upload_kernel(const int * __restrict__ src, int * __restrict__ seq, int * __restrict__ last, int n_texts,
                                                           unsigned * done, unsigned stamp) {
     for (int i = threadIdx.x; i < 2 * n_texts + 1; i += 256) {
diff --git a/clip_cpp_amd/csrc/kernels.h b/clip_cpp_amd/csrc/kernels.h
--- a/clip_cpp_amd/csrc/kernels.h
+++ b/clip_cpp_amd/csrc/kernels.h
@@ -35,6 +35,21 @@
     const void * dm = nullptr;
     const void * w16 = nullptr;
 };
+
+inline DevWeight weight_rows(const DevWeight & W, int n0, int n) {
+    DevWeight v = W;
+    v.N = n;
+    if (W.wtype == W_F16 || W.wtype == W_F32) {
+        v.Npad = W.Npad - n0;
+        v.w16 = (const char *)W.w16 + (size_t)n0 * W.Kpad * (W.wtype == W_F32 ? 4 : 2);
+        return v;
+    }
+    const bool dm2 = W.wtype == W_Q4_1 || W.wtype == W_Q5_1;
+    v.qs = (const char *)W.qs + (size_t)n0 * (W.wtype == W_Q8_0 ? 32 : 16);
+    if (W.qh) v.qh = (const char *)W.qh + (size_t)n0 * 4;
+    v.dm = (const char *)W.dm + (size_t)n0 * (dm2 ? 4 : 2);
+    return v;
+}
 
 enum Epilogue : int {
     EPI_F32 = 0,
@@ -158,12 +173,18 @@
 bool launch_attention_long(const half_t * qkv, half_t * out, int nseq, int T_uniform, const int * seq_start, int max_len,
                            int h, int n_head, bool causal, hipStream_t stream);
 
+bool launch_attention_pooled(const half_t * qkv, const half_t * qp, half_t * out, int nseq, int T_uniform, const int * seq_start, int h, int n_head,
+                             hipStream_t stream);
+
 bool launch_attention_f32(const float * qkv, float * out, int nseq, int T_uniform, const int * seq_start, int max_len,
                           int h, int n_head, bool causal, hipStream_t stream);
 
 void launch_im2col(const void * imgs, bool imgs_f16, half_t * col, int B, int S, int P, int Kpad, hipStream_t stream);
 
 void launch_gather_rows(const float * x, const half_t * a, const int * in_rows, int in_row_mul, int rows, int h, float * xp, half_t * ap, hipStream_t stream);
+
+void launch_gather_ln_rows(const float * x, const int * in_rows, int in_row_mul, const float * w, const float * b, float eps, int rows, int h,
+                           float * xp, half_t * xn, hipStream_t stream);
 
 void launch_cls_rows(float * x, const float * class_embd, const float * pos, int B, int T, int h, hipStream_t stream);
 
diff --git a/clip_cpp_amd/csrc/model.h b/clip_cpp_amd/csrc/model.h
--- a/clip_cpp_amd/csrc/model.h
+++ b/clip_cpp_amd/csrc/model.h
@@ -187,6 +187,7 @@
     float * mu = nullptr;
     float * xp = nullptr;
     half_t * ap = nullptr, * xnp = nullptr, * midp = nullptr;
+    half_t * qp = nullptr;
 };
 bool vision_stage_begin(clip_ctx * ctx, int Bc, VisionStage & st);
 bool vision_stage_patch(clip_ctx * ctx, const VisionStage & st, const void * imgs, int i0, int n);
diff --git a/include/clip_amd.h b/include/clip_amd.h
--- a/include/clip_amd.h
+++ b/include/clip_amd.h
@@ -91,6 +91,10 @@
                             float * y, int out_f16);
 int clip_amd_test_attention(const float * qkv, int nseq, int T, int h, int n_head, int causal, float * out);
 int clip_amd_test_attention_ex(const float * qkv, int nseq, int T, int h, int n_head, int causal, float * out, int kernel);
+int clip_amd_test_attention_pooled(const float * qkv, const float * qp, int nseq, int T, const int * seq_start, int h, int n_head, int causal,
+                                   const int * rows_in, float * out, float * full_rows);
+int clip_amd_test_gemm_rows(int type, const void * w_raw, int64_t N, int64_t K, const float * x, int64_t M, const float * bias, float * y, int tile,
+                            int64_t n0, int64_t n, int qcols, float qscale);
 float clip_amd_bench_attention(int nseq, int T, int h, int n_head, int causal, int kernel, int iters);
 
 #ifdef __cplusplus
```
